# leijue222/Intra-and-Inter-Human-Relation-Network-for-MPEE

Hardware: AMD Instinct MI355X
Metric: images/sec (256x192 crops) I2R-Net HRNet-W48 inference (higher is better)
Workload: dtype f32; 1 GPU; vanilla I2R-Net HRNet-W48-S 256x192, 6 encoder layers, fp32, random weights (BASELINE configs[1]: w48_pure_en6); images_per_gpu=8, persons_per_image=4, crops_per_gpu_step=32, parallelism=single GPU, programs_per_forward=3

## Files before the change

### include/i2r_hip.h

```cpp
#ifndef I2R_HIP_H
#define I2R_HIP_H

#include <stdint.h>

#ifdef __cplusplus
extern "C" {
#endif

#define I2R_ABI_VERSION 17

#define I2R_API __attribute__((visibility("default")))

#define I2R_OK 0
#define I2R_E_ARG (-1)
#define I2R_E_LAUNCH (-2)
#define I2R_E_NODEV (-3)

#define I2R_MAX_TAPS 9

typedef struct i2r_conv_desc {
    const float* in;
    const float* in2;
    const float* w;
    const float* bias;
    const float* res1;
    const float* res2;
    const float* res_post;
    float* out;
    int32_t n_img;
    int32_t in_h, in_w, in_cs;
    int32_t cin;
    int32_t conv_h, conv_w;
    int32_t out_h, out_w, out_cs;
    int32_t cout, cout_pad;
    int32_t stride;
    int32_t iy0, ix0;
    int32_t ntaps;
    int32_t dy[I2R_MAX_TAPS], dx[I2R_MAX_TAPS];
    int32_t out_step, out_off_y, out_off_x, rep;
    int32_t relu;
    int32_t tile_h, tile_w;
    int32_t ck;
    int32_t wn;
    int32_t mt;
    int32_t dtype;
    int32_t in_f16, out_f16;
    int32_t algo;
    int32_t t1_shift, t2_shift;
    const float* t1;
    const float* t2;
    float* y;
    int32_t seq;
} i2r_conv_desc;

I2R_API int i2r_conv(const i2r_conv_desc* d, void* stream);

#define I2R_MAX_GROUP 4
I2R_API int i2r_conv_grouped(const i2r_conv_desc* const* descs, int32_t n, const int32_t* block_map, int32_t map_len,
                     void* stream);

I2R_API int i2r_stem_conv(const float* in_nchw, const float* w, const float* bias, float* out_nhwc, int32_t n_img,
                  int32_t cin, int32_t in_h, int32_t in_w, int32_t cout, int32_t out_cs, int32_t n_src, int32_t n_valid,
                  int32_t out_dt , void* stream);

I2R_API int i2r_pe_res_stem(const float* mask_nchw, const float* w_pre, const float* w7, const float* bias, float* out_nhwc,
                    int32_t n_img, int32_t in_h, int32_t in_w, int32_t cout, int32_t out_cs, int32_t n_src, int32_t n_valid, void* stream);

typedef struct i2r_pe_cat_vec_args {
    const float* in; const float* w; const float* bias; float* out;
    int32_t n_img, in_h, in_w, th, tw, rate, vec, out_cs, c0, c_end, n_src, n_valid;
} i2r_pe_cat_vec_args;
I2R_API int i2r_pe_cat_vec(const i2r_pe_cat_vec_args* a, void* stream);

I2R_API int i2r_maxpool3x3s2(const float* in, float* out, int32_t n_img, int32_t in_h, int32_t in_w, int32_t c,
                     int32_t in_cs, int32_t out_cs, void* stream);

I2R_API int i2r_head(const float* in, const float* w, const float* bias, float* out_nchw, int32_t n_img, int32_t h,
             int32_t w_, int32_t cin, int32_t in_cs, int32_t cout, void* stream);

I2R_API int i2r_conv_kernel_name(const i2r_conv_desc* const* descs, int32_t n, char* buf, int32_t buflen);

I2R_API int i2r_conv_grid(const i2r_conv_desc* const* descs, int32_t n, int32_t with_map, int32_t* grid, int32_t* seq);

I2R_API int i2r_flip_merge(const float* y, const float* y_flipped, const int32_t* joint_map, float* out, int32_t n, int32_t joints,
                   int32_t h, int32_t w, void* stream);

I2R_API int i2r_decode(const float* heatmaps, const float* center, const float* scale, float* preds, float* maxvals, int32_t n,
               int32_t joints, int32_t h, int32_t w, int32_t blur_kernel, int32_t transform_back, void* stream);

typedef struct i2r_pose_nms_args {
    const float* preds; const float* maxvals; const float* scale; const float* area; const float* box_score;
    const int32_t* img_off; const float* sigmas;
    float* score; int32_t* rank; int32_t* n_keep;
    double in_vis_thre, oks_thre, oks_vis_thre;
    int32_t n_crops, n_img, joints, max_persons, soft, max_dets, use_oks_vis, reserved;
} i2r_pose_nms_args;
I2R_API int i2r_pose_nms(const i2r_pose_nms_args* a, void* stream);

I2R_API int i2r_group_nearest(const double* anchors, const int32_t* person_off, const int32_t* member_off, int32_t n_img, int32_t n_persons,
                              int32_t n_members, int32_t max_patch, int32_t* members, void* stream);

typedef struct i2r_oks_match_args {
    const float* dt_kpts; const float* dt_score; const uint8_t* dt_valid; const int32_t* dt_off;
    const double* gt_kpts; const double* gt_area; const double* gt_bbox; const int32_t* gt_flags; const int32_t* gt_off;
    const double* sigmas; const double* thr; const double* area_rng;
    int32_t* dt_rank; uint32_t* dt_match; uint32_t* dt_ignore; uint8_t* gt_ignore; double* oks; const int64_t* oks_off;
    int64_t oks_len;
    int32_t n_dt, n_gt, n_img, joints, n_thr, n_area, max_dets, max_dt_per_img, max_gt_per_img, reserved;
} i2r_oks_match_args;
I2R_API int i2r_oks_match(const i2r_oks_match_args* a, void* stream);

typedef struct i2r_oks_accumulate_args {
    const uint32_t* dt_match; const uint32_t* dt_ignore; const int32_t* dt_rank; const int32_t* order; const int32_t* dt_img;
    const int32_t* img_group; const uint8_t* gt_ignore; const int32_t* gt_off; const double* rec_thr;
    double* precision; double* recall; int32_t* npig;
    int32_t n_dt, n_gt, n_img, n_part, n_group, n_thr, n_area, n_rec;
} i2r_oks_accumulate_args;
I2R_API int i2r_oks_accumulate(const i2r_oks_accumulate_args* a, void* stream);

typedef struct i2r_joint_targets_args {
    const double* joints_hm; const float* joints_vis; const float* joints_weight;
    float* target_weight; float* target;
    double sigma;
    int32_t n_crops, joints, h, w;
} i2r_joint_targets_args;
I2R_API int i2r_joint_targets(const i2r_joint_targets_args* a, void* stream);

typedef struct i2r_val_metrics_args {
    const float* output;
    const float* target; const float* target_weight;
    const double* joints_hm; const float* joints_vis; const float* joints_weight;
    void* ws;
    double* loss; double* acc; double* avg_acc; int32_t* cnt; float* pred; double* sse; int32_t* hits; int32_t* valid; double* meter;
    double sigma;
    int32_t n_crops, joints, h, w, use_target_weight, reserved;
} i2r_val_metrics_args;
I2R_API int i2r_val_metrics(const i2r_val_metrics_args* a, void* stream);

typedef struct i2r_val_combine_args {
    const double* parts;
    double* sse; int32_t* hits; int32_t* valid;
    double* loss; double* acc; double* avg_acc; int32_t* cnt; int32_t* n_crops; double* meter;
    int32_t n_part, joints, h, w;
} i2r_val_combine_args;
I2R_API int i2r_val_combine(const i2r_val_combine_args* a, void* stream);

I2R_API int i2r_crop_affine(const unsigned char* img, int32_t ih, int32_t iw, int32_t row_bytes, int32_t swap_rb, const float* inv_trans,
                    const float* mean, const float* inv_std, float* out, int32_t n, int32_t oh, int32_t ow, void* stream);

I2R_API int i2r_box_mask(const int32_t* boxes, int32_t ih, int32_t iw, float* out, int32_t n, int32_t oh, int32_t ow, void* stream);

I2R_API int i2r_crop_affine_cv2(const unsigned char* img, int32_t ih, int32_t iw, int32_t row_bytes, int32_t swap_rb, const double* inv_m,
                        const float* mean, const float* inv_std, float* out, int32_t n, int32_t oh, int32_t ow, void* stream);
I2R_API int i2r_box_mask_cv2(const int32_t* boxes, int32_t ih, int32_t iw, float* out, int32_t n, int32_t oh, int32_t ow, void* stream);

typedef struct {
    const unsigned char* img;
    int32_t ih, iw, row_bytes, reserved;
} i2r_image_ref;
typedef struct {
    double inv_m[6];
    int32_t box[4];
    int32_t image;
    int32_t reserved[3];
} i2r_crop_ref;
I2R_API int i2r_person_inputs_cv2(const i2r_image_ref* images, int32_t n_images, const i2r_crop_ref* crops, int32_t n_crops, int32_t swap_rb,
                          const float* mean, const float* inv_std, float* x_out, float* mask_out, int32_t oh, int32_t ow, void* stream);

I2R_API int i2r_layernorm(const float* in, const float* w, const float* b, float* out, int32_t npix, int32_t c, int32_t cs,
                  float eps, int32_t out_dt , void* stream);

I2R_API int i2r_window_attn(const float* qkv, const float* bias_qkv, float* out, int32_t n_img, int32_t h, int32_t w, int32_t c,
                    int32_t hs, int32_t heads, void* stream);

I2R_API int i2r_hrt_attn_block(const float* x, float* out, const float* ln_w, const float* ln_b, const void* wqkv, const float* bqkv,
                       const void* wo, const float* bo, int32_t n_img, int32_t h, int32_t w, int32_t c, int32_t cs, int32_t heads,
                       float eps, int32_t dtype, int32_t variant, void* stream);

I2R_API int i2r_hrt_mlp_block(const float* x, float* out, const float* ln_w, const float* ln_b, const void* w1, const float* b1,
                      const float* wdw, const float* bdw, const void* w2, const float* b2, int32_t n_img, int32_t h, int32_t w,
                      int32_t c, int32_t cs, int32_t hidden_pad, float eps, int32_t dtype, int32_t variant, void* stream);

I2R_API int i2r_dwconv3x3(const float* in, const float* w, const float* bias, float* out, int32_t n_img, int32_t in_h, int32_t in_w,
                  int32_t c, int32_t cs, int32_t stride, int32_t act, int32_t dt ,
                  void* stream);

I2R_API int i2r_upsample_bilinear_add(const float* low, const float* res, float* out, int32_t n_img, int32_t low_h, int32_t low_w,
                              int32_t scale, int32_t c, int32_t cs, int32_t act, void* stream);
struct i2r_up_args;
I2R_API int i2r_upsample_bilinear_add_multi(const struct i2r_up_args* a, void* stream);

I2R_API int i2r_fuse_up_add(const float* base, const float* t1, int32_t s1, const float* t2, int32_t s2, float* out, int32_t n_img,
                    int32_t h, int32_t w, int32_t cs, int32_t act, int32_t dt, void* stream);

typedef struct i2r_conv1x1_pair_args {
    const float* x; const float* w_a; const float* b_a; const float* res; float* y;
    const float* w_b; const float* b_b; float* z;
    int32_t n_pix, k_a, ca_out, cb_out, x_cs, y_cs, z_cs, relu_a, relu_b, mt;
} i2r_conv1x1_pair_args;
I2R_API int i2r_conv1x1_pair(const i2r_conv1x1_pair_args* a, void* stream);

typedef struct i2r_conv1x1_lp_args {
    const void* x; const void* w; const float* bias; const void* res1; const void* res_post; void* out;
    int32_t n_pix, cin_pad, cout_pad, x_cs, out_cs, act, dtype, in_16, out_16, mt;
    const void* res2;
} i2r_conv1x1_lp_args;
I2R_API int i2r_conv1x1_lp(const i2r_conv1x1_lp_args* a, void* stream);

typedef struct i2r_encoder_desc {
    const float* src;
    const float* pos;
    float* kbuf;
    float* vbuf;
    float* out;
    const int32_t* grp_off;
    const float* w_in;
    const float* b_in;
    const float* w_out;
    const float* b_out;
    const float* ln1_w; const float* ln1_b;
    const float* w1;
    const float* b1;
    const float* w2;
    const float* b2;
    const float* ln2_w; const float* ln2_b;
    int32_t n_tok, n_grp;
    int32_t d;
    int32_t cs;
    int32_t dff_pad;
    int32_t pos_period;
    int32_t n_qtiles32;
    float ln_eps;
    int32_t dtype;
    int32_t n_qtiles16, n_qtiles64;
    const void* w_in_lp; const void* w_out_lp; const void* w1_lp; const void* w2_lp;
    const float* next_w_in; const float* next_b_in; float* next_kbuf; float* next_vbuf;
    const float* vec_lp;
    float* split_ws; int32_t* split_cnt;
    int32_t n_qtiles192;
} i2r_encoder_desc;

I2R_API int i2r_encoder_kv(const i2r_encoder_desc* d, void* stream);
I2R_API int i2r_encoder_layer(const i2r_encoder_desc* d, void* stream);

typedef struct i2r_mh_attn_args {
    const float* qk; const float* v; float* out; const int32_t* grp_off;
    int32_t n_grp, heads, hp, k_off, qk_cs, v_cs, out_cs, n_qtiles16, n_qtiles32, n_qtiles64;
    const int32_t* key_len;
} i2r_mh_attn_args;
I2R_API int i2r_mh_attention(const i2r_mh_attn_args* a, void* stream);

typedef struct i2r_attn_weights_args {
    const float* qk; float* out; const int32_t* grp_off; const int64_t* out_off; float* ws;
    int32_t n_grp, heads, hp, k_off, qk_cs, n_tiles, ws_stride;
} i2r_attn_weights_args;
I2R_API int i2r_attn_weights(const i2r_attn_weights_args* a, void* stream);

typedef struct i2r_attn_query_args {
    const float* qk; float* out; const int32_t* grp_off; const int64_t* out_off; float* ws; const int32_t* q_tok; const int32_t* q_cnt;
    float* rows; const int32_t* grp_off_host;
    int32_t n_grp, heads, hp, k_off, qk_cs, n_tiles, ws_stride, mode, K, scale, h, w, n_col_tiles, reserved;
} i2r_attn_query_args;
I2R_API int i2r_attn_query_maps(const i2r_attn_query_args* a, void* stream);

I2R_API int i2r_rows_gather(const float* src, float* out, const int32_t* map, int32_t n_out, int32_t floats_per_crop, void* stream);
I2R_API int i2r_view_scramble(const float* o, float* out, const int32_t* person_map, int32_t n_out, int32_t n_images, int32_t max_persons, int32_t c,
                              int32_t cs, int32_t hw, void* stream);
typedef struct i2r_gather_args { const float* src; float* out; const int32_t* map; int32_t n_out, floats_per_crop; } i2r_gather_args;
typedef struct i2r_scramble_args { const float* o; float* out; const int32_t* person_map; int32_t n_out, n_images, max_persons, c, cs, hw; } i2r_scramble_args;

#define I2R_MAX_GATHER_SEGS 8
typedef struct i2r_gather_seg { const void* src; void* out; const int32_t* map; int32_t n_out, n_src; int64_t row_bytes; } i2r_gather_seg;
typedef struct i2r_gather_multi_args { i2r_gather_seg seg[I2R_MAX_GATHER_SEGS ]; int32_t n_seg; } i2r_gather_multi_args;
I2R_API int i2r_rows_gather_multi(const i2r_gather_multi_args* a, void* stream);

enum {
    I2R_OP_CONV = 1, I2R_OP_STEM = 2, I2R_OP_MAXPOOL = 3, I2R_OP_HEAD = 4,
    I2R_OP_ENC_KV = 5, I2R_OP_ENC_LAYER = 6, I2R_OP_FORK = 7, I2R_OP_JOIN = 8, I2R_OP_CONV_GROUP = 9,
    I2R_OP_LAYERNORM = 10, I2R_OP_WINATTN = 11, I2R_OP_DWCONV = 12, I2R_OP_UPSAMPLE = 13,
    I2R_OP_PE_RES_STEM = 15, I2R_OP_HRT_ATTN = 16, I2R_OP_HRT_MLP = 17,  I2R_OP_FUSE_UP = 19,
    I2R_OP_CONV1X1_PAIR = 20, I2R_OP_CONV1X1_LP = 21, I2R_OP_MH_ATTN = 22, I2R_OP_PE_CAT_VEC = 23, I2R_OP_ROWS_GATHER = 24, I2R_OP_VIEW_SCRAMBLE = 25,
    I2R_OP_RECORD = 26, I2R_OP_WAIT = 27, I2R_OP_LANE_FLAGS = 28, I2R_OP_ATTN_WEIGHTS = 29,
    I2R_OP_ATTN_QUERY = 30,
    I2R_OP_ROWS_GATHER_MULTI = 31
};

typedef struct i2r_stem_args {
    const float* in; const float* w; const float* bias; float* out;
    int32_t n_img, cin, in_h, in_w, cout, out_cs, n_src, n_valid, out_dt;
} i2r_stem_args;

typedef struct i2r_pe_res_args {
    const float* in; const float* w_pre; const float* w7; const float* bias; float* out;
    int32_t n_img, in_h, in_w, cout, out_cs, n_src, n_valid;
} i2r_pe_res_args;

typedef struct i2r_pool_args {
    const float* in; float* out;
    int32_t n_img, in_h, in_w, c, in_cs, out_cs;
} i2r_pool_args;

typedef struct i2r_head_args {
    const float* in; const float* w; const float* bias; float* out;
    int32_t n_img, h, w_, cin, in_cs, cout;
} i2r_head_args;

typedef struct i2r_ln_args {
    const float* in; const float* w; const float* b; float* out;
    int32_t npix, c, cs; float eps; int32_t out_dt;
} i2r_ln_args;

typedef struct i2r_winattn_args {
    const float* qkv; const float* bias; float* out;
    int32_t n_img, h, w_, c, cs, heads;
} i2r_winattn_args;

typedef struct i2r_hrt_attn_args {
    const float* x; float* out; const float* ln_w; const float* ln_b; const void* wqkv; const float* bqkv; const void* wo; const float* bo;
    int32_t n_img, h, w_, c, cs, heads; float eps; int32_t dtype, variant;
} i2r_hrt_attn_args;

typedef struct i2r_hrt_mlp_args {
    const float* x; float* out; const float* ln_w; const float* ln_b; const void* w1; const float* b1; const float* wdw; const float* bdw;
    const void* w2; const float* b2;
    int32_t n_img, h, w_, c, cs, hidden_pad; float eps; int32_t dtype, variant;
} i2r_hrt_mlp_args;

typedef struct i2r_dw_args {
    const float* in; const float* w; const float* bias; float* out;
    int32_t n_img, in_h, in_w, c, cs, stride, act, dt;
} i2r_dw_args;

typedef struct i2r_up_args {
    const float* low; const float* res; float* out;
    int32_t n_img, low_h, low_w, scale, c, cs, act;
    const float* low2; const float* low3;
    int32_t scale2, scale3;
} i2r_up_args;

typedef struct i2r_fuse_up_args {
    const float* base; const float* t1; const float* t2; float* out;
    int32_t n_img, h, w, cs, s1, s2, act, dt;
} i2r_fuse_up_args;

typedef struct i2r_conv_group_args {
    const i2r_conv_desc* d[I2R_MAX_GROUP];
    const int32_t* block_map;
    int32_t n;
    int32_t map_len;
} i2r_conv_group_args;

typedef struct i2r_op {
    int32_t kind;
    int32_t lane;
    const void* args;
} i2r_op;

I2R_API int i2r_run_program(const i2r_op* ops, int32_t n_ops, void* const* streams, void* const* events);
I2R_API int i2r_run_program_timed(const i2r_op* ops, int32_t n_ops, void* const* streams, void* const* events, void* const* t0,
                                  void* const* t1);

I2R_API int i2r_abi_version(void);
I2R_API const char* i2r_last_error(void);
I2R_API int i2r_device_check(int32_t dev, int32_t* cu_count, int32_t* lds_bytes);

#ifdef __cplusplus
}
#endif
#endif
```

### intra-and-inter-human-relation-network-for-mpee_amd/cabi.py

```python
import ctypes as C
import os

import torch

_HERE = os.path.dirname(os.path.abspath(__file__))
LIB_PATH = os.path.join(_HERE, "libi2r_hip.so")

MAX_TAPS = 9
ABI_VERSION = 17
OP_CONV, OP_STEM, OP_MAXPOOL, OP_HEAD, OP_ENC_KV, OP_ENC_LAYER, OP_FORK, OP_JOIN, OP_CONV_GROUP = 1, 2, 3, 4, 5, 6, 7, 8, 9
MAX_GROUP = 4
OP_LAYERNORM, OP_WINATTN, OP_DWCONV, OP_UPSAMPLE = 10, 11, 12, 13
OP_CONV_CHAIN = 14
OP_PE_RES_STEM = 15
OP_HRT_ATTN = 16
OP_HRT_MLP = 17
OP_XSYNC = 18
OP_FUSE_UP = 19
OP_CONV1X1_PAIR = 20
OP_CONV1X1_LP = 21
OP_MH_ATTN = 22
OP_PE_CAT_VEC = 23
OP_ROWS_GATHER, OP_VIEW_SCRAMBLE = 24, 25
OP_RECORD, OP_WAIT = 26, 27
OP_LANE_FLAGS = 28
CAPTURE_OP_ATTN_WEIGHTS = 29
CAPTURE_OP_ATTN_QUERY = 30
GROUPS_OP_ROWS_GATHER_MULTI = 31
MAX_GATHER_SEGS = 8
SYNC_OPS = (OP_FORK, OP_JOIN, OP_XSYNC, OP_RECORD, OP_WAIT, OP_LANE_FLAGS)

_fp = C.c_void_p
_i32 = C.c_int32


class ConvDesc(C.Structure):
    _fields_ = [
        ("in_", _fp), ("in2", _fp), ("w", _fp), ("bias", _fp), ("res1", _fp), ("res2", _fp), ("res_post", _fp), ("out", _fp),
        ("n_img", _i32), ("in_h", _i32), ("in_w", _i32), ("in_cs", _i32), ("cin", _i32),
        ("conv_h", _i32), ("conv_w", _i32), ("out_h", _i32), ("out_w", _i32), ("out_cs", _i32),
        ("cout", _i32), ("cout_pad", _i32), ("stride", _i32), ("iy0", _i32), ("ix0", _i32), ("ntaps", _i32),
        ("dy", _i32 * MAX_TAPS), ("dx", _i32 * MAX_TAPS),
        ("out_step", _i32), ("out_off_y", _i32), ("out_off_x", _i32), ("rep", _i32), ("relu", _i32),
        ("tile_h", _i32), ("tile_w", _i32), ("ck", _i32), ("wn", _i32), ("mt", _i32), ("dtype", _i32),
        ("in_f16", _i32), ("out_f16", _i32), ("algo", _i32),
        ("t1_shift", _i32), ("t2_shift", _i32), ("t1", _fp), ("t2", _fp), ("y", _fp),
        ("seq", _i32),
    ]


class EncoderDesc(C.Structure):
    _fields_ = [
        ("src", _fp), ("pos", _fp), ("kbuf", _fp), ("vbuf", _fp), ("out", _fp), ("grp_off", _fp),
        ("w_in", _fp), ("b_in", _fp), ("w_out", _fp), ("b_out", _fp), ("ln1_w", _fp), ("ln1_b", _fp),
        ("w1", _fp), ("b1", _fp), ("w2", _fp), ("b2", _fp), ("ln2_w", _fp), ("ln2_b", _fp),
        ("n_tok", _i32), ("n_grp", _i32), ("d", _i32), ("cs", _i32), ("dff_pad", _i32), ("pos_period", _i32),
        ("n_qtiles32", _i32), ("ln_eps", C.c_float), ("dtype", _i32), ("n_qtiles16", _i32), ("n_qtiles64", _i32),
        ("w_in_lp", _fp), ("w_out_lp", _fp), ("w1_lp", _fp), ("w2_lp", _fp),
        ("next_w_in", _fp), ("next_b_in", _fp), ("next_kbuf", _fp), ("next_vbuf", _fp), ("vec_lp", _fp),
        ("split_ws", _fp), ("split_cnt", _fp), ("n_qtiles192", _i32),
    ]


class StemArgs(C.Structure):
    _fields_ = [("in_", _fp), ("w", _fp), ("bias", _fp), ("out", _fp),
                ("n_img", _i32), ("cin", _i32), ("in_h", _i32), ("in_w", _i32), ("cout", _i32), ("out_cs", _i32), ("n_src", _i32),
                ("n_valid", _i32), ("out_dt", _i32)]


class PeResArgs(C.Structure):
    _fields_ = [("in_", _fp), ("w_pre", _fp), ("w7", _fp), ("bias", _fp), ("out", _fp),
                ("n_img", _i32), ("in_h", _i32), ("in_w", _i32), ("cout", _i32), ("out_cs", _i32), ("n_src", _i32), ("n_valid", _i32)]


class PeCatVecArgs(C.Structure):
    _fields_ = [("in_", _fp), ("w", _fp), ("bias", _fp), ("out", _fp),
                ("n_img", _i32), ("in_h", _i32), ("in_w", _i32), ("th", _i32), ("tw", _i32), ("rate", _i32), ("vec", _i32), ("out_cs", _i32),
                ("c0", _i32), ("c_end", _i32), ("n_src", _i32), ("n_valid", _i32)]


class PoolArgs(C.Structure):
    _fields_ = [("in_", _fp), ("out", _fp),
                ("n_img", _i32), ("in_h", _i32), ("in_w", _i32), ("c", _i32), ("in_cs", _i32), ("out_cs", _i32)]


class HeadArgs(C.Structure):
    _fields_ = [("in_", _fp), ("w", _fp), ("bias", _fp), ("out", _fp),
                ("n_img", _i32), ("h", _i32), ("w_", _i32), ("cin", _i32), ("in_cs", _i32), ("cout", _i32)]


class LnArgs(C.Structure):
    _fields_ = [("in_", _fp), ("w", _fp), ("b", _fp), ("out", _fp), ("npix", _i32), ("c", _i32), ("cs", _i32), ("eps", C.c_float),
                ("out_dt", _i32)]


class MhAttnArgs(C.Structure):
    _fields_ = [("qk", _fp), ("v", _fp), ("out", _fp), ("grp_off", _fp),
                ("n_grp", _i32), ("heads", _i32), ("hp", _i32), ("k_off", _i32), ("qk_cs", _i32), ("v_cs", _i32), ("out_cs", _i32),
                ("n_qtiles16", _i32), ("n_qtiles32", _i32), ("n_qtiles64", _i32), ("key_len", _fp)]


class AttnWeightsArgs(C.Structure):
    _fields_ = [("qk", _fp), ("out", _fp), ("grp_off", _fp), ("out_off", _fp), ("ws", _fp),
                ("n_grp", _i32), ("heads", _i32), ("hp", _i32), ("k_off", _i32), ("qk_cs", _i32), ("n_tiles", _i32), ("ws_stride", _i32)]


class AttnQueryArgs(C.Structure):
    _fields_ = [("qk", _fp), ("out", _fp), ("grp_off", _fp), ("out_off", _fp), ("ws", _fp), ("q_tok", _fp), ("q_cnt", _fp), ("rows", _fp),
                ("grp_off_host", _fp),
                ("n_grp", _i32), ("heads", _i32), ("hp", _i32), ("k_off", _i32), ("qk_cs", _i32), ("n_tiles", _i32), ("ws_stride", _i32),
                ("mode", _i32), ("K", _i32), ("scale", _i32), ("h", _i32), ("w", _i32), ("n_col_tiles", _i32), ("reserved", _i32)]


class GatherArgs(C.Structure):
    _fields_ = [("src", _fp), ("out", _fp), ("map", _fp), ("n_out", _i32), ("floats_per_crop", _i32)]


class GatherSeg(C.Structure):
    _fields_ = [("src", _fp), ("out", _fp), ("map", _fp), ("n_out", _i32), ("n_src", _i32), ("row_bytes", C.c_int64)]


class GatherMultiArgs(C.Structure):
    _fields_ = [("seg", GatherSeg * MAX_GATHER_SEGS), ("n_seg", _i32)]


class ScrambleArgs(C.Structure):
    _fields_ = [("o", _fp), ("out", _fp), ("person_map", _fp), ("n_out", _i32), ("n_images", _i32), ("max_persons", _i32), ("c", _i32), ("cs", _i32),
                ("hw", _i32)]


class WinAttnArgs(C.Structure):
    _fields_ = [("qkv", _fp), ("bias", _fp), ("out", _fp),
                ("n_img", _i32), ("h", _i32), ("w_", _i32), ("c", _i32), ("cs", _i32), ("heads", _i32)]


class HrtAttnArgs(C.Structure):
    _fields_ = [("x", _fp), ("out", _fp), ("ln_w", _fp), ("ln_b", _fp), ("wqkv", _fp), ("bqkv", _fp), ("wo", _fp), ("bo", _fp),
                ("n_img", _i32), ("h", _i32), ("w_", _i32), ("c", _i32), ("cs", _i32), ("heads", _i32), ("eps", C.c_float), ("dtype", _i32),
                ("variant", _i32)]


class HrtMlpArgs(C.Structure):
    _fields_ = [("x", _fp), ("out", _fp), ("ln_w", _fp), ("ln_b", _fp), ("w1", _fp), ("b1", _fp), ("wdw", _fp), ("bdw", _fp), ("w2", _fp),
                ("b2", _fp), ("n_img", _i32), ("h", _i32), ("w_", _i32), ("c", _i32), ("cs", _i32), ("hidden_pad", _i32), ("eps", C.c_float),
                ("dtype", _i32), ("variant", _i32)]


class DwArgs(C.Structure):
    _fields_ = [("in_", _fp), ("w", _fp), ("bias", _fp), ("out", _fp),
                ("n_img", _i32), ("in_h", _i32), ("in_w", _i32), ("c", _i32), ("cs", _i32), ("stride", _i32), ("act", _i32), ("dt", _i32)]


class UpArgs(C.Structure):
    _fields_ = [("low", _fp), ("res", _fp), ("out", _fp),
                ("n_img", _i32), ("low_h", _i32), ("low_w", _i32), ("scale", _i32), ("c", _i32), ("cs", _i32), ("act", _i32),
                ("low2", _fp), ("low3", _fp), ("scale2", _i32), ("scale3", _i32)]


class FuseUpArgs(C.Structure):
    _fields_ = [("base", _fp), ("t1", _fp), ("t2", _fp), ("out", _fp),
                ("n_img", _i32), ("h", _i32), ("w", _i32), ("cs", _i32), ("s1", _i32), ("s2", _i32), ("act", _i32), ("dt", _i32)]


class Conv1x1PairArgs(C.Structure):
    _fields_ = [("x", _fp), ("w_a", _fp), ("b_a", _fp), ("res", _fp), ("y", _fp), ("w_b", _fp), ("b_b", _fp), ("z", _fp),
                ("n_pix", _i32), ("k_a", _i32), ("ca_out", _i32), ("cb_out", _i32), ("x_cs", _i32), ("y_cs", _i32), ("z_cs", _i32),
                ("relu_a", _i32), ("relu_b", _i32), ("mt", _i32)]


class Conv1x1LpArgs(C.Structure):
    _fields_ = [("x", _fp), ("w", _fp), ("bias", _fp), ("res1", _fp), ("res_post", _fp), ("out", _fp),
                ("n_pix", _i32), ("cin_pad", _i32), ("cout_pad", _i32), ("x_cs", _i32), ("out_cs", _i32), ("act", _i32), ("dtype", _i32),
                ("in_16", _i32), ("out_16", _i32), ("mt", _i32), ("res2", _fp)]


class ConvGroupArgs(C.Structure):
    _fields_ = [("d", C.POINTER(ConvDesc) * MAX_GROUP), ("block_map", _fp), ("n", _i32), ("map_len", _i32)]


class PoseNmsArgs(C.Structure):
    _fields_ = [("preds", _fp), ("maxvals", _fp), ("scale", _fp), ("area", _fp), ("box_score", _fp), ("img_off", _fp), ("sigmas", _fp),
                ("score", _fp), ("rank", _fp), ("n_keep", _fp),
                ("in_vis_thre", C.c_double), ("oks_thre", C.c_double), ("oks_vis_thre", C.c_double),
                ("n_crops", _i32), ("n_img", _i32), ("joints", _i32), ("max_persons", _i32), ("soft", _i32), ("max_dets", _i32),
                ("use_oks_vis", _i32), ("reserved", _i32)]


class OksMatchArgs(C.Structure):
    _fields_ = [("dt_kpts", _fp), ("dt_score", _fp), ("dt_valid", _fp), ("dt_off", _fp),
                ("gt_kpts", _fp), ("gt_area", _fp), ("gt_bbox", _fp), ("gt_flags", _fp), ("gt_off", _fp),
                ("sigmas", _fp), ("thr", _fp), ("area_rng", _fp),
                ("dt_rank", _fp), ("dt_match", _fp), ("dt_ignore", _fp), ("gt_ignore", _fp), ("oks", _fp), ("oks_off", _fp),
                ("oks_len", C.c_int64),
                ("n_dt", _i32), ("n_gt", _i32), ("n_img", _i32), ("joints", _i32), ("n_thr", _i32), ("n_area", _i32), ("max_dets", _i32),
                ("max_dt_per_img", _i32), ("max_gt_per_img", _i32), ("reserved", _i32)]


class OksAccumulateArgs(C.Structure):
    _fields_ = [("dt_match", _fp), ("dt_ignore", _fp), ("dt_rank", _fp), ("order", _fp), ("dt_img", _fp),
                ("img_group", _fp), ("gt_ignore", _fp), ("gt_off", _fp), ("rec_thr", _fp),
                ("precision", _fp), ("recall", _fp), ("npig", _fp),
                ("n_dt", _i32), ("n_gt", _i32), ("n_img", _i32), ("n_part", _i32), ("n_group", _i32), ("n_thr", _i32), ("n_area", _i32),
                ("n_rec", _i32)]


class JointTargetsArgs(C.Structure):
    _fields_ = [("joints_hm", _fp), ("joints_vis", _fp), ("joints_weight", _fp), ("target_weight", _fp), ("target", _fp),
                ("sigma", C.c_double), ("n_crops", _i32), ("joints", _i32), ("h", _i32), ("w", _i32)]


class ValMetricsArgs(C.Structure):
    _fields_ = [("output", _fp), ("target", _fp), ("target_weight", _fp), ("joints_hm", _fp), ("joints_vis", _fp), ("joints_weight", _fp),
                ("ws", _fp), ("loss", _fp), ("acc", _fp), ("avg_acc", _fp), ("cnt", _fp), ("pred", _fp), ("sse", _fp), ("hits", _fp),
                ("valid", _fp), ("meter", _fp), ("sigma", C.c_double),
                ("n_crops", _i32), ("joints", _i32), ("h", _i32), ("w", _i32), ("use_target_weight", _i32), ("reserved", _i32)]


class ValCombineArgs(C.Structure):
    _fields_ = [("parts", _fp), ("sse", _fp), ("hits", _fp), ("valid", _fp), ("loss", _fp), ("acc", _fp), ("avg_acc", _fp), ("cnt", _fp),
                ("n_crops", _fp), ("meter", _fp), ("n_part", _i32), ("joints", _i32), ("h", _i32), ("w", _i32)]


class ImageRef(C.Structure):
    _fields_ = [("img", C.c_void_p), ("ih", _i32), ("iw", _i32), ("row_bytes", _i32), ("reserved", _i32)]


class CropRef(C.Structure):
    _fields_ = [("inv_m", C.c_double * 6), ("box", _i32 * 4), ("image", _i32), ("reserved", _i32 * 3)]


class Op(C.Structure):
    _fields_ = [("kind", _i32), ("lane", _i32), ("args", C.c_void_p)]


EXPORTS = ("i2r_conv", "i2r_conv_grouped", "i2r_conv_kernel_name", "i2r_conv_grid", "i2r_stem_conv", "i2r_pe_res_stem", "i2r_maxpool3x3s2", "i2r_head", "i2r_layernorm", "i2r_window_attn", "i2r_hrt_attn_block", "i2r_hrt_mlp_block", "i2r_dwconv3x3",
           "i2r_upsample_bilinear_add", "i2r_upsample_bilinear_add_multi", "i2r_fuse_up_add", "i2r_conv1x1_pair", "i2r_conv1x1_lp", "i2r_flip_merge", "i2r_decode", "i2r_pose_nms", "i2r_group_nearest", "i2r_oks_match", "i2r_oks_accumulate", "i2r_joint_targets", "i2r_val_metrics", "i2r_val_combine", "i2r_crop_affine", "i2r_box_mask", "i2r_crop_affine_cv2", "i2r_box_mask_cv2", "i2r_person_inputs_cv2", "i2r_encoder_kv", "i2r_encoder_layer", "i2r_mh_attention", "i2r_attn_weights", "i2r_attn_query_maps", "i2r_pe_cat_vec", "i2r_rows_gather", "i2r_rows_gather_multi", "i2r_view_scramble",
           "i2r_run_program", "i2r_run_program_timed", "i2r_abi_version", "i2r_last_error", "i2r_device_check")

_LIB = None


class I2RError(RuntimeError):
    pass


def load_library(path=LIB_PATH):
    if not os.path.exists(path):
        raise I2RError(
            "HIP extension %s is missing -- build it with `python -c 'import __graft_entry__ as g; g.build()'`. "
            "There is no CPU fallback for the product path." % path)
    L = C.CDLL(path)
    L.i2r_conv.argtypes = [C.POINTER(ConvDesc), C.c_void_p]
    L.i2r_conv_grouped.argtypes = [C.POINTER(C.POINTER(ConvDesc)), _i32, _fp, _i32, C.c_void_p]
    L.i2r_conv_kernel_name.argtypes = [C.POINTER(C.POINTER(ConvDesc)), _i32, C.c_char_p, _i32]
    L.i2r_conv_grid.argtypes = [C.POINTER(C.POINTER(ConvDesc)), _i32, _i32, C.POINTER(_i32), C.POINTER(_i32)]
    L.i2r_stem_conv.argtypes = [_fp, _fp, _fp, _fp, _i32, _i32, _i32, _i32, _i32, _i32, _i32, _i32, _i32, C.c_void_p]
    L.i2r_pe_res_stem.argtypes = [_fp, _fp, _fp, _fp, _fp, _i32, _i32, _i32, _i32, _i32, _i32, _i32, C.c_void_p]
    L.i2r_flip_merge.argtypes = [_fp, _fp, _fp, _fp, _i32, _i32, _i32, _i32, C.c_void_p]
    L.i2r_decode.argtypes = [_fp, _fp, _fp, _fp, _fp, _i32, _i32, _i32, _i32, _i32, _i32, C.c_void_p]
    L.i2r_pose_nms.argtypes = [C.POINTER(PoseNmsArgs), C.c_void_p]
    L.i2r_group_nearest.argtypes = [_fp, _fp, _fp, _i32, _i32, _i32, _i32, _fp, C.c_void_p]
    L.i2r_oks_match.argtypes = [C.POINTER(OksMatchArgs), C.c_void_p]
    L.i2r_oks_accumulate.argtypes = [C.POINTER(OksAccumulateArgs), C.c_void_p]
    L.i2r_joint_targets.argtypes = [C.POINTER(JointTargetsArgs), C.c_void_p]
    L.i2r_val_metrics.argtypes = [C.POINTER(ValMetricsArgs), C.c_void_p]
    L.i2r_val_combine.argtypes = [C.POINTER(ValCombineArgs), C.c_void_p]
    L.i2r_crop_affine.argtypes = [_fp, _i32, _i32, _i32, _i32, _fp, _fp, _fp, _fp, _i32, _i32, _i32, C.c_void_p]
    L.i2r_box_mask.argtypes = [_fp, _i32, _i32, _fp, _i32, _i32, _i32, C.c_void_p]
    L.i2r_crop_affine_cv2.argtypes = [_fp, _i32, _i32, _i32, _i32, _fp, _fp, _fp, _fp, _i32, _i32, _i32, C.c_void_p]
    L.i2r_box_mask_cv2.argtypes = [_fp, _i32, _i32, _fp, _i32, _i32, _i32, C.c_void_p]
    L.i2r_person_inputs_cv2.argtypes = [_fp, _i32, _fp, _i32, _i32, C.POINTER(C.c_float), C.POINTER(C.c_float), _fp, _fp, _i32, _i32, C.c_void_p]
    L.i2r_fuse_up_add.argtypes = [_fp, _fp, _i32, _fp, _i32, _fp, _i32, _i32, _i32, _i32, _i32, _i32, C.c_void_p]
    L.i2r_conv1x1_pair.argtypes = [C.POINTER(Conv1x1PairArgs), C.c_void_p]
    L.i2r_conv1x1_lp.argtypes = [C.POINTER(Conv1x1LpArgs), C.c_void_p]
    L.i2r_maxpool3x3s2.argtypes = [_fp, _fp, _i32, _i32, _i32, _i32, _i32, _i32, C.c_void_p]
    L.i2r_head.argtypes = [_fp, _fp, _fp, _fp, _i32, _i32, _i32, _i32, _i32, _i32, C.c_void_p]
    L.i2r_layernorm.argtypes = [_fp, _fp, _fp, _fp, _i32, _i32, _i32, C.c_float, _i32, C.c_void_p]
    L.i2r_window_attn.argtypes = [_fp, _fp, _fp, _i32, _i32, _i32, _i32, _i32, _i32, C.c_void_p]
    L.i2r_hrt_attn_block.argtypes = [_fp, _fp, _fp, _fp, _fp, _fp, _fp, _fp, _i32, _i32, _i32, _i32, _i32, _i32, C.c_float, _i32, _i32, C.c_void_p]
    L.i2r_hrt_mlp_block.argtypes = [_fp] * 10 + [_i32] * 6 + [C.c_float, _i32, _i32, C.c_void_p]
    L.i2r_dwconv3x3.argtypes = [_fp, _fp, _fp, _fp, _i32, _i32, _i32, _i32, _i32, _i32, _i32, _i32, C.c_void_p]
    L.i2r_upsample_bilinear_add_multi.argtypes = [C.POINTER(UpArgs), C.c_void_p]
    L.i2r_upsample_bilinear_add.argtypes = [_fp, _fp, _fp, _i32, _i32, _i32, _i32, _i32, _i32, _i32, C.c_void_p]
    L.i2r_encoder_kv.argtypes = [C.POINTER(EncoderDesc), C.c_void_p]
    L.i2r_encoder_layer.argtypes = [C.POINTER(EncoderDesc), C.c_void_p]
    L.i2r_rows_gather.argtypes = [_fp, _fp, _fp, _i32, _i32, C.c_void_p]
    L.i2r_rows_gather_multi.argtypes = [C.POINTER(GatherMultiArgs), C.c_void_p]
    L.i2r_view_scramble.argtypes = [_fp, _fp, _fp, _i32, _i32, _i32, _i32, _i32, _i32, C.c_void_p]
    L.i2r_pe_cat_vec.argtypes = [C.POINTER(PeCatVecArgs), C.c_void_p]
    L.i2r_mh_attention.argtypes = [C.POINTER(MhAttnArgs), C.c_void_p]
    L.i2r_attn_weights.argtypes = [C.POINTER(AttnWeightsArgs), C.c_void_p]
    L.i2r_attn_query_maps.argtypes = [C.POINTER(AttnQueryArgs), C.c_void_p]
    L.i2r_run_program.argtypes = [C.POINTER(Op), _i32, C.POINTER(C.c_void_p), C.POINTER(C.c_void_p)]
    L.i2r_run_program_timed.argtypes = [C.POINTER(Op), _i32] + [C.POINTER(C.c_void_p)] * 4
    L.i2r_device_check.argtypes = [_i32, C.POINTER(_i32), C.POINTER(_i32)]
    L.i2r_last_error.restype = C.c_char_p
    for name in EXPORTS:
        if name != "i2r_last_error":
            getattr(L, name).restype = C.c_int
    return L


def lib():
    global _LIB
    if _LIB is None:
        L = load_library()
        if L.i2r_abi_version() != ABI_VERSION:
            raise I2RError("libi2r_hip.so ABI version %d != %d -- rebuild" % (L.i2r_abi_version(), ABI_VERSION))
        _LIB = L
    return _LIB


def check(rc, what=""):
    if rc != 0:
        msg = lib().i2r_last_error()
        raise I2RError("%s failed (rc=%d): %s" % (what or "i2r call", rc, msg.decode() if msg else "?"))


def require_gfx950(device_index=0):
    cu, lds = _i32(0), _i32(0)
    check(lib().i2r_device_check(device_index, C.byref(cu), C.byref(lds)), "i2r_device_check")
    return cu.value, lds.value
```

### intra-and-inter-human-relation-network-for-mpee_amd/csrc/i2r_conv.h

```cpp
#pragma once
#include "i2r_common.h"

#ifdef I2R_TUNING
#define I2R_DBG(p) ((p).dbg)
#else
#define I2R_DBG(p) 0
#endif

namespace {

struct ConvK {
    const float* in;
    const float* in2;
    const float* w;
    const float* bias;
    const float* res1;
    const float* res2;
    const float* res_post;
    float* out;
    int n_img, in_h, in_w, in_cs, cin;
    int conv_h, conv_w, out_h, out_w, out_cs, cout, cout_pad;
    int stride, iy0, ix0, ntaps;
    int tap_kh, tap_kw;
    int out_step, out_off_y, out_off_x, rep, relu;
    int tile_h, tile_w, tiles_y, tiles_x, n_cblk;
    int ph, pw, plane;
    int ck;
    int wn;
    int dtype;
    int in16, out16;
    int dbg;
    unsigned m_cblk, m_tx, m_ty, m_pw, m_tw;
    unsigned in_bytes, w_bytes, out_bytes;
    int wn_log, npass;
    int algo, w_fwlog, w_pitch, w_half, w_nfrag, w_rcp;
    int w_seq;
    int w_band;
    unsigned w_m_cblk, w_m_img, w_m_tx;
    const float* f_t1;
    const float* f_t2;
    float* f_y;
    int f_sh1, f_sh2;
    unsigned f_bytes1, f_bytes2;
};

__device__ __forceinline__ int div_m(int n, int d, unsigned m) { return d == 1 ? n : (int)__umulhi((unsigned)n, m); }

typedef unsigned u32x4 __attribute__((ext_vector_type(4)));
typedef unsigned u32x2 __attribute__((ext_vector_type(2)));
constexpr unsigned kOOB = 0x80000000u;
__device__ __forceinline__ __amdgpu_buffer_rsrc_t make_rsrc(const void* base, unsigned bytes) {
    return __builtin_amdgcn_make_buffer_rsrc(const_cast<void*>(base), 0, base ? bytes : 0, 0x00020000);
}
__device__ __forceinline__ f32x4 buf_ld16(const __amdgpu_buffer_rsrc_t& rs, unsigned voff, int soff) {
    return __builtin_bit_cast(f32x4, __builtin_amdgcn_raw_buffer_load_b128(rs, voff, soff, 0));
}
__device__ __forceinline__ void buf_st16(const __amdgpu_buffer_rsrc_t& rs, unsigned voff, int soff, f32x4 v) {
    __builtin_amdgcn_raw_buffer_store_b128(__builtin_bit_cast(u32x4, v), rs, voff, soff, 0);
    asm volatile("s_nop 1" ::"v"(v));
}

constexpr int kMaxPP = 5;

constexpr int kMaxGroups = 4;
struct ConvGroupK {
    ConvK g[kMaxGroups];
    int blk_end[kMaxGroups];
    int n;
    const int* blk_map;
};

template <int DT>
__device__ __forceinline__ f32x4 ld_act4(const float* base, size_t off, bool h16) {
    if constexpr (DT != 0) {
        if (h16) {
            const uint2 u = *reinterpret_cast<const uint2*>(reinterpret_cast<const unsigned short*>(base) + off);
            if constexpr (DT == 1)
                return (f32x4){__uint_as_float(u.x << 16), __uint_as_float(u.x & 0xFFFF0000u), __uint_as_float(u.y << 16), __uint_as_float(u.y & 0xFFFF0000u)};
            else {
                typedef _Float16 h4 __attribute__((ext_vector_type(4)));
                const h4 h = __builtin_bit_cast(h4, u);
                return (f32x4){(float)h[0], (float)h[1], (float)h[2], (float)h[3]};
            }
        }
    }
    return *reinterpret_cast<const f32x4*>(base + off);
}
template <int DT>
__device__ __forceinline__ void st_act4(float* base, size_t off, f32x4 v, bool h16) {
    if constexpr (DT != 0) {
        if (h16) {
            uint2 u;
            if constexpr (DT == 1) {
                typedef __bf16 b4 __attribute__((ext_vector_type(4)));
                const b4 b = {(__bf16)v[0], (__bf16)v[1], (__bf16)v[2], (__bf16)v[3]};
                u = __builtin_bit_cast(uint2, b);
            } else {
                typedef _Float16 h4 __attribute__((ext_vector_type(4)));
                const h4 h = {(_Float16)v[0], (_Float16)v[1], (_Float16)v[2], (_Float16)v[3]};
                u = __builtin_bit_cast(uint2, h);
            }
            *reinterpret_cast<uint2*>(reinterpret_cast<unsigned short*>(base) + off) = u;
            return;
        }
    }
    *reinterpret_cast<f32x4*>(base + off) = v;
}

template <int DT>
__device__ __forceinline__ f32x4 buf_ld_act4(const __amdgpu_buffer_rsrc_t& rs, unsigned voff, bool h16) {
    if constexpr (DT != 0) {
        if (h16) {
            const u32x2 u = __builtin_amdgcn_raw_buffer_load_b64(rs, voff, 0, 0);
            if constexpr (DT == 1)
                return (f32x4){__uint_as_float(u.x << 16), __uint_as_float(u.x & 0xFFFF0000u), __uint_as_float(u.y << 16), __uint_as_float(u.y & 0xFFFF0000u)};
            else {
                typedef _Float16 h4 __attribute__((ext_vector_type(4)));
                const h4 h = __builtin_bit_cast(h4, u);
                return (f32x4){(float)h[0], (float)h[1], (float)h[2], (float)h[3]};
            }
        }
    }
    return buf_ld16(rs, voff, 0);
}
template <int DT>
__device__ __forceinline__ void buf_st_act4(const __amdgpu_buffer_rsrc_t& rs, unsigned voff, f32x4 v, bool h16) {
    if constexpr (DT != 0) {
        if (h16) {
            u32x2 u;
            if constexpr (DT == 1) {
                typedef __bf16 b4 __attribute__((ext_vector_type(4)));
                const b4 b = {(__bf16)v[0], (__bf16)v[1], (__bf16)v[2], (__bf16)v[3]};
                u = __builtin_bit_cast(u32x2, b);
            } else {
                typedef _Float16 h4 __attribute__((ext_vector_type(4)));
                const h4 h = {(_Float16)v[0], (_Float16)v[1], (_Float16)v[2], (_Float16)v[3]};
                u = __builtin_bit_cast(u32x2, h);
            }
            __builtin_amdgcn_raw_buffer_store_b64(u, rs, voff, 0, 0);
            return;
        }
    }
    __builtin_amdgcn_raw_buffer_store_b128(__builtin_bit_cast(u32x4, v), rs, voff, 0, 0);
}

template <int MT, int NT, int DT>
__device__ __forceinline__ void conv_epilogue(const ConvK& p, f32x4 (&acc)[MT][NT], int img, int oy0, int ox0, int wm, int n_base,
                                              int li, int g, int tile_px) {
    if ((I2R_DBG(p) & 1) && acc[0][0][0] != 12345.678f) return;
    const int j4 = li & 3;
    const int pj = li >> 2, pq = li & 3;
    const int perm_src = (g * 16 + pq * 4 + pj) * 4;
    auto to_pixel_major = [&](f32x4 v) {
        v = quad_transpose(v, j4);
#pragma unroll
        for (int e = 0; e < 4; ++e) {
            const float x = v[e];
            v[e] = __int_as_float(__builtin_amdgcn_ds_bpermute(perm_src, __float_as_int(x)));
        }
        return v;
    };
    const bool h16 = DT != 0 && p.out16;
    const unsigned esz = h16 ? 2u : 4u;
    const __amdgpu_buffer_rsrc_t rs_out = make_rsrc(p.out, p.out_bytes), rs_r1 = make_rsrc(p.res1, p.out_bytes),
                                 rs_r2 = make_rsrc(p.res2, p.out_bytes), rs_rp = make_rsrc(p.res_post, p.out_bytes);
    auto finish = [&](f32x4 t, int n, bool full, unsigned voff) {
        if (p.relu == 1) {
            t[0] = fmaxf(t[0], 0.f); t[1] = fmaxf(t[1], 0.f); t[2] = fmaxf(t[2], 0.f); t[3] = fmaxf(t[3], 0.f);
        } else if (p.relu == 2) {
#pragma unroll
            for (int e = 0; e < 4; ++e) t[e] = 0.5f * t[e] * (1.f + erff(t[e] * 0.70710678118654752f));
        }
        if (p.res_post) t += buf_ld_act4<DT>(rs_rp, voff, h16);
        if (!full) {
#pragma unroll
            for (int e = 0; e < 4; ++e)
                if (n + e >= p.cout) t[e] = 0.f;
        }
        return t;
    };
    f32x4 bias[NT];
    unsigned noff[NT];
    const bool tail = n_base + NT * 16 > p.cout || n_base + NT * 16 > p.out_cs;
#pragma unroll
    for (int nt = 0; nt < NT; ++nt) {
        const int n = n_base + nt * 16 + pq * 4;
        const bool nok = n < p.cout_pad && (n + 4 <= p.cout || n + 4 <= p.out_cs);
        noff[nt] = nok ? (unsigned)n * esz : kOOB;
        bias[nt] = n < p.cout_pad ? *reinterpret_cast<const f32x4*>(p.bias + n) : (f32x4){0.f, 0.f, 0.f, 0.f};
    }
    if (p.rep == 1 && !(I2R_DBG(p) & 16)) {
        unsigned off[MT];
#pragma unroll
        for (int mt = 0; mt < MT; ++mt) {
            const int m = (wm * MT + mt) * 16 + g * 4 + pj;
            const int ty = div_m(m, p.tile_w, p.m_tw), tx = m - ty * p.tile_w;
            const int oy = oy0 + ty, ox = ox0 + tx;
            const bool pv = m < tile_px && oy < p.conv_h && ox < p.conv_w;
            off[mt] = pv ? (unsigned)(((img * p.out_h + oy * p.out_step + p.out_off_y) * p.out_w + ox * p.out_step + p.out_off_x) * p.out_cs) * esz : kOOB;
        }
        auto at = [&](int mt, int nt) { return (tail && noff[nt] == kOOB) ? kOOB : off[mt] + noff[nt]; };
        f32x4 r[MT][NT];
#pragma unroll
        for (int mt = 0; mt < MT; ++mt)
#pragma unroll
            for (int nt = 0; nt < NT; ++nt) {
                r[mt][nt] = bias[nt];
                if (p.res1) r[mt][nt] += buf_ld_act4<DT>(rs_r1, at(mt, nt), h16);
                if (p.res2) r[mt][nt] += buf_ld_act4<DT>(rs_r2, at(mt, nt), h16);
            }
#pragma unroll
        for (int mt = 0; mt < MT; ++mt)
#pragma unroll
            for (int nt = 0; nt < NT; ++nt) {
                const f32x4 v = to_pixel_major(acc[mt][nt]);
                const int n = n_base + nt * 16 + pq * 4;
                const unsigned o = at(mt, nt);
                buf_st_act4<DT>(rs_out, o, finish(v + r[mt][nt], n, !tail || n + 4 <= p.cout, o), h16);
            }
        return;
    }
#pragma unroll
    for (int mt = 0; mt < MT; ++mt) {
        const int m = (wm * MT + mt) * 16 + g * 4 + pj;
        const int ty = div_m(m, p.tile_w, p.m_tw), tx = m - ty * p.tile_w;
        const int oy = oy0 + ty, ox = ox0 + tx;
        const bool pvalid = m < tile_px && oy < p.conv_h && ox < p.conv_w;
        const int by = oy * p.out_step + p.out_off_y, bx = ox * p.out_step + p.out_off_x;
#pragma unroll
        for (int nt = 0; nt < NT; ++nt) {
            const f32x4 v = to_pixel_major(acc[mt][nt]) + bias[nt];
            const int n = n_base + nt * 16 + pq * 4;
            if (!pvalid || noff[nt] == kOOB) continue;
            for (int ry = 0; ry < p.rep; ++ry)
                for (int rx = 0; rx < p.rep; ++rx) {
                    const unsigned o = (unsigned)(((img * p.out_h + by + ry) * p.out_w + bx + rx) * p.out_cs) * esz + noff[nt];
                    f32x4 t = v;
                    if (p.res1) t += buf_ld_act4<DT>(rs_r1, o, h16);
                    if (p.res2) t += buf_ld_act4<DT>(rs_r2, o, h16);
                    buf_st_act4<DT>(rs_out, o, finish(t, n, n + 4 <= p.cout, o), h16);
                }
        }
    }
}



typedef void (*conv_fn)(const ConvGroupK);

}

void* i2r_pick_conv_bf16(int nt, int mt, int cap, int pf);
void* i2r_pick_conv_f16(int nt, int mt, int cap, int pf);
void* i2r_pick_conv_wino(int nt, int mt, int fin);
size_t i2r_conv_wino_lds(int nt, int mt, int plane);
```

### intra-and-inter-human-relation-network-for-mpee_amd/csrc/i2r_conv.hip

```cpp
#include <stdlib.h>

#include <algorithm>

#include "i2r_conv.h"

namespace {

template <int MT, int NT, int CAP, int PF>
__device__ __forceinline__ void conv_body(const ConvK& p, int bid, f32x4* lds) {
    const int tid = threadIdx.x;
    unsigned long long ts0 = 0, ts1 = 0, ts2 = 0;
    const bool stamp = (I2R_DBG(p) & 8) != 0;
    const int bid_stamp = bid;
    if (stamp) ts0 = __builtin_amdgcn_s_memtime();
    const int lane = tid & 63, wave = tid >> 6;
    const int WN = p.wn;
    const int wm = wave >> p.wn_log, wn = wave & (WN - 1);
    const int li = lane & 15, g = lane >> 4;

    int q = div_m(bid, p.n_cblk, p.m_cblk);
    const int cb = bid - q * p.n_cblk;
    bid = q;
    q = div_m(bid, p.tiles_x, p.m_tx);
    const int tile_x = bid - q * p.tiles_x;
    bid = q;
    const int img = div_m(bid, p.tiles_y, p.m_ty);
    const int tile_y = bid - img * p.tiles_y;
    const int oy0 = tile_y * p.tile_h, ox0 = tile_x * p.tile_w;
    const int py0 = oy0 * p.stride + p.iy0, px0 = ox0 * p.stride + p.ix0;
    const int phw = p.ph * p.pw;

    constexpr int NPP = PF > 0 ? 4 * PF : kMaxPP;
    const int ul = tid & 3;
    const __amdgpu_buffer_rsrc_t rs_in = make_rsrc(p.in, p.in_bytes), rs_in2 = make_rsrc(p.in2, p.in_bytes), rs_w = make_rsrc(p.w, p.w_bytes);
    unsigned goff[NPP];
#pragma unroll
    for (int j = 0; j < NPP; ++j) {
        const int pp = PF > 0 ? (tid >> 2) + j * 64 : tid + j * 256;
        goff[j] = kOOB;
        if (pp < phw) {
            const int py = div_m(pp, p.pw, p.m_pw), px = pp - py * p.pw;
            const int iy = py0 + py, ix = px0 + px;
            if (iy >= 0 && iy < p.in_h && ix >= 0 && ix < p.in_w) goff[j] = (unsigned)(((img * p.in_h + iy) * p.in_w + ix) * p.in_cs) * 4u;
        }
    }
    const int npp = (phw + 255) >> 8;

    const int tile_px = p.tile_h * p.tile_w;
    int ppix[MT];
#pragma unroll
    for (int mt = 0; mt < MT; ++mt) {
        int m = (wm * MT + mt) * 16 + li;
        if (m >= tile_px) m = 0;
        const int ty = div_m(m, p.tile_w, p.m_tw), tx = m - ty * p.tile_w;
        ppix[mt] = ty * p.stride * p.pw + tx * p.stride;
    }

    f32x4 acc[MT][NT];
#pragma unroll
    for (int mt = 0; mt < MT; ++mt)
#pragma unroll
        for (int nt = 0; nt < NT; ++nt) acc[mt][nt] = (f32x4){0.f, 0.f, 0.f, 0.f};

    const int n_base = (cb * WN + wn) * NT * 16;
    const int cin4 = p.cin >> 2;
    const unsigned wlane = (unsigned)(n_base + li + g * p.cout_pad) * 16u;

    auto run_chunk = [&](const f32x4* buf, int c0, int ckc, auto&& mid) {
        const int ncs = ckc >> 4;
        const int nit = p.ntaps * ncs;
        const int wp0 = (c0 >> 2) * p.cout_pad * 16;
        int wp = wp0;
        const int inc_cs = 4 * p.cout_pad * 16;
        const int inc_tap = (cin4 - (ncs - 1) * 4) * p.cout_pad * 16;
        int cs_n = 0, tx_n = 0, ty_n = 0;
        auto fetch = [&](f32x4(&a)[MT], f32x4(&b)[NT]) {
#pragma unroll
            for (int nt = 0; nt < NT; ++nt) b[nt] = buf_ld16(rs_w, wlane + nt * 256u, (I2R_DBG(p) & 4) ? wp0 : wp);
            const int abase = (cs_n * 4 + g) * p.plane + ty_n * p.pw + tx_n;
#pragma unroll
            for (int mt = 0; mt < MT; ++mt) a[mt] = buf[abase + ppix[mt]];
            if (++cs_n == ncs) {
                cs_n = 0;
                wp += inc_tap;
                if (++tx_n == p.tap_kw) {
                    tx_n = 0;
                    if (++ty_n == p.tap_kh) { ty_n = 0; wp = wp0; }
                }
            } else {
                wp += inc_cs;
            }
        };
        auto fma_step = [&](const f32x4(&a)[MT], const f32x4(&b)[NT]) {
#pragma unroll
            for (int s = 0; s < 4; ++s)
#pragma unroll
                for (int mt = 0; mt < MT; ++mt)
#pragma unroll
                    for (int nt = 0; nt < NT; ++nt) acc[mt][nt] = mfma16(a[mt][s], b[nt][s], acc[mt][nt]);
        };
        f32x4 a0[MT], a1[MT], b0[NT], b1[NT];
        fetch(a0, b0);
        mid();
        int it = 0;
        for (; it + 2 <= nit; it += 2) {
            fetch(a1, b1);
            fma_step(a0, b0);
            fetch(a0, b0);
            fma_step(a1, b1);
        }
        if (it < nit) fma_step(a0, b0);
    };

    if constexpr (PF > 0) {
        constexpr int UQ = CAP / 4, PJ = 4 * PF;
        f32x4 v[UQ][PJ];
        const int ckg = p.ck >> 2;
        auto stage_load = [&](int c0) {
#pragma unroll
            for (int uq = 0; uq < UQ; ++uq)
                if (uq * 4 < ckg) {
#pragma unroll
                    for (int j = 0; j < PJ; ++j)
                        v[uq][j] = (I2R_DBG(p) & 2) ? (f32x4){0.f, 0.f, 0.f, 0.f} : buf_ld16(rs_in, goff[j] + (uq * 4 + ul) * 16u, c0 * 4);
                }
            if (p.in2) {
#pragma unroll
                for (int uq = 0; uq < UQ; ++uq)
                    if (uq * 4 < ckg) {
#pragma unroll
                        for (int j = 0; j < PJ; ++j)
                            v[uq][j] += buf_ld16(rs_in2, goff[j] + (uq * 4 + ul) * 16u, c0 * 4);
                    }
            }
        };
        auto stage_store = [&](f32x4* buf) {
#pragma unroll
            for (int uq = 0; uq < UQ; ++uq)
                if (uq * 4 < ckg) {
#pragma unroll
                    for (int j = 0; j < PJ; ++j) {
                        const int pp = (tid >> 2) + j * 64;
                        if (pp < phw) buf[(uq * 4 + ul) * p.plane + pp] = v[uq][j];
                    }
                }
        };
        const int npass = p.npass;
        stage_load(0);
        stage_store(lds);
        __syncthreads();
        if (stamp) ts1 = __builtin_amdgcn_s_memtime();
        for (int pass = 0; pass < npass; ++pass) {
            f32x4* cur = lds + (pass & 1) * ckg * p.plane;
            f32x4* nxt = lds + ((pass + 1) & 1) * ckg * p.plane;
            const bool more = pass + 1 < npass;
            run_chunk(cur, pass * p.ck, p.ck, [&]() { if (more) stage_load((pass + 1) * p.ck); });
            if (more) stage_store(nxt);
            __syncthreads();
        }
    } else {
        for (int c0 = 0; c0 < p.cin; c0 += p.ck) {
            const int ckc = min(p.ck, p.cin - c0);
            const int ncg = ckc >> 2;
            if (c0 != 0) __syncthreads();
            for (int cg0 = 0; cg0 < ncg; cg0 += 4) {
                f32x4 v[4][kMaxPP];
#pragma unroll
                for (int u = 0; u < 4; ++u)
#pragma unroll
                    for (int j = 0; j < kMaxPP; ++j)
                        v[u][j] = (j < npp && !(I2R_DBG(p) & 2)) ? buf_ld16(rs_in, goff[j] + u * 16u, (c0 + cg0 * 4) * 4) : (f32x4){0.f, 0.f, 0.f, 0.f};
                if (p.in2) {
#pragma unroll
                    for (int u = 0; u < 4; ++u)
#pragma unroll
                        for (int j = 0; j < kMaxPP; ++j)
                            if (j < npp) v[u][j] += buf_ld16(rs_in2, goff[j] + u * 16u, (c0 + cg0 * 4) * 4);
                }
#pragma unroll
                for (int u = 0; u < 4; ++u)
#pragma unroll
                    for (int j = 0; j < kMaxPP; ++j) {
                        const int pp = tid + j * 256;
                        if (j < npp && pp < phw)
                            lds[(cg0 + u) * p.plane + pp] = v[u][j];
                    }
            }
            __syncthreads();
            run_chunk(lds, c0, ckc, []() {});
        }
    }

    if (stamp) {
        ts2 = __builtin_amdgcn_s_memtime();
        ConvK q = p;
        q.res2 = nullptr;
        conv_epilogue<MT, NT, 0>(q, acc, img, oy0, ox0, wm, n_base, li, g, tile_px);
        asm volatile("s_waitcnt vmcnt(0)" ::: "memory");
        const unsigned long long ts3 = __builtin_amdgcn_s_memtime();
        if (tid == 0) {
            unsigned long long* o = reinterpret_cast<unsigned long long*>(const_cast<float*>(p.res2)) + (size_t)bid_stamp * 4;
            o[0] = ts0; o[1] = ts1; o[2] = ts2; o[3] = ts3;
            if (I2R_DBG(p) & 32) {
                const unsigned hw = __builtin_amdgcn_s_getreg((4 << 0) | (0 << 6) | (31 << 11));
                const unsigned xcc = __builtin_amdgcn_s_getreg((20 << 0) | (0 << 6) | (3 << 11));
                o[1] = ((unsigned long long)xcc << 32) | hw;
            }
        }
        return;
    }
    conv_epilogue<MT, NT, 0>(p, acc, img, oy0, ox0, wm, n_base, li, g, tile_px);
}

template <int MT, int NT, int CAP, int PF>
__global__ __launch_bounds__(256) void conv_igemm_f32(const ConvGroupK grp) {
    extern __shared__ __attribute__((aligned(16))) f32x4 lds[];
    int bid = blockIdx.x, gi = 0, start = 0;
    if (grp.blk_map) {
        const int v = __builtin_amdgcn_readfirstlane(grp.blk_map[bid]);
        gi = v >> 24;
        bid = v & 0xFFFFFF;
    } else {
#pragma unroll
        for (int i = 0; i < kMaxGroups - 1; ++i)
            if (i + 1 < grp.n && bid >= grp.blk_end[i]) { gi = i + 1; start = grp.blk_end[i]; }
    }
    conv_body<MT, NT, CAP, PF>(grp.g[gi], bid - start, lds);
}

template <int NT, int CAP, int PF>
conv_fn pick_mt(int mt) {
    switch (mt) {
        case 1: return conv_igemm_f32<1, NT, CAP, PF>;
        case 2: return conv_igemm_f32<2, NT, CAP, PF>;
        case 3: return conv_igemm_f32<3, NT, CAP, PF>;
        case 4: return conv_igemm_f32<4, NT, CAP, PF>;
    }
    return nullptr;
}

template <int CAP, int PF>
conv_fn pick_nt(int nt, int mt) {
    switch (nt) {
        case 3: return pick_mt<3, CAP, PF>(mt);
        case 4: return pick_mt<4, CAP, PF>(mt);
        case 5: return pick_mt<5, CAP, PF>(mt);
    }
    return nullptr;
}

conv_fn pick_kernel(int nt, int mt, int cap, int pf) {
    if (pf == 0) return pick_nt<4, 0>(nt, mt);
    if (pf == 1 && cap == 4) return pick_nt<4, 1>(nt, mt);
    if (pf == 1 && cap == 12) return pick_nt<12, 1>(nt, mt);
    if (pf == 2 && cap == 4) return pick_nt<4, 2>(nt, mt);
    return nullptr;
}

inline int cdiv(int a, int b) { return (a + b - 1) / b; }

}

static void copy_desc(const i2r_conv_desc* d, ConvK& k) {
    k.in = d->in; k.in2 = d->in2; k.w = d->w; k.bias = d->bias; k.res1 = d->res1; k.res2 = d->res2; k.res_post = d->res_post; k.out = d->out;
    k.n_img = d->n_img; k.in_h = d->in_h; k.in_w = d->in_w; k.in_cs = d->in_cs; k.cin = d->cin;
    k.conv_h = d->conv_h; k.conv_w = d->conv_w; k.out_h = d->out_h; k.out_w = d->out_w; k.out_cs = d->out_cs;
    k.cout = d->cout; k.cout_pad = d->cout_pad; k.stride = d->stride; k.iy0 = d->iy0; k.ix0 = d->ix0;
    k.ntaps = d->ntaps;
    k.out_step = d->out_step; k.out_off_y = d->out_off_y; k.out_off_x = d->out_off_x; k.rep = d->rep; k.relu = d->relu;
    k.dtype = d->dtype;
    k.in16 = d->in_f16; k.out16 = d->out_f16;
    k.algo = d->algo; k.w_fwlog = k.w_pitch = k.w_half = k.w_nfrag = k.w_rcp = k.w_band = 0; k.w_seq = 1;
    k.w_m_cblk = k.w_m_img = k.w_m_tx = 0; k.in_bytes = k.w_bytes = k.out_bytes = 0;
    k.m_cblk = k.m_tx = k.m_ty = k.m_pw = k.m_tw = 0; k.wn_log = 0; k.npass = 0;
    k.dbg = 0;
    k.f_t1 = d->t1; k.f_t2 = d->t2; k.f_y = d->y; k.f_sh1 = d->t1_shift; k.f_sh2 = d->t2 ? d->t2_shift : 0; k.f_bytes1 = k.f_bytes2 = 0;
}

constexpr int kWinoMaxSeq = 8;
constexpr int kWinoRunPasses = 6;
constexpr int kWinoMinWg = 512;
static long long wino_runs(const ConvK& k, int mt) { return (((long long)k.w_nfrag + mt - 1) / mt + k.w_seq - 1) / k.w_seq; }

static int prepare_wino(const i2r_conv_desc* d, int force_mt, ConvK& k, int* nt_out, int* mt_out, int* cap_out, int* pf_out, size_t* lds_out,
                        long long* nblk_out) {
    I2R_CHECK_ARG(d->dtype == 0 && !d->in_f16 && !d->out_f16, "i2r_conv: the Winograd kernels are fp32");
    I2R_CHECK_ARG(d->stride == 1 && d->ntaps == 9 && d->iy0 == -1 && d->ix0 == -1 && d->rep == 1 && d->out_step == 1 && d->out_off_y == 0 &&
                      d->out_off_x == 0 && d->in2 == nullptr,
                  "i2r_conv: algo 1 (Winograd) needs a plain 3x3 stride-1 pad-1 convolution");
    for (int t = 0; t < 9; ++t) I2R_CHECK_ARG(d->dy[t] == t / 3 && d->dx[t] == t % 3, "i2r_conv: algo 1 needs row-major 3x3 taps");
    I2R_CHECK_ARG(d->relu == 0 || d->relu == 1, "i2r_conv: algo 1 has no GELU epilogue");
    I2R_CHECK_ARG((long long)d->n_img * d->in_h * d->in_w * d->in_cs < (1ll << 29) && (long long)d->n_img * d->out_h * d->out_w * d->out_cs < (1ll << 29) &&
                      (long long)16 * d->cin * d->cout_pad < (1ll << 29),
                  "i2r_conv: algo 1 addresses its tensors through buffer descriptors of < 2 GiB");
    I2R_CHECK_ARG(d->conv_h == d->in_h && d->conv_w == d->in_w && d->out_h == d->conv_h && d->out_w == d->conv_w, "i2r_conv: algo 1 geometry");
    if (d->t1) {
        I2R_CHECK_ARG(d->y != nullptr, "i2r_conv: a fused input (t1) needs y");
        I2R_CHECK_ARG(d->in_cs == d->cin, "i2r_conv: fused input: y is complete only when the conv reads every channel (cin=%d in_cs=%d)", d->cin, d->in_cs);
        for (int t = 0; t < (d->t2 ? 2 : 1); ++t) {
            const int sh = t ? d->t2_shift : d->t1_shift;
            I2R_CHECK_ARG((sh == 1 || sh == 2) && d->in_h % (1 << sh) == 0 && d->in_w % (1 << sh) == 0,
                          "i2r_conv: fused input: t%d_shift %d must be 1 or 2 and the %dx%d map divisible by the scale", t + 1, sh, d->in_h, d->in_w);
        }
        const void* others[] = {d->in, d->t1, d->t2, d->out, d->res1, d->res2, d->res_post};
        for (const void* o : others) I2R_CHECK_ARG((const void*)d->y != o, "i2r_conv: fused input: y aliases another tensor of the launch");
        I2R_CHECK_ARG(d->t1 != (const float*)d->out && d->t2 != (const float*)d->out, "i2r_conv: out aliases a fused-input term");
    }
    const int nfrag = d->cout_pad / 16;
    const int nt = nfrag % 3 == 0 ? 3 : (nfrag % 4 == 0 ? 4 : 0);
    I2R_CHECK_ARG(nt != 0, "i2r_conv: algo 1 needs cout_pad=%d to be a multiple of 48 or 64", d->cout_pad);
    const int mt = force_mt ? force_mt : (d->mt ? d->mt : 1);
    I2R_CHECK_ARG(mt == 1, "i2r_conv: algo 1 takes mt 1 (got %d)", mt);
    I2R_CHECK_ARG(d->seq >= 0 && d->seq <= kWinoMaxSeq, "i2r_conv: algo 1 runs 1..%d fragments per workgroup (seq=%d; 0 = choose)", kWinoMaxSeq, d->seq);
    int fw = 0;
    if (d->tile_w) {
        I2R_CHECK_ARG(d->tile_w == 16 || d->tile_w == 8 || d->tile_w == 4, "i2r_conv: algo 1 fragment width %d (16, 8, 4)", d->tile_w);
        fw = d->tile_w / 2;
    } else {
        long long best = -1;
        for (int cand : {8, 4, 2}) {
            const long long n = (long long)cdiv(d->conv_w, 2 * cand) * cdiv(d->conv_h, 32 / cand);
            if (best < 0 || n < best) { best = n; fw = cand; }
        }
    }
    copy_desc(d, k);
    k.w_fwlog = fw == 8 ? 3 : (fw == 4 ? 2 : 1);
    k.tile_w = 2 * fw; k.tile_h = 32 / fw;
    k.tiles_x = cdiv(d->conv_w, k.tile_w); k.tiles_y = cdiv(d->conv_h, k.tile_h);
    k.n_cblk = nfrag / nt;
    k.ph = k.tile_h + 2; k.pw = k.tile_w + 2;
    k.w_half = fw + 1;
    k.w_pitch = fw == 8 ? 20 : (fw == 4 ? 10 : 9);
    k.plane = cdiv(k.ph * k.w_pitch, 16) * 16;
    k.w_rcp = (65536 + k.pw - 1) / k.pw;
    k.in_bytes = (unsigned)((long long)d->n_img * d->in_h * d->in_w * d->in_cs * 4);
    k.w_bytes = (unsigned)((long long)16 * d->cin * d->cout_pad * 4);
    k.out_bytes = (unsigned)((long long)d->n_img * d->out_h * d->out_w * d->out_cs * 4);
    if (d->t1) k.f_bytes1 = (unsigned)((long long)d->n_img * (d->in_h >> d->t1_shift) * (d->in_w >> d->t1_shift) * d->in_cs * 4);
    if (d->t2) k.f_bytes2 = (unsigned)((long long)d->n_img * (d->in_h >> d->t2_shift) * (d->in_w >> d->t2_shift) * d->in_cs * 4);
    auto magic = [](int d) { return d == 1 ? 0u : (unsigned)(((1ull << 32) + d - 1) / d); };
    k.w_m_cblk = magic(k.n_cblk); k.w_m_img = magic(k.tiles_y * k.tiles_x); k.w_m_tx = magic(k.tiles_x);
    k.tap_kw = k.tap_kh = 3;
    k.ck = 16; k.wn = 1;
    const long long nf = (long long)d->n_img * k.tiles_y * k.tiles_x;
    I2R_CHECK_ARG(nf > 0 && nf * k.n_cblk < (1ll << 20) && k.tiles_y * k.tiles_x < 2048 && k.n_cblk < 2048, "i2r_conv: algo 1 grid (%lld fragments)", nf);
    k.w_nfrag = (int)nf;
    k.w_seq = d->seq ? d->seq : 1;
#ifdef I2R_TUNING
    {
        static const int dbg = getenv("I2R_CONV_DBG") ? atoi(getenv("I2R_CONV_DBG")) : 0;
        k.dbg = dbg;
    }
#endif
    *nt_out = nt; *mt_out = mt; *cap_out = 0; *pf_out = 100;
    *lds_out = i2r_conv_wino_lds(nt, mt, k.plane);
    *nblk_out = wino_runs(k, mt) * k.n_cblk;
    return I2R_OK;
}

static void wino_choose_seq(ConvK* g, const i2r_conv_desc* const* descs, int n, int mt) {
    auto total = [&]() { long long t = 0; for (int i = 0; i < n; ++i) t += wino_runs(g[i], mt) * g[i].n_cblk; return t; };
    long long at_one = 0;
    for (int i = 0; i < n; ++i) at_one += ((long long)g[i].w_nfrag + mt - 1) / mt * g[i].n_cblk;
    const long long floor_wg = std::min<long long>(at_one, kWinoMinWg);
    for (int i = 0; i < n; ++i)
        if (descs[i]->seq == 0) g[i].w_seq = std::max(1, std::min(kWinoMaxSeq, kWinoRunPasses / (g[i].cin >> 4)));
    while (total() < floor_wg) {
        int pick = -1;
        for (int i = 0; i < n; ++i) {
            if (descs[i]->seq != 0 || g[i].w_seq == 1) continue;
            const int len = g[i].w_seq * (g[i].cin >> 4);
            if (pick < 0 || len > g[pick].w_seq * (g[pick].cin >> 4) || (len == g[pick].w_seq * (g[pick].cin >> 4) && g[i].cin > g[pick].cin)) pick = i;
        }
        if (pick < 0) break;
        --g[pick].w_seq;
    }
}

static int prepare(const i2r_conv_desc* d, int force_mt, int force_cap, int force_pf, ConvK& k, int* nt_out, int* mt_out, int* cap_out,
                   int* pf_out, size_t* lds_out, long long* nblk_out) {
    I2R_CHECK_ARG(d && d->in && d->w && d->bias && d->out, "i2r_conv: null pointer");
    I2R_CHECK_ARG(d->cin > 0 && d->cin % 16 == 0 && d->cin <= d->in_cs && d->in_cs % 4 == 0,
                  "i2r_conv: cin=%d must be a multiple of 16 and <= in_cs=%d (in_cs %% 4 == 0)", d->cin, d->in_cs);
    I2R_CHECK_ARG(d->cout > 0 && d->cout_pad % 16 == 0 && d->cout <= d->cout_pad && d->cout <= d->out_cs && d->out_cs % 4 == 0,
                  "i2r_conv: cout=%d cout_pad=%d out_cs=%d", d->cout, d->cout_pad, d->out_cs);
    I2R_CHECK_ARG(d->stride == 1 || d->stride == 2, "i2r_conv: stride %d", d->stride);
    I2R_CHECK_ARG(d->dtype >= 0 && d->dtype <= 2 && (d->dtype == 0 || d->in2 == nullptr), "i2r_conv: dtype %d", d->dtype);
    I2R_CHECK_ARG((d->in_f16 == 0 || d->in_f16 == 1) && (d->out_f16 == 0 || d->out_f16 == 1) && (d->dtype != 0 || (!d->in_f16 && !d->out_f16)),
                  "i2r_conv: 16-bit activation storage (in_f16=%d out_f16=%d) needs a 16-bit operand type (dtype=%d)", d->in_f16, d->out_f16, d->dtype);
    I2R_CHECK_ARG(!d->in_f16 || d->in_cs % 8 == 0, "i2r_conv: 16-bit input needs in_cs %% 8 == 0 (in_cs=%d)", d->in_cs);
    I2R_CHECK_ARG(d->ntaps >= 1 && d->ntaps <= I2R_MAX_TAPS, "i2r_conv: ntaps %d", d->ntaps);
    I2R_CHECK_ARG(d->rep >= 1 && d->out_step >= 1, "i2r_conv: rep/out_step");
    I2R_CHECK_ARG((d->conv_h - 1) * d->out_step + d->out_off_y + d->rep <= d->out_h &&
                      (d->conv_w - 1) * d->out_step + d->out_off_x + d->rep <= d->out_w,
                  "i2r_conv: destination grid exceeds out tensor");
    I2R_CHECK_ARG(d->in2 != (const float*)d->out && d->in != (const float*)d->out, "i2r_conv: out aliases in");
    I2R_CHECK_ARG(d->algo == 0 || d->algo == 1, "i2r_conv: algo %d", d->algo);
    I2R_CHECK_ARG(d->t1 ? d->algo == 1 : (!d->t2 && !d->y), "i2r_conv: a fused input (t1, t2, y) needs algo 1 and starts with t1");
    if (d->algo == 1) return prepare_wino(d, force_mt, k, nt_out, mt_out, cap_out, pf_out, lds_out, nblk_out);

    int max_dy = 0, max_dx = 0;
    for (int t = 0; t < d->ntaps; ++t) {
        I2R_CHECK_ARG(d->dy[t] >= 0 && d->dx[t] >= 0, "i2r_conv: negative tap offset");
        if (d->dy[t] > max_dy) max_dy = d->dy[t];
        if (d->dx[t] > max_dx) max_dx = d->dx[t];
    }

    const int nfrag = d->cout_pad / 16;
    int nt = 0;
    for (int cand : {3, 4, 5})
        if (nfrag % cand == 0) { nt = cand; break; }
    I2R_CHECK_ARG(nt != 0, "i2r_conv: cout_pad=%d is not a multiple of 48, 64 or 80", d->cout_pad);
    int wn = d->wn;
    if (wn == 0) {
        const int nb = nfrag / nt;
        wn = (nb % 4 == 0) ? 4 : (nb % 2 == 0) ? 2 : 1;
        if (wn == 4 && d->cout_pad < 192) wn = 2;
    }
    I2R_CHECK_ARG((wn == 1 || wn == 2 || wn == 4) && (nfrag / nt) % wn == 0, "i2r_conv: wn=%d does not divide cout", wn);
    const int wm = 4 / wn;

    int th = d->tile_h, tw = d->tile_w, mt = force_mt ? force_mt : d->mt;
    if (th == 0 || tw == 0) {
        tw = d->conv_w <= 16 ? d->conv_w : (d->conv_w % 16 == 0 ? 16 : (d->conv_w % 12 == 0 ? 12 : 8));
        if (mt == 0) mt = 2;
        th = (wm * mt * 16) / tw;
        if (th < 1) th = 1;
        if (th > d->conv_h) th = d->conv_h;
    }
    if (mt == 0) mt = cdiv(th * tw, wm * 16);
    I2R_CHECK_ARG(mt >= 1 && mt <= 4 && th * tw <= wm * mt * 16, "i2r_conv: tile %dx%d does not fit wm=%d mt=%d", th, tw, wm, mt);

    copy_desc(d, k);
    k.tile_h = th; k.tile_w = tw;
    k.tiles_y = cdiv(d->conv_h, th); k.tiles_x = cdiv(d->conv_w, tw);
    k.n_cblk = nfrag / (nt * wn);
    k.ph = (th - 1) * d->stride + max_dy + 1;
    k.pw = (tw - 1) * d->stride + max_dx + 1;
    I2R_CHECK_ARG(k.ph * k.pw <= kMaxPP * 256, "i2r_conv: patch %dx%d too large", k.ph, k.pw);
#ifdef I2R_TUNING
    static const int plane_pad = getenv("I2R_CONV_PLANE_PAD") ? atoi(getenv("I2R_CONV_PLANE_PAD")) : 0;
#else
    constexpr int plane_pad = 0;
#endif
    k.plane = cdiv(k.ph * k.pw, 16) * 16 + plane_pad;
    k.tap_kw = max_dx + 1;
    k.tap_kh = max_dy + 1;
    for (int t = 0; t < d->ntaps; ++t)
        I2R_CHECK_ARG(d->dy[t] == t / k.tap_kw && d->dx[t] == t % k.tap_kw && d->ntaps == (max_dy + 1) * (max_dx + 1),
                      "i2r_conv: taps must form a dense row-major kh x kw grid");
    const int npp = cdiv(k.ph * k.pw, 256);
#ifdef I2R_TUNING
    static const int pf_env = getenv("I2R_CONV_PF") ? atoi(getenv("I2R_CONV_PF")) : 1;
#else
    constexpr int pf_env = 1;
#endif
    const int cin_g = d->dtype == 0 ? d->cin / 4 : (d->cin / 8 + 3) / 4 * 4;
    const int g_ch = d->dtype == 0 ? 4 : 8;
    int pf = (pf_env && d->ck == 0 && npp <= 2 && cin_g % 4 == 0) ? npp : 0;
    int cap = 4;
    if (force_pf >= 0) {
        I2R_CHECK_ARG(force_pf == 0 || (npp <= force_pf && d->ck == 0 && cin_g % 4 == 0), "i2r_conv: grouped members disagree on the staging mode");
        pf = force_pf;
    }
    int ck = d->ck;
    size_t lds_bytes;
    if (pf > 0) {
        int ckg = 4;
#ifdef I2R_TUNING
        static const int cap_env = getenv("I2R_CONV_CAP") ? atoi(getenv("I2R_CONV_CAP")) : 12;
#else
        constexpr int cap_env = 12;
#endif
        const int cap_max = std::min(cap_env, d->dtype == 0 ? 12 : 8);
        const int cap_lim = force_pf >= 0 ? force_cap : (pf == 1 ? cap_max : 4);
        for (int cand : {12, 8, 4})
            if (cand <= cap_lim && cin_g % cand == 0 && (size_t)2 * cand * k.plane * 16 <= 40 * 1024) { ckg = cand; break; }
        cap = force_pf >= 0 ? force_cap : (ckg > 4 ? cap_max : 4);
        ck = ckg * g_ch;
        lds_bytes = (size_t)2 * ckg * k.plane * 16;
    } else if (d->dtype != 0) {
        const int g8_pad = (d->cin / 8 + 3) / 4 * 4;
        int fit = (24 * 1024 / (k.plane * 16)) / 4 * 4;
        if (fit < 4) fit = 4;
        const int nchunk = cdiv(g8_pad, fit);
        const int ckg = cdiv(cdiv(g8_pad, nchunk), 4) * 4;
        ck = ckg * 8;
        lds_bytes = (size_t)ckg * k.plane * 16;
    } else {
        if (ck == 0) {
            const int budget = 20 * 1024;
            int fit = (budget / (k.plane * 16)) * 4;
            fit = fit < 16 ? 16 : fit / 16 * 16;
            const int nchunk = cdiv(d->cin, fit);
            ck = cdiv(cdiv(d->cin, nchunk), 16) * 16;
        }
        I2R_CHECK_ARG(ck % 16 == 0 && ck >= 16, "i2r_conv: ck=%d", ck);
        lds_bytes = (size_t)(ck / 4) * k.plane * 16;
    }
    k.ck = ck;
    I2R_CHECK_ARG(lds_bytes <= 160 * 1024, "i2r_conv: LDS %zu B", lds_bytes);
    k.wn = wn;
    {
        const long long esz_in = d->in_f16 ? 2 : 4, esz_out = d->out_f16 ? 2 : 4;
        const long long inb = (long long)d->n_img * d->in_h * d->in_w * d->in_cs * esz_in, outb = (long long)d->n_img * d->out_h * d->out_w * d->out_cs * esz_out;
        const long long wb = d->dtype == 0 ? (long long)d->ntaps * d->cin * d->cout_pad * 4 : (long long)d->ntaps * ((d->cin / 8 + 3) / 4 * 4) * 8 * d->cout_pad * 2;
        I2R_CHECK_ARG(inb < (1ll << 31) && outb < (1ll << 31) && wb < (1ll << 31), "i2r_conv: tensors of 2 GiB and more are not supported (in %lld, out %lld, weights %lld bytes)", inb, outb, wb);
        k.in_bytes = (unsigned)inb; k.out_bytes = (unsigned)outb; k.w_bytes = (unsigned)wb;
        auto magic = [](int d) { return d == 1 ? 0u : (unsigned)(((1ull << 32) + d - 1) / d); };
        k.m_cblk = magic(k.n_cblk); k.m_tx = magic(k.tiles_x); k.m_ty = magic(k.tiles_y); k.m_pw = magic(k.pw); k.m_tw = magic(k.tile_w);
        k.wn_log = wn == 4 ? 2 : (wn == 2 ? 1 : 0);
        k.npass = d->dtype == 0 ? d->cin / ck : ((d->cin / 8 + 3) / 4 * 4) / (ck / 8);
    }
#ifdef I2R_TUNING
    {
        static const int dbg = getenv("I2R_CONV_DBG") ? atoi(getenv("I2R_CONV_DBG")) : 0;
        k.dbg = dbg;
    }
#endif
    const long long nblk = (long long)d->n_img * k.tiles_y * k.tiles_x * k.n_cblk;
    I2R_CHECK_ARG(nblk > 0 && nblk < (1ll << 30), "i2r_conv: grid");
    I2R_CHECK_ARG(nblk * std::max(k.n_cblk, std::max(k.tiles_x, k.tiles_y)) < (1ll << 32) && (long long)kMaxPP * 256 * k.pw < (1ll << 32),
                  "i2r_conv: grid of %lld workgroups exceeds the index-decode range", nblk);
    *nt_out = nt; *mt_out = mt; *cap_out = cap; *pf_out = pf; *lds_out = lds_bytes; *nblk_out = nblk;
    return I2R_OK;
}

static int resolve(const i2r_conv_desc* const* descs, int32_t n, ConvGroupK& grp, int* nt0_, int* mt0_, int* cap0_, int* pf0_,
                   size_t* lds_, long long* total_, bool table = true) {
    I2R_CHECK_ARG(descs && n >= 1 && n <= kMaxGroups, "i2r_conv_grouped: 1..%d descriptors", kMaxGroups);
    int nt0 = 0, mt0 = 0, pf0 = -1, cap0 = 4;
    size_t lds_max = 0;
    long long total = 0;
    for (int i = 0; i < n; ++i) I2R_CHECK_ARG(descs[i] && descs[i]->algo == descs[0]->algo, "i2r_conv_grouped: members mix algorithms");
    if (n > 1 && descs[0]->algo == 0) {
        pf0 = 0;
        cap0 = 4;
        bool all_pf = true;
        for (int i = 0; i < n; ++i) {
            ConvK tmp;
            int nt, mt, cap, pf;
            size_t lds;
            long long nblk;
            int rc = prepare(descs[i], mt0, 4, -1, tmp, &nt, &mt, &cap, &pf, &lds, &nblk);
            if (rc) return rc;
            if (i == 0) mt0 = mt;
            if (pf == 0) all_pf = false;
            if (pf > pf0) pf0 = pf;
            if (cap > cap0) cap0 = cap;
        }
        if (!all_pf) pf0 = 0;
        if (pf0 != 1) cap0 = 4;
        mt0 = 0;
    }
    for (int i = 0; i < n; ++i) {
        int nt, mt, cap, pf;
        size_t lds;
        long long nblk;
        int rc = prepare(descs[i], mt0, cap0, pf0, grp.g[i], &nt, &mt, &cap, &pf, &lds, &nblk);
        if (rc) return rc;
        if (i == 0) { nt0 = nt; mt0 = mt; pf0 = pf; cap0 = cap; }
        I2R_CHECK_ARG(nt == nt0 && mt == mt0, "i2r_conv_grouped: descriptor %d has fragment blocking (%d,%d) != (%d,%d)", i, mt, nt, mt0, nt0);
        I2R_CHECK_ARG(descs[i]->dtype == descs[0]->dtype, "i2r_conv_grouped: members mix compute dtypes");
        if (lds > lds_max) lds_max = lds;
        if (descs[i]->algo == 1) continue;
        total += nblk;
        grp.blk_end[i] = (int)total;
    }
    if (descs[0]->algo == 1) {
        wino_choose_seq(grp.g, descs, n, mt0);
        for (int i = 0; i < n; ++i) {
            const long long runs = wino_runs(grp.g[i], mt0);
            long long nblk = runs * grp.g[i].n_cblk;
            if (!table) {
                grp.g[i].w_band = (int)((runs + 7) / 8);
                nblk = (long long)grp.g[i].w_band * 8 * grp.g[i].n_cblk;
            }
            total += nblk;
            grp.blk_end[i] = (int)total;
        }
    }
    for (int i = n; i < kMaxGroups; ++i) { grp.g[i] = grp.g[0]; grp.blk_end[i] = (int)total; }
    grp.n = n;
    I2R_CHECK_ARG(total < (1ll << 31), "i2r_conv_grouped: grid");
    *nt0_ = nt0; *mt0_ = mt0; *cap0_ = cap0; *pf0_ = pf0; *lds_ = lds_max; *total_ = total;
    return I2R_OK;
}

static bool any_fused_input(const i2r_conv_desc* const* descs, int32_t n) {
    for (int i = 0; i < n; ++i)
        if (descs[i]->t1) return true;
    return false;
}

extern "C" int i2r_conv_grouped(const i2r_conv_desc* const* descs, int32_t n, const int32_t* block_map,
                                int32_t map_len, void* stream) {
    ConvGroupK grp;
    int nt0, mt0, cap0, pf0;
    size_t lds_max;
    long long total;
    int rc = resolve(descs, n, grp, &nt0, &mt0, &cap0, &pf0, &lds_max, &total, block_map != nullptr);
    if (rc) return rc;
    grp.blk_map = block_map;
    I2R_CHECK_ARG(block_map == nullptr || map_len == (int32_t)total, "i2r_conv_grouped: block_map has %d entries, grid has %lld", map_len, total);
    conv_fn fn = descs[0]->algo == 1 ? reinterpret_cast<conv_fn>(i2r_pick_conv_wino(nt0, mt0, any_fused_input(descs, n)))
                 : descs[0]->dtype == 0 ? pick_kernel(nt0, mt0, cap0, pf0)
                                      : reinterpret_cast<conv_fn>(descs[0]->dtype == 1 ? i2r_pick_conv_bf16(nt0, mt0, cap0, pf0) : i2r_pick_conv_f16(nt0, mt0, cap0, pf0));
    I2R_CHECK_ARG(fn != nullptr, "i2r_conv: no kernel for nt=%d mt=%d cap=%d pf=%d dtype=%d", nt0, mt0, cap0, pf0, descs[0]->dtype);
    if (lds_max > 64 * 1024)
        (void)hipFuncSetAttribute(reinterpret_cast<const void*>(fn), hipFuncAttributeMaxDynamicSharedMemorySize, (int)lds_max);
    const unsigned grid = (unsigned)total;
    i2r_launch(fn, dim3(grid), dim3(256), lds_max, (hipStream_t)stream, grp);
    I2R_CHECK_LAUNCH("i2r_conv");
    return I2R_OK;
}

extern "C" int i2r_conv(const i2r_conv_desc* d, void* stream) { return i2r_conv_grouped(&d, 1, nullptr, 0, stream); }

extern "C" int i2r_conv_grid(const i2r_conv_desc* const* descs, int32_t n, int32_t with_map, int32_t* grid, int32_t* seq) {
    ConvGroupK grp;
    int nt0, mt0, cap0, pf0;
    size_t lds_max;
    long long total;
    int rc = resolve(descs, n, grp, &nt0, &mt0, &cap0, &pf0, &lds_max, &total, with_map != 0);
    if (rc) return rc;
    I2R_CHECK_ARG(grid != nullptr, "i2r_conv_grid: grid");
    *grid = (int32_t)total;
    if (seq)
        for (int i = 0; i < n; ++i) seq[i] = descs[0]->algo == 1 ? grp.g[i].w_seq : 1;
    return I2R_OK;
}

extern "C" int i2r_conv_kernel_name(const i2r_conv_desc* const* descs, int32_t n, char* buf, int32_t buflen) {
    ConvGroupK grp;
    int nt0, mt0, cap0, pf0;
    size_t lds_max;
    long long total;
    int rc = resolve(descs, n, grp, &nt0, &mt0, &cap0, &pf0, &lds_max, &total);
    if (rc) return rc;
    I2R_CHECK_ARG(buf && buflen > 0, "i2r_conv_kernel_name: buffer");
    if (descs[0]->algo == 1)
        snprintf(buf, (size_t)buflen, "conv_wino_%sf32<%d, %d>", any_fused_input(descs, n) ? "fin_" : "", mt0, nt0);
    else if (descs[0]->dtype)
        snprintf(buf, (size_t)buflen, "conv_igemm_lp<%d, %d, %d, %d>/%s", mt0, nt0, cap0, pf0, descs[0]->dtype == 1 ? "bf16" : "f16");
    else
        snprintf(buf, (size_t)buflen, "conv_igemm_f32<%d, %d, %d, %d>", mt0, nt0, cap0, pf0);
    return I2R_OK;
}
```

### intra-and-inter-human-relation-network-for-mpee_amd/csrc/i2r_conv_wino.hip

```cpp
#include "i2r_conv.h"

namespace {

constexpr int kWinoPatchMax = 108;

typedef const ConvK __attribute__((address_space(4)))* ConvKArg;

template <int MT, int NT, bool FIN>
__device__ __forceinline__ void conv_wino_body(const ConvGroupK& grp, ConvKArg args) {
    extern __shared__ __attribute__((aligned(16))) f32x4 lds[];
    const int tid = threadIdx.x, lane = tid & 63;
    const int wi = __builtin_amdgcn_readfirstlane(tid >> 6);
    const int li = lane & 15, g = lane >> 4;

    int bid = blockIdx.x, gi = 0;
    if (grp.blk_map) {
        const int v = __builtin_amdgcn_readfirstlane(grp.blk_map[bid]);
        gi = v >> 24;
        bid = v & 0xFFFFFF;
    } else {
        int start = 0;
#pragma unroll
        for (int i = 0; i < kMaxGroups - 1; ++i)
            if (i + 1 < grp.n && bid >= grp.blk_end[i]) { gi = i + 1; start = grp.blk_end[i]; }
        bid -= start;
    }
    const ConvK& p = grp.g[gi];
    const bool stamp = (I2R_DBG(p) & 8) != 0;
    unsigned long long ts0 = 0, ts1 = 0, ts2 = 0;
    if (stamp) ts0 = __builtin_amdgcn_s_memtime();

    int wg, cb;
    if (grp.blk_map) {
        wg = div_m(bid, p.n_cblk, p.w_m_cblk);
        cb = bid - wg * p.n_cblk;
    } else {
        const int q = bid >> 3, qq = div_m(q, p.n_cblk, p.w_m_cblk);
        cb = q - qq * p.n_cblk;
        wg = (bid & 7) * p.w_band + qq;
    }
    const int run0 = wg * p.w_seq;
    const int nrun = min(p.w_seq, (p.w_nfrag + MT - 1) / MT - run0);
    if (nrun <= 0) return;
    const int fwl = p.w_fwlog, FW = 1 << fwl;
    const int pitch = p.w_pitch, half = p.w_half, plane = p.plane;
    const int n_base = cb * NT * 16;

    constexpr int NIT = (MT * kWinoPatchMax * 4 + 255) / 256;
    const __amdgpu_buffer_rsrc_t rs_in = __builtin_amdgcn_make_buffer_rsrc(const_cast<float*>(p.in), 0, p.in_bytes, 0x00020000);
    const __amdgpu_buffer_rsrc_t rs_w = __builtin_amdgcn_make_buffer_rsrc(const_cast<float*>(p.w), 0, p.w_bytes, 0x00020000);
    unsigned goff[NIT];
    int lslot[NIT];
    constexpr int kOwn = 1 << 30;
    const bool fin = FIN && p.f_t1 != nullptr, fin2 = fin && p.f_t2 != nullptr;
    const __amdgpu_buffer_rsrc_t rs_t1 = make_rsrc(fin ? p.f_t1 : nullptr, p.f_bytes1), rs_t2 = make_rsrc(fin2 ? p.f_t2 : nullptr, p.f_bytes2),
                                 rs_y = make_rsrc(fin ? p.f_y : nullptr, p.in_bytes);
    unsigned goff1[FIN ? NIT : 1], goff2[FIN ? NIT : 1];
    const int cg = tid & 3;
    auto patch_pixel = [&](const auto& pq, int t, int k, int& f, int& row, int& col) {
        const int PC = pq.pw, PP = pq.ph * pq.pw;
        const int pix = (t + k * 256) >> 2;
        int pp = pix;
        f = 0;
#pragma unroll
        for (int m = 1; m <= MT; ++m)
            if (pix >= m * PP) { f = m; pp = pix - m * PP; }
        row = (pp * pq.w_rcp) >> 16;
        col = pp - row * PC;
    };
#pragma unroll
    for (int k = 0; k < NIT; ++k) {
        int f, row, col;
        patch_pixel(p, tid, k, f, row, col);
        lslot[k] = f < MT ? (f * 4 + cg) * plane + row * pitch + (col & 1) * half + (col >> 1) : -1;
        if constexpr (FIN) {
            if (f < MT && row >= 1 && row < p.ph - 1 && col >= 1 && col < p.pw - 1) lslot[k] |= kOwn;
        }
    }
    auto lane_now = []() {
        int l;
        asm volatile("v_mbcnt_lo_u32_b32 %0, -1, 0\n\tv_mbcnt_hi_u32_b32 %0, -1, %0" : "=v"(l));
        return l;
    };
    int f_img[MT], f_oy[MT], f_ox[MT];
    bool f_ok[MT];
    auto set_fragment = [&](int fg, int t, const auto& ps) {
#pragma unroll
        for (int mt = 0; mt < MT; ++mt) {
            int fid = fg * MT + mt;
            f_ok[mt] = fid < ps.w_nfrag;
            if (!f_ok[mt]) fid = 0;
            f_img[mt] = div_m(fid, (ps.tiles_y * ps.tiles_x), ps.w_m_img);
            const int rem = fid - f_img[mt] * (ps.tiles_y * ps.tiles_x);
            const int fy = div_m(rem, ps.tiles_x, ps.w_m_tx);
            f_oy[mt] = fy * (32 >> fwl);
            f_ox[mt] = (rem - fy * ps.tiles_x) * (2 * FW);
        }
#pragma unroll
        for (int k = 0; k < NIT; ++k) {
            int f, row, col;
            patch_pixel(ps, t, k, f, row, col);
            int img = f_img[0], oy = f_oy[0], ox = f_ox[0];
            bool ok = f_ok[0] && f < MT;
#pragma unroll
            for (int m = 1; m < MT; ++m)
                if (f == m) { img = f_img[m]; oy = f_oy[m]; ox = f_ox[m]; ok = f_ok[m]; }
            const int iy = oy - 1 + row, ix = ox - 1 + col;
            const bool in_img = ok && (unsigned)iy < (unsigned)ps.in_h && (unsigned)ix < (unsigned)ps.in_w;
            goff[k] = in_img ? (unsigned)(((img * ps.in_h + iy) * ps.in_w + ix) * ps.in_cs + (t & 3) * 4) * 4u : kOOB;
            if constexpr (FIN) {
                const int s1 = ps.f_sh1, s2 = ps.f_sh2;
                goff1[k] = in_img ? (unsigned)(((img * (ps.in_h >> s1) + (iy >> s1)) * (ps.in_w >> s1) + (ix >> s1)) * ps.in_cs + (t & 3) * 4) * 4u : kOOB;
                goff2[k] = in_img ? (unsigned)(((img * (ps.in_h >> s2) + (iy >> s2)) * (ps.in_w >> s2) + (ix >> s2)) * ps.in_cs + (t & 3) * 4) * 4u : kOOB;
            }
        }
    };
    f32x4 v[NIT];
    auto stage_load = [&](int c0) {
#pragma unroll
        for (int k = 0; k < NIT; ++k)
            v[k] = (I2R_DBG(p) & 2) ? (f32x4){0.f, 0.f, 0.f, 0.f}
                                    : __builtin_bit_cast(f32x4, __builtin_amdgcn_raw_buffer_load_b128(rs_in, goff[k], c0 * 4, 0));
    };
    f32x4 vt[FIN ? NIT : 1];
    auto stage_load_t1 = [&](int c0) {
        if constexpr (FIN) {
            if (fin) {
#pragma unroll
                for (int k = 0; k < NIT; ++k) vt[k] = buf_ld16(rs_t1, goff1[k], c0 * 4);
            }
        }
    };
    auto stage_mid = [&](int c0) {
        if constexpr (FIN) {
            if (fin2) {
#pragma unroll
                for (int k = 0; k < NIT; ++k) {
                    v[k] += vt[k];
                    vt[k] = buf_ld16(rs_t2, goff2[k], c0 * 4);
                }
            }
        }
    };
    auto stage_store = [&](f32x4* buf, int c0) {
        if constexpr (FIN) {
            if (fin) {
#pragma unroll
                for (int k = 0; k < NIT; ++k) {
                    v[k] += vt[k];
                    v[k][0] = fmaxf(v[k][0], 0.f); v[k][1] = fmaxf(v[k][1], 0.f); v[k][2] = fmaxf(v[k][2], 0.f); v[k][3] = fmaxf(v[k][3], 0.f);
                    if (cb == 0) buf_st16(rs_y, (unsigned)lslot[k] >= (unsigned)kOwn ? goff[k] : kOOB, c0 * 4, v[k]);
                }
            }
        }
#pragma unroll
        for (int k = 0; k < NIT; ++k)
            if (lslot[k] >= 0) buf[FIN ? lslot[k] & (kOwn - 1) : lslot[k]] = v[k];
    };

    const int ra = wi == 0 ? 0 : (wi == 2 ? 2 : 1);
    const int rb = wi == 0 ? 2 : (wi == 1 ? 2 : (wi == 2 ? 1 : 3));
    const float sg = wi == 1 ? 1.f : -1.f;
    const int ty = li >> fwl, tx = li & (FW - 1);
    const int abase = g * plane + 2 * ty * pitch + tx;
    int abase_f;
    const int oa = ra * pitch, ob = rb * pitch;
    auto load_a = [&](const f32x4* buf, f32x4 (&a)[MT][4]) {
#pragma unroll
        for (int mt = 0; mt < MT; ++mt) {
            const f32x4* q = buf + mt * 4 * plane + abase_f;
            f32x4 R[4];
#pragma unroll
            for (int c = 0; c < 4; ++c) {
                const int oc = (c & 1) * half + (c >> 1);
                const f32x4 xa = q[oa + oc], xb = q[ob + oc];
                R[c] = xa + sg * xb;
            }
            a[mt][0] = R[0] - R[2];
            a[mt][1] = R[1] + R[2];
            a[mt][2] = R[2] - R[1];
            a[mt][3] = R[1] - R[3];
        }
    };

    const int cin4 = p.cin >> 2;
    const unsigned wlane = (unsigned)(n_base + li + g * p.cout_pad) * 16u;
    const int wp0 = wi * 4 * cin4 * p.cout_pad * 16;
    int wp;
    const int inc_j = cin4 * p.cout_pad * 16;
    const int inc_wrap = (4 - 3 * cin4) * p.cout_pad * 16;
    auto fetch_b = [&](f32x4 (&b)[NT]) {
#pragma unroll
        for (int nt = 0; nt < NT; ++nt)
            b[nt] = __builtin_bit_cast(f32x4, __builtin_amdgcn_raw_buffer_load_b128(rs_w, wlane + nt * 256u, (I2R_DBG(p) & 4) ? 0 : wp, 0));
    };

    f32x4 acc[4][MT][NT];
    const int npass = p.cin >> 4;
    const int bufsz = MT * 4 * plane;
    f32x4 a[MT][4], b0[NT], b1[NT];
#define WINO_MMA(J, B, FIRST)                                                                                   \
    if (!(I2R_DBG(p) & 16))                                                                                     \
    _Pragma("unroll") for (int s = 0; s < 4; ++s) _Pragma("unroll") for (int mt = 0; mt < MT; ++mt)             \
        _Pragma("unroll") for (int nt = 0; nt < NT; ++nt)                                                       \
            acc[J][mt][nt] = mfma16(a[mt][J][s], B[nt][s], ((FIRST) && s == 0) ? (f32x4){0.f, 0.f, 0.f, 0.f} : acc[J][mt][nt]);
#define WINO_PASS(PASS, FIRST)                                                                   \
    {                                                                                            \
        const int pass_ = (PASS);                                                                \
        f32x4* cur = lds + (pass_ & 1) * bufsz;                                                  \
        f32x4* nxt = lds + ((pass_ + 1) & 1) * bufsz;                                            \
        const bool more = pass_ + 1 < npass;                                                     \
        if (more) { stage_load((pass_ + 1) * 16); stage_load_t1((pass_ + 1) * 16); }             \
        load_a(cur, a);                                                                          \
        wp += inc_j; fetch_b(b1);                                                                \
        WINO_MMA(0, b0, FIRST)                                                                   \
        wp += inc_j; fetch_b(b0);                                                                \
        WINO_MMA(1, b1, FIRST)                                                                   \
        if (more) stage_mid((pass_ + 1) * 16);                                                   \
        wp += inc_j; fetch_b(b1);                                                                \
        WINO_MMA(2, b0, FIRST)                                                                   \
        if (more) { wp += inc_wrap; fetch_b(b0); }                                               \
        WINO_MMA(3, b1, FIRST)                                                                   \
        if (more) stage_store(nxt, (pass_ + 1) * 16);                                            \
        if (!(I2R_DBG(p) & 64)) __syncthreads();                                                 \
    }
    float* const Tl = reinterpret_cast<float*>(lds);
    constexpr int TW = NT * 16;
    constexpr int TPL = MT * 16 * TW;
    const bool tail = n_base + NT * 16 > p.cout || n_base + NT * 16 > p.out_cs;

    for (int fs = 0; fs < nrun; ++fs) {
    {
        const int tid_s = wi * 64 + lane_now();
        ConvKArg ps_ = args + gi;
        asm volatile("" : "+s"(ps_));
        set_fragment(run0 + fs, tid_s, *ps_);
        abase_f = abase;
        asm volatile("" : "+v"(abase_f));
#pragma unroll
        for (int k = 0; k < NIT; ++k) asm volatile("" : "+v"(lslot[k]));
    }
    wp = wp0;
    stage_load(0);
    stage_load_t1(0);
    if constexpr (FIN) {
        if (fin2) {
            f32x4 vu[NIT];
#pragma unroll
            for (int k = 0; k < NIT; ++k) vu[k] = buf_ld16(rs_t2, goff2[k], 0);
#pragma unroll
            for (int k = 0; k < NIT; ++k) {
                v[k] += vt[k];
                vt[k] = vu[k];
            }
        }
    }
    fetch_b(b0);
    if (fs) __syncthreads();
    stage_store(lds, 0);
    __syncthreads();
    if (stamp) ts1 = __builtin_amdgcn_s_memtime();
    WINO_PASS(0, true)
    for (int pass = 1; pass < npass; ++pass) WINO_PASS(pass, false)
    if (stamp) ts2 = __builtin_amdgcn_s_memtime();

    const int tid_f = wi * 64 + lane_now();
    ConvKArg pe_ = args + gi;
    asm volatile("" : "+s"(pe_));
    const auto& pe = *pe_;
    const float* const res2e = stamp ? nullptr : pe.res2;
    const unsigned out_bytes = pe.out_bytes;
    const __amdgpu_buffer_rsrc_t rs_out = make_rsrc(pe.out, out_bytes), rs_r1 = make_rsrc(pe.res1, out_bytes), rs_r2 = make_rsrc(res2e, out_bytes),
                                 rs_rp = make_rsrc(pe.res_post, out_bytes);
#pragma unroll
    for (int mt = 0; mt < MT; ++mt)
#pragma unroll
        for (int nt = 0; nt < NT; ++nt) {
            const f32x4 t0 = acc[0][mt][nt] + acc[1][mt][nt] + acc[2][mt][nt];
            const f32x4 t1 = acc[1][mt][nt] - acc[2][mt][nt] - acc[3][mt][nt];
            float* q = Tl + (wi * 2) * TPL + (mt * 16 + ((tid_f & 63) >> 4) * 4) * TW + nt * 16 + (tid_f & 15);
#pragma unroll
            for (int r = 0; r < 4; ++r) {
                q[r * TW] = t0[r];
                q[TPL + r * TW] = t1[r];
            }
        }
    unsigned obase[MT];
    const int q4 = tid_f & 3, px = tid_f >> 2;
    const bool hi = (px & 2) != 0;
    const int n0 = n_base + q4 * 4;
    f32x4 r[MT][NT];
#pragma unroll
    for (int mt = 0; mt < MT; ++mt) {
        const int t = px >> 2;
        const int oy = f_oy[mt] + 2 * (t >> fwl) + (hi ? 1 : 0);
        const int ox = f_ox[mt] + 2 * (t & (FW - 1)) + (px & 1);
        const bool ok = f_ok[mt] && oy < pe.conv_h && ox < pe.conv_w;
        obase[mt] = ok ? (unsigned)(((f_img[mt] * pe.out_h + oy) * pe.out_w + ox) * pe.out_cs + n0) * 4u : kOOB;
#pragma unroll
        for (int k = 0; k < NT; ++k) {
            r[mt][k] = *reinterpret_cast<const f32x4*>(pe.bias + n0 + 16 * k);
            if (!(I2R_DBG(p) & 1)) {
                if (pe.res1) r[mt][k] += buf_ld16(rs_r1, obase[mt] + 64u * k, 0);
                if (res2e) r[mt][k] += buf_ld16(rs_r2, obase[mt] + 64u * k, 0);
            }
        }
    }
    const float* const tq = Tl + ((px & 1) + (hi ? 2 : 0)) * TPL + (px >> 2) * TW + q4 * 4;
    const float sgn = hi ? -1.f : 1.f;
    __syncthreads();
#pragma unroll
    for (int mt = 0; mt < MT; ++mt)
#pragma unroll
        for (int k = 0; k < NT; ++k) {
            const float* q = tq + mt * 16 * TW + 16 * k;
            const f32x4 u0 = *reinterpret_cast<const f32x4*>(q);
            const f32x4 u1 = *reinterpret_cast<const f32x4*>(q + 2 * TPL);
            const f32x4 u2 = *reinterpret_cast<const f32x4*>(q + 4 * TPL);
            f32x4 y = u0 + sgn * (u1 + u2) + r[mt][k];
            if (pe.relu) { y[0] = fmaxf(y[0], 0.f); y[1] = fmaxf(y[1], 0.f); y[2] = fmaxf(y[2], 0.f); y[3] = fmaxf(y[3], 0.f); }
            unsigned off = obase[mt] + 64u * k;
            if (pe.res_post) y += buf_ld16(rs_rp, off, 0);
            if (tail) {
                const int n = n0 + 16 * k;
                if (!(n + 4 <= pe.cout || n + 4 <= pe.out_cs)) off = kOOB;
#pragma unroll
                for (int e = 0; e < 4; ++e)
                    if (n + e >= pe.cout) y[e] = 0.f;
            }
            if (!(I2R_DBG(p) & 1) || y[0] == 12345.678f) __builtin_amdgcn_raw_buffer_store_b128(__builtin_bit_cast(u32x4, y), rs_out, off, 0, 0);
        }
    }
#undef WINO_PASS
#undef WINO_MMA
    if (stamp) {
        asm volatile("s_waitcnt vmcnt(0)" ::: "memory");
        const unsigned long long ts3 = __builtin_amdgcn_s_memtime();
        if (tid == 0) {
            unsigned long long* o = reinterpret_cast<unsigned long long*>(const_cast<float*>(p.res2)) + (size_t)bid * 4;
            o[0] = ts0; o[1] = ts1; o[2] = ts2; o[3] = ts3;
        }
    }
}

__device__ __forceinline__ ConvKArg wino_args() {
    static_assert(offsetof(ConvGroupK, g) == 0, "the members lead the kernel argument");
    return (ConvKArg)__builtin_amdgcn_kernarg_segment_ptr();
}

template <int MT, int NT>
__global__ __launch_bounds__(256, (MT == 1 ? (NT == 3 ? 4 : 3) : 2)) void conv_wino_f32(const ConvGroupK grp) {
    conv_wino_body<MT, NT, false>(grp, wino_args());
}

template <int MT, int NT>
__global__ __launch_bounds__(256, (MT == 1 ? (NT == 3 ? 4 : 3) : 2)) void conv_wino_fin_f32(const ConvGroupK grp) {
    conv_wino_body<MT, NT, true>(grp, wino_args());
}

}

void* i2r_pick_conv_wino(int nt, int mt, int fin) {
    conv_fn fn = nullptr;
    if (mt == 1 && nt == 3) fn = fin ? conv_wino_fin_f32<1, 3> : conv_wino_f32<1, 3>;
    if (mt == 1 && nt == 4) fn = fin ? conv_wino_fin_f32<1, 4> : conv_wino_f32<1, 4>;
    return reinterpret_cast<void*>(fn);
}

size_t i2r_conv_wino_lds(int nt, int mt, int plane) {
    const size_t stage = (size_t)2 * mt * 4 * plane * 16;
    const size_t xchg = (size_t)4 * 2 * mt * 16 * nt * 16 * 4;
    return stage > xchg ? stage : xchg;
}
```

### intra-and-inter-human-relation-network-for-mpee_amd/engine.py

```python
import ctypes as C
import math
import os

import torch

from . import cabi
from .pack import (PRECISIONS, PackedConv, Packer, _m16, _r16, fold_bn, pack_frag, pack_frag32, pack_k4, pack_k8,
                   winograd_weights)


def wino_fragment(conv_h, conv_w):
    best = None
    for fw in (8, 4, 2):
        n = -(-conv_w // (2 * fw)) * -(-conv_h // (32 // fw))
        if best is None or n < best[0]:
            best = (n, 2 * fw, 32 // fw)
    return best[1], best[2]


LP1X1 = True
LP1X1_MAX_PIX = 65536
_HRT_FUSED_ATTN = (78, 156, 312)
_HRT_FUSED_MLP = (78, 156, 312)
_MLP_VARIANT = {78: 1, 156: 2, 312: 2}
PAIR1X1 = True
FUSE_IN = True
PRUNE_FUSE = True
WINOGRAD = True
WINO_SEQ = True
PROFILER_ATTACHED = bool(os.environ.get("ROCP_TOOL_LIBRARIES") or os.environ.get("ROCPROFILER_LIBRARY_CTOR") or os.environ.get("HSA_TOOLS_LIB")
                         or any(t in os.environ.get("LD_PRELOAD", "") for t in ("rocprof", "roctracer", "rocprofiler")))
DEVICE_SYNC = not PROFILER_ATTACHED


class Act:
    __slots__ = ("t", "n", "h", "w", "c", "cs", "dt")
    TORCH_DT = {0: torch.float32, 1: torch.bfloat16, 2: torch.float16}

    def __init__(self, t, n, h, w, c, cs, dt=0):
        self.t, self.n, self.h, self.w, self.c, self.cs, self.dt = t, n, h, w, c, cs, dt

    def view(self):
        return self.t.view(self.TORCH_DT[self.dt])[:self.n * self.h * self.w * self.cs].view(self.n, self.h, self.w, self.cs)

    @property
    def ptr(self):
        return self.t.data_ptr()


class _RawAct:
    __slots__ = ("ptr", "n", "h", "w", "c", "cs", "dt")

    def __init__(self, ptr, like, n=None):
        self.ptr, self.n, self.h, self.w, self.c, self.cs, self.dt = ptr, like.n if n is None else n, like.h, like.w, like.c, like.cs, 0


_MT_EFF = {1: 0.62, 2: 0.9, 3: 1.0, 4: 0.9}


def choose_tile(conv_h, conv_w, wm, stride, max_d, n_img, n_cblk, force_mt=0, want_cost=False):
    best = None
    cands_w = sorted({w for w in (conv_w, 48, 32, 24, 16, 12, 8, 6, 4) if w <= conv_w and w <= 48})
    for mt in ((force_mt,) if force_mt else (1, 2, 3, 4)):
        cap = wm * mt * 16
        for tw in cands_w:
            th = min(conv_h, cap // tw)
            if th < 1:
                continue
            ph, pw = (th - 1) * stride + max_d + 1, (tw - 1) * stride + max_d + 1
            if ph * pw > 1280:
                continue
            tiles = -(-conv_h // th) * -(-conv_w // tw)
            blocks = tiles * n_img * n_cblk
            rounds = -(-blocks // 256)
            halo = ph * pw / float(th * stride * tw * stride)
            cost = rounds * (cap / _MT_EFF[mt]) * (1.0 + 0.08 * (halo - 1.0))
            if best is None or cost < best[0] - 1e-9:
                best = (cost, th, tw, mt)
    assert best is not None, "no tile for %dx%d" % (conv_h, conv_w)
    if want_cost:
        return best
    return best[1], best[2], best[3]


_LPT_CACHE = {}
_LPT_DEV = {}


def lpt_block_table(device, counts, works):
    key = (str(device), tuple(counts), tuple(works))
    t = _LPT_DEV.get(key)
    if t is None:
        ck = (tuple(counts), tuple(works), 256)
        if ck not in _LPT_CACHE:
            _LPT_CACHE[ck] = lpt_block_order(counts, works)
        t = _LPT_DEV[key] = torch.tensor(_LPT_CACHE[ck], dtype=torch.int32, device=device)
    return t


def lpt_block_order(counts, works, n_cu=256):
    import heapq
    items = sorted(((w, g, i) for g, (c, w) in enumerate(zip(counts, works)) for i in range(c)),
                   key=lambda t: (-t[0], t[1], t[2]))
    heap = [(0, b) for b in range(n_cu)]
    bins = [[] for _ in range(n_cu)]
    for w, g, i in items:
        load, b = heapq.heappop(heap)
        bins[b].append((g << 24) | i)
        heapq.heappush(heap, (load + w, b))
    out, r = [], 0
    while len(out) < len(items):
        for b in range(n_cu):
            if r < len(bins[b]):
                out.append(bins[b][r])
        r += 1
    return out


def conv_split(cout_pad):
    nfrag = cout_pad // 16
    nt = next(c for c in (3, 4, 5) if nfrag % c == 0)
    nb = nfrag // nt
    wn = 4 if nb % 4 == 0 else 2 if nb % 2 == 0 else 1
    return nt, wn


class Program:
    def __init__(self, device):
        self.device = device
        self.ops = []
        self.keep = []
        self.pool = {}
        self.pending = []
        self.lane_pool = {}
        self.lane_ctx = 0
        self.groupings = []
        self.enc_stacks = []
        self.split_counters = []
        self.captures = []
        self.query = None
        self.store_dt = 0
        self.in_fork = False
        self.nbytes = 0
        self._snap = None
        self._next_slot = -1
        self._c_ops = None
        self._flags_op = None
        self.uses_lanes = False
        self.device_sync = False
        self._flags = None
        self._events = None
        self._tev = None
        self._capture_ws = None

    def alloc(self, n, h, w, c, dt=0):
        cs = _r16(c)
        numel = (n * h * w * cs + 1) // 2 if dt else n * h * w * cs
        lst = (self.lane_pool.get((self.lane_ctx, numel)) if self.in_fork else None) or self.pool.get(numel)
        if lst:
            t = lst.pop()
        else:
            t = torch.empty(numel, dtype=torch.float32, device=self.device)
            self.nbytes += numel * 4
            self.keep.append(t)
        return Act(t, n, h, w, c, cs, dt)

    def release(self, *acts):
        for a in acts:
            if a is None:
                continue
            if self.in_fork:
                self.lane_pool.setdefault((self.lane_ctx, a.t.numel()), []).append(a.t)
            else:
                self.pool.setdefault(a.t.numel(), []).append(a.t)

    def release_deferred(self, *acts):
        for a in acts:
            if self.in_fork:
                self.pending.append(a.t)
            else:
                self.pool.setdefault(a.t.numel(), []).append(a.t)

    def stem(self, st, n, h, w, in_ptr=0, lane=0, n_src=None, out_dt=0):
        out = self.alloc(n, (h - 1) // 2 + 1, (w - 1) // 2 + 1, st["cout"], out_dt)
        self.keep.append(st)
        ns = n if n_src is None else n_src
        a = cabi.StemArgs(in_ptr, st["w"].data_ptr(), st["bias"].data_ptr(), out.ptr, n, st["cin"], h, w, st["cout"], out.cs, ns, ns, out_dt)
        self.ops.append((cabi.OP_STEM, lane, a))
        return out, a

    def pe_res_stem(self, st, n, h, w, lane=0, n_src=None):
        out = self.alloc(n, (h - 1) // 2 + 1, (w - 1) // 2 + 1, st["cout"])
        self.keep.append(st)
        ns = n if n_src is None else n_src
        a = cabi.PeResArgs(0, st["w_pre"].data_ptr(), st["w7"].data_ptr(), st["bias"].data_ptr(), out.ptr, n, h, w, st["cout"], out.cs, ns, ns)
        self.ops.append((cabi.OP_PE_RES_STEM, lane, a))
        return out, a

    def conv(self, x, pc, relu=False, res1=None, res2=None, res_post=None, in2=None, up=1, out=None, out_step=1,
             out_off=(0, 0), out_hw=None, lane=0, group=None, act=None, out_dt=None, fuse_in=None):
        assert x.cs >= pc.cin_pad and x.c == pc.cin, "conv input channels %d/%d vs weight %d" % (x.c, x.cs, pc.cin)
        assert x.dt in (0, pc.dtype), "16-bit stored input needs the matching 16-bit conv (input %d, conv %d)" % (x.dt, pc.dtype)
        if (LP1X1 and pc.w_lp1 is not None and fuse_in is None and group is None and in2 is None and up == 1 and out_step == 1 and tuple(out_off) == (0, 0)
                and out_hw is None and x.n * x.h * x.w <= LP1X1_MAX_PIX and (out is None or (out.n, out.h, out.w) == (x.n, x.h, x.w))
                and (out is None or out.cs >= pc.cout_pad) and all(r is None or out is None or r.cs == out.cs for r in (res1, res2, res_post))
                and all(r is None or r.cs >= pc.cout_pad for r in (res1, res2, res_post))):
            return self.conv1x1_lp(x, pc, relu=relu, res1=res1, res2=res2, res_post=res_post, out=out, lane=lane, act=act, out_dt=out_dt)
        k = pc.ksize
        if pc.stride == 1:
            conv_h, conv_w = x.h, x.w
        else:
            conv_h, conv_w = (x.h - 1) // 2 + 1, (x.w - 1) // 2 + 1
        if up > 1:
            out_step = up
        if out is None:
            oh, ow = out_hw if out_hw else (conv_h * out_step, conv_w * out_step)
            out = self.alloc(x.n, oh, ow, pc.cout, x.dt if out_dt is None else out_dt)
        assert out.cs >= pc.cout_pad or out.cs >= pc.cout
        assert out.dt in (0, pc.dtype) and all(r is None or r.dt == out.dt for r in (res1, res2, res_post)), "residuals share the output's storage type"
        self._check_like(out, res1, res2, res_post)
        if in2 is not None and (in2.n, in2.h, in2.w, in2.cs) != (x.n, x.h, x.w, x.cs):
            raise ValueError("conv second input is [%d, %d, %d, cs %d], the first [%d, %d, %d, cs %d]" % (in2.n, in2.h, in2.w, in2.cs, x.n, x.h, x.w, x.cs))
        self.keep.append(pc)
        d = cabi.ConvDesc()
        d.in_, d.in2, d.w, d.bias = x.ptr, (in2.ptr if in2 is not None else None), pc.w.data_ptr(), pc.bias.data_ptr()
        d.res1 = res1.ptr if res1 is not None else None
        d.res2 = res2.ptr if res2 is not None else None
        d.res_post = res_post.ptr if res_post is not None else None
        d.out = out.ptr
        d.n_img, d.in_h, d.in_w, d.in_cs, d.cin = x.n, x.h, x.w, x.cs, pc.cin_pad
        d.conv_h, d.conv_w, d.out_h, d.out_w, d.out_cs = conv_h, conv_w, out.h, out.w, out.cs
        d.cout, d.cout_pad, d.stride, d.iy0, d.ix0 = pc.cout, pc.cout_pad, pc.stride, pc.iy0, pc.ix0
        d.ntaps = len(pc.taps)
        for i, (dy, dx) in enumerate(pc.taps):
            d.dy[i], d.dx[i] = dy, dx
        d.out_step, d.out_off_y, d.out_off_x, d.rep = out_step, out_off[0], out_off[1], up
        d.relu = int(relu) if act is None else act
        d.dtype = pc.dtype
        d.in_f16, d.out_f16 = int(x.dt != 0), int(out.dt != 0)
        wino = (WINOGRAD and pc.w_wino is not None and pc.dtype == 0 and in2 is None and up == 1 and out_step == 1 and tuple(out_off) == (0, 0)
                and (out.h, out.w) == (conv_h, conv_w) and d.relu in (0, 1))
        if fuse_in is not None:
            terms, y = fuse_in
            if not (wino and self.fuse_in_ok(x, terms, pc)):
                raise ValueError("fuse_in needs an fp32 Winograd conv over every channel of x and 1 or 2 terms at 1/2 or 1/4 of its map")
            assert all(t.cs == x.cs and t.dt == 0 and t.n == x.n for t in terms) and (y.n, y.h, y.w, y.cs, y.dt) == (x.n, x.h, x.w, x.cs, 0)
            sh = [{2: 1, 4: 2}[x.h // t.h] for t in terms]
            assert all((t.h << k, t.w << k) == (x.h, x.w) for t, k in zip(terms, sh))
            d.t1, d.t1_shift, d.y = terms[0].ptr, sh[0], y.ptr
            if len(terms) > 1:
                d.t2, d.t2_shift = terms[1].ptr, sh[1]
        if wino:
            nfrag = pc.cout_pad // 16
            nt = 3 if nfrag % 3 == 0 else 4
            fw, fh = wino_fragment(conv_h, conv_w)
            d.algo, d.w = 1, pc.w_wino.data_ptr()
            mt = 1
            d.tile_h, d.tile_w, d.mt, d.wn, d.ck = fh, fw, mt, 1, 0
            d.seq = 0 if WINO_SEQ else 1
            n_frag = x.n * -(-conv_h // fh) * -(-conv_w // fw)
            geo = ("wino", -(-n_frag // mt) * (nfrag // nt))
            key = ("wino", nt, mt)
        else:
            nt, wn = conv_split(pc.cout_pad)
            n_cblk = (pc.cout_pad // 16) // (nt * wn)
            max_d = max(max(t) for t in pc.taps)
            th, tw, mt = choose_tile(conv_h, conv_w, 4 // wn, pc.stride, max_d, x.n, n_cblk, force_mt=1 if pc.stride == 2 else 0)
            d.tile_h, d.tile_w, d.mt, d.wn, d.ck = th, tw, mt, wn, 0
            geo = (conv_h, conv_w, 4 // wn, pc.stride, max_d, x.n, n_cblk)
            key = nt
        if group is not None:
            group.append((d, geo, key))
        elif wino:
            self.flush_group([(d, geo, key)], lane=lane)
        else:
            self.ops.append((cabi.OP_CONV, lane, d))
        return out

    @staticmethod
    def fuse_in_ok(x, terms, pc):
        return (WINOGRAD and pc.w_wino is not None and pc.dtype == 0 and x.dt == 0 and x.c == pc.cin and x.cs == pc.cin_pad
                and 1 <= len(terms) <= 2 and all((t.h * 2, t.w * 2) == (x.h, x.w) or (t.h * 4, t.w * 4) == (x.h, x.w) for t in terms))

    @staticmethod
    def _group_tiles(group):
        best = None
        s2 = all(geo[3] == 2 for _, geo, _ in group)
        for mt in ((1,) if s2 else (2, 3, 4, 1)):
            try:
                tiles = [choose_tile(*geo, force_mt=mt, want_cost=True) for _, geo, _ in group]
            except AssertionError:
                continue
            blocks = 0
            work = 0.0
            for (d, geo, _), t in zip(group, tiles):
                conv_h, conv_w, wm, stride, max_d, n_img, n_cblk = geo
                nb = -(-conv_h // t[1]) * -(-conv_w // t[2]) * n_img * n_cblk
                blocks += nb
                work += nb * (wm * mt * 16 / _MT_EFF[mt]) * d.cin * d.ntaps
            cost = work * max(1.0, 256.0 / blocks)
            if best is None or cost < best[0]:
                best = (cost, mt, tiles)
        _, mt, tiles = best
        return mt, tiles

    def flush_group(self, group, lane=0):
        if not group:
            return
        nts = {g[2] for g in group}
        wino = group[0][0].algo == 1
        if (len(group) == 1 and not wino) or len(nts) != 1 or len(group) > cabi.MAX_GROUP:
            for m in list(group):
                if m[0].algo == 1:
                    self.flush_group([m], lane=lane)
                else:
                    self.ops.append((cabi.OP_CONV, lane, m[0]))
            del group[:]
            return
        if not wino:
            mt, tiles = self._group_tiles(group)
        order = sorted(range(len(group)), key=lambda i: -(group[i][0].cin * group[i][0].ntaps))
        a = cabi.ConvGroupArgs()
        counts, works = [], []
        for slot, i in enumerate(order):
            d, geo, _ = group[i]
            a.d[slot] = C.pointer(d)
            self.keep.append(d)
            if wino:
                counts.append(geo[1])
            else:
                d.tile_h, d.tile_w, d.mt = tiles[i][1], tiles[i][2], mt
                conv_h, conv_w, wm, stride, max_d, n_img, n_cblk = geo
                counts.append(-(-conv_h // d.tile_h) * -(-conv_w // d.tile_w) * n_img * n_cblk)
            works.append(d.cin * d.ntaps)
        a.n = len(group)
        if not wino and len(set(works)) > 1:
            bm = lpt_block_table(self.device, counts, works)
            self.keep.append(bm)
            a.block_map, a.map_len = bm.data_ptr(), bm.numel()
        self.ops.append((cabi.OP_CONV_GROUP, lane, a))
        del group[:]

    def channel_slice(self, a, c0, c):
        assert c0 % 16 == 0 and c0 + c <= a.cs
        words = c0 // 2 if a.dt else c0
        return Act(a.t[words:], a.n, a.h, a.w, c, a.cs, a.dt)

    def stem_conv2_layer1(self, a, conv2, blocks):
        first = blocks[0]
        assert "c3ds" in first, "layer1.0 carries the downsample"
        cx, cm = conv2.cout, first["c2"].cout
        cat = self.alloc(a.n, (a.h - 1) // 2 + 1, (a.w - 1) // 2 + 1, cx + cm, a.dt)
        x, t2 = self.channel_slice(cat, 0, cx), self.channel_slice(cat, cx, cm)
        self.conv(a, conv2, relu=True, out=x)
        self.release(a)
        t1 = self.conv(x, first["c1"], relu=True)
        self.conv(t1, first["c2"], relu=True, out=t2)
        def pair_ok(pa, pb):
            return (pa.w_frag is not None and pa.cin in (64, 128) and pa.cout % 32 == 0 and pa.cout == pa.cout_pad
                    and (pb is None or (pb.w_frag is not None and pb.cout == 64 and pb.cin == pa.cout)))
        nxt = [b["c1"] for b in blocks[1:]] + [None]
        if PAIR1X1 and a.dt == 0 and pair_ok(first["c3ds"], nxt[0]) and all(pair_ok(b["c3"], nxt[i]) for i, b in enumerate(blocks[1:], 1)):
            self.release(t1)
            y, t1 = self.conv1x1_pair(cat, first["c3ds"], None, blocks[1]["c1"] if len(blocks) > 1 else None)
            self.release(cat)
            for i, blk in enumerate(blocks[1:], 1):
                t2 = self.conv(t1, blk["c2"], relu=True)
                self.release(t1)
                yn, t1 = self.conv1x1_pair(t2, blk["c3"], y, blocks[i + 1]["c1"] if i + 1 < len(blocks) else None)
                self.release(t2, y)
                y = yn
            return y
        y = self.conv(cat, first["c3ds"], relu=True)
        self.release(t1, cat)
        x = y
        for blk in blocks[1:]:
            t1 = self.conv(x, blk["c1"], relu=True)
            t2 = self.conv(t1, blk["c2"], relu=True)
            y = self.conv(t2, blk["c3"], relu=True, res1=x)
            self.release(t1, t2, x)
            x = y
        return x

    def deconv(self, x, pcs, relu=True, res_post=None, lane=0):
        out = self.alloc(x.n, 2 * x.h, 2 * x.w, pcs[(0, 0)].cout, x.dt)
        grp = []
        for (py, px), pc in pcs.items():
            self.conv(x, pc, relu=relu, res_post=res_post, out=out, out_step=2, out_off=(py, px), lane=lane, group=grp)
        self.flush_group(grp, lane=lane)
        return out

    def rows_gather(self, src, crop_map, lane=0):
        out = self.alloc(len(crop_map), src.h, src.w, src.c)
        assert out.cs == src.cs, "rows_gather copies whole rows: source and output need the same row stride (%d vs %d)" % (src.cs, out.cs)
        m = torch.tensor(list(crop_map), dtype=torch.int32).to(self.device)
        self.keep.append(m)
        a = cabi.GatherArgs(src.ptr, out.ptr, m.data_ptr(), len(crop_map), src.h * src.w * src.cs)
        self.ops.append((cabi.OP_ROWS_GATHER, lane, a))
        return out

    def rows_gather_multi(self, segments, lane=0):
        assert 1 <= len(segments) <= cabi.MAX_GATHER_SEGS, "rows_gather_multi: %d segments (1..%d)" % (len(segments), cabi.MAX_GATHER_SEGS)
        a = cabi.GatherMultiArgs()
        a.n_seg = len(segments)
        for g, (src, out, table, n_out, n_src, src_crop, out_crop) in zip(a.seg, segments):
            row = src.h * src.w * src.cs * (2 if src.dt else 4)
            assert (out.h, out.w, out.cs, out.dt) == (src.h, src.w, src.cs, src.dt), "rows_gather_multi copies whole rows of one stride and type"
            assert row % 16 == 0 and table.dtype == torch.int32 and table.numel() >= n_out
            assert 0 <= out_crop and out_crop + n_out <= out.n and 0 <= src_crop and src_crop + n_src <= src.n
            self.keep.append(table)
            g.src, g.out, g.map = src.ptr + row * src_crop, out.ptr + row * out_crop, table.data_ptr()
            g.n_out, g.n_src, g.row_bytes = n_out, n_src, row
        self.ops.append((cabi.GROUPS_OP_ROWS_GATHER_MULTI, lane, a))
        return a

    def view_scramble(self, o, person_map, n_images, max_persons, c, lane=0):
        out = self.alloc(len(person_map), o.h, o.w, c)
        m = torch.tensor(list(person_map), dtype=torch.int32).to(self.device)
        self.keep.append(m)
        a = cabi.ScrambleArgs(o.ptr, out.ptr, m.data_ptr(), len(person_map), n_images, max_persons, c, out.cs, o.h * o.w)
        assert o.cs == out.cs and o.n == n_images * max_persons
        self.ops.append((cabi.OP_VIEW_SCRAMBLE, lane, a))
        return out

    def pe_cat_vec(self, fc, n, h, w, th, tw, out, c0, lane=0, n_src=None):
        rate = int(math.log(w // tw, 2))
        assert (out.n, out.h, out.w) == (n, th, tw) and out.dt == 0 and c0 + fc["vec"] <= out.cs
        self.keep.append(fc)
        ns = n if n_src is None else n_src
        a = cabi.PeCatVecArgs(0, fc["w"].data_ptr(), fc["b"].data_ptr(), out.ptr, n, h, w, th, tw, rate, fc["vec"], out.cs, c0, out.cs, ns, ns)
        self.ops.append((cabi.OP_PE_CAT_VEC, lane, a))
        return a

    def maxpool(self, x, lane=0, out=None):
        assert x.dt == 0, "fp32 kernel: the producer must store fp32 (conv(..., out_dt=0))"
        if out is None:
            out = self.alloc(x.n, (x.h - 1) // 2 + 1, (x.w - 1) // 2 + 1, x.c)
        assert (out.n, out.h, out.w) == (x.n, (x.h - 1) // 2 + 1, (x.w - 1) // 2 + 1) and out.cs >= x.cs and out.dt == 0
        a = cabi.PoolArgs(x.ptr, out.ptr, x.n, x.h, x.w, x.cs, x.cs, out.cs)
        self.ops.append((cabi.OP_MAXPOOL, lane, a))
        return out

    def layernorm(self, x, ln, eps=1e-6, lane=0, out_dt=0):
        assert x.dt == 0, "fp32 kernel: the producer must store fp32 (conv(..., out_dt=0))"
        out = self.alloc(x.n, x.h, x.w, x.c, out_dt)
        self.keep.append(ln)
        a = cabi.LnArgs(x.ptr, ln["w"].data_ptr(), ln["b"].data_ptr(), out.ptr, x.n * x.h * x.w, x.c, x.cs, eps, out_dt)
        self.ops.append((cabi.OP_LAYERNORM, lane, a))
        return out

    def winattn(self, qkv, bias, c, heads, lane=0):
        hs = heads * Packer.HEAD_PAD
        assert qkv.cs == 3 * hs, (qkv.cs, hs)
        out = self.alloc(qkv.n, qkv.h, qkv.w, hs)
        self.keep.append(bias)
        a = cabi.WinAttnArgs(qkv.ptr, bias.data_ptr(), out.ptr, qkv.n, qkv.h, qkv.w, c, hs, heads)
        self.ops.append((cabi.OP_WINATTN, lane, a))
        return out

    def hrt_attn(self, x, ab, eps=1e-6, lane=0, variant=None):
        assert x.dt == 0 and x.c == ab["c"] and x.cs == ab["cs"]
        if not variant or (variant == 1 and ab["c"] not in (78, 156)):
            variant = 2
        out = self.alloc(x.n, x.h, x.w, x.c)
        self.keep.append(ab)
        a = cabi.HrtAttnArgs(x.ptr, out.ptr, ab["ln"]["w"].data_ptr(), ab["ln"]["b"].data_ptr(), ab["wqkv"].data_ptr(), ab["bqkv"].data_ptr(),
                             ab["wo"].data_ptr(), ab["bo"].data_ptr(), x.n, x.h, x.w, x.c, x.cs, ab["heads"], eps, ab["dtype"], variant)
        self.ops.append((cabi.OP_HRT_ATTN, lane, a))
        return out

    def hrt_mlp(self, x, mb, eps=1e-6, lane=0, variant=None):
        assert x.dt == 0 and x.c == mb["c"] and x.cs == mb["cs"]
        if not variant or (variant == 1 and mb["c"] > 156):
            variant = _MLP_VARIANT[mb["c"]]
        out = self.alloc(x.n, x.h, x.w, x.c)
        self.keep.append(mb)
        a = cabi.HrtMlpArgs(x.ptr, out.ptr, mb["ln"]["w"].data_ptr(), mb["ln"]["b"].data_ptr(), mb["w1"].data_ptr(), mb["b1"].data_ptr(),
                            mb["wdw"].data_ptr(), mb["bdw"].data_ptr(), mb["w2"].data_ptr(), mb["b2"].data_ptr(), x.n, x.h, x.w, x.c, x.cs,
                            mb["hidden_pad"], eps, mb["dtype"], variant)
        self.ops.append((cabi.OP_HRT_MLP, lane, a))
        return out

    def dwconv(self, x, dw, stride=1, act=0, lane=0):
        assert x.dt == 0 or stride == 1
        assert x.c == dw["c"] and x.cs == dw["cs"]
        out = self.alloc(x.n, (x.h - 1) // stride + 1, (x.w - 1) // stride + 1, x.c, x.dt)
        self.keep.append(dw)
        a = cabi.DwArgs(x.ptr, dw["w"].data_ptr(), dw["bias"].data_ptr(), out.ptr, x.n, x.h, x.w, x.c, x.cs, stride, act, x.dt)
        self.ops.append((cabi.OP_DWCONV, lane, a))
        return out

    def upsample_add(self, low, res, out, act=0, lane=0):
        lows = list(low) if isinstance(low, (list, tuple)) else [low]
        assert 1 <= len(lows) <= 3
        sc = [out.h // t.h for t in lows]
        assert all(t.h * s == out.h and t.w * s == out.w and t.cs == out.cs == res.cs and t.n == out.n for t, s in zip(lows, sc))
        a = cabi.UpArgs(lows[0].ptr, res.ptr, out.ptr, lows[0].n, lows[0].h, lows[0].w, sc[0], lows[0].c, lows[0].cs, act,
                        lows[1].ptr if len(lows) > 1 else None, lows[2].ptr if len(lows) > 2 else None,
                        sc[1] if len(lows) > 1 else 1, sc[2] if len(lows) > 2 else 1)
        self.ops.append((cabi.OP_UPSAMPLE, lane, a))
        return out

    @staticmethod
    def _check_like(out, *residuals):
        for r in residuals:
            if r is not None and (r.n, r.h, r.w, r.cs) != (out.n, out.h, out.w, out.cs):
                raise ValueError("conv residual is [%d, %d, %d, row %d], the output [%d, %d, %d, row %d]" % (r.n, r.h, r.w, r.cs, out.n, out.h, out.w, out.cs))

    def conv1x1_lp(self, x, pc, relu=False, res1=None, res_post=None, out=None, lane=0, act=None, out_dt=None, res2=None):
        if out is None:
            out = self.alloc(x.n, x.h, x.w, pc.cout, x.dt if out_dt is None else out_dt)
        assert out.cs >= pc.cout_pad and out.dt in (0, pc.dtype) and all(r is None or (r.dt == out.dt and r.cs == out.cs) for r in (res1, res2, res_post))
        self._check_like(out, res1, res2, res_post)
        self.keep.append(pc)
        a = cabi.Conv1x1LpArgs(x.ptr, pc.w_lp1.data_ptr(), pc.bias.data_ptr(), res1.ptr if res1 is not None else None,
                               res_post.ptr if res_post is not None else None, out.ptr, x.n * x.h * x.w, pc.cin_pad, pc.cout_pad, x.cs, out.cs,
                               (int(relu) if act is None else act), pc.dtype, int(x.dt != 0), int(out.dt != 0), 0,
                               res2.ptr if res2 is not None else None)
        self.ops.append((cabi.OP_CONV1X1_LP, lane, a))
        return out

    def conv1x1_pair(self, x, pa, res, pb, lane=0):
        assert x.dt == 0 and pa.w_frag is not None and pa.ksize == 1 and pa.cin == x.cs and (pb is None or (pb.w_frag is not None and pb.cin == pa.cout))
        y = self.alloc(x.n, x.h, x.w, pa.cout)
        z = self.alloc(x.n, x.h, x.w, pb.cout) if pb is not None else None
        assert res is None or (res.cs == y.cs and res.dt == 0 and res.n * res.h * res.w == y.n * y.h * y.w)
        self.keep.extend([pa, pb])
        a = cabi.Conv1x1PairArgs(x.ptr, pa.w_frag.data_ptr(), pa.bias.data_ptr(), res.ptr if res is not None else None, y.ptr,
                                 pb.w_frag.data_ptr() if pb is not None else None, pb.bias.data_ptr() if pb is not None else None,
                                 z.ptr if z is not None else None, x.n * x.h * x.w, pa.cin, pa.cout, pb.cout if pb is not None else 0,
                                 x.cs, y.cs, z.cs if z is not None else 0, 1, 1, 0)
        self.ops.append((cabi.OP_CONV1X1_PAIR, lane, a))
        return y, z

    def fuse_up_add(self, base, terms, out, relu=True, lane=0):
        assert 1 <= len(terms) <= 2 and all(t.cs == base.cs == out.cs and t.dt == base.dt == out.dt and t.n == base.n for t in terms)
        sc = [base.h // t.h for t in terms]
        assert all(t.h * s == base.h and t.w * s == base.w for t, s in zip(terms, sc))
        a = cabi.FuseUpArgs(base.ptr, terms[0].ptr, terms[1].ptr if len(terms) > 1 else None, out.ptr, base.n, base.h, base.w, base.cs,
                            sc[0], sc[1] if len(terms) > 1 else 1, int(relu), base.dt)
        self.ops.append((cabi.OP_FUSE_UP, lane, a))
        return out

    def head(self, x, hd, out_ptr=0, lane=0):
        assert x.dt == 0, "fp32 kernel: the producer must store fp32 (conv(..., out_dt=0))"
        self.keep.append(hd)
        tmp = None
        if hd.get("conv3") is not None:
            x = tmp = self.conv(x, hd["conv3"], out_dt=0, lane=lane)
        a = cabi.HeadArgs(x.ptr, hd["w"].data_ptr(), hd["bias"].data_ptr(), out_ptr, x.n, x.h, x.w, hd["cin"], x.cs, hd["cout"])
        self.ops.append((cabi.OP_HEAD, lane, a))
        if tmp is not None:
            self.release(tmp)
        return a

    def encoder(self, x, layers, grp_off_host, pos=None, pos_period=0, lane=0, regroupable=False, pre_norm=False, pos_table=None, capture=None):
        assert x.dt == 0, "the encoder kernels read fp32 token rows"
        if layers and layers[0].get("mh"):
            return self.encoder_mh(x, layers, grp_off_host, pos=pos, pos_period=pos_period, lane=lane, regroupable=regroupable, pre_norm=pre_norm,
                                   pos_table=pos_table, capture=capture)
        assert not pre_norm, "the fused layer kernels are post-norm"
        cap = self._capture_begin(capture, x)
# ... 4 lines not shown
        fuse_kv = all(not L.get("dtype", 0) for L in layers) and len(layers) > 1
        nbuf = 2 if fuse_kv else 1
        kv_floats = max((n_tok // 16 + x.n + 1) * 16 * cs, (n_tok // 32 + x.n + 1) * 32 * 96 // 2)
        kbufs = [torch.zeros(kv_floats, dtype=torch.float32, device=self.device) for _ in range(nbuf)]
        vbufs = [torch.zeros(kv_floats, dtype=torch.float32, device=self.device) for _ in range(nbuf)]
        goff = torch.zeros(x.n + 1, dtype=torch.int32, device=self.device)
        split_ws = torch.empty(256 * 2 * 1792, dtype=torch.float32, device=self.device)
        split_cnt = torch.zeros(256, dtype=torch.int32, device=self.device)
        self.keep += kbufs + vbufs + [goff, split_ws, split_cnt]
        self.nbytes += sum(t.numel() * t.element_size() for t in kbufs + vbufs + [goff, split_ws, split_cnt])
        self.split_counters.append(split_cnt)
        cur = x
        self.keep.append(layers)
        descs = []
        for i, L in enumerate(layers):
            assert L["cs"] == cs
            if cap is not None and i in capture["layers"]:
                mh = capture["layers"][i]
                qk = self.conv(cur, mh["qk"], in2=pos_act, lane=lane)
                self._capture_layer(cap, i, qk, mh, goff, lane)
                self.release(qk)
            out = self.alloc(x.n, x.h, x.w, x.c)
            d = cabi.EncoderDesc()
            d.src, d.pos = cur.ptr, (pos if pos else None)
            d.kbuf, d.vbuf, d.out, d.grp_off = kbufs[i % nbuf].data_ptr(), vbufs[i % nbuf].data_ptr(), out.ptr, goff.data_ptr()
            for name in ("w_in", "b_in", "w_out", "b_out", "ln1_w", "ln1_b", "w1", "b1", "w2", "b2", "ln2_w", "ln2_b"):
                setattr(d, name, L[name].data_ptr())
            d.n_tok, d.d, d.cs, d.dff_pad = n_tok, L["d"], cs, L["dff_pad"]
            d.pos_period, d.ln_eps = pos_period, 1e-5
            d.split_ws, d.split_cnt = split_ws.data_ptr(), split_cnt.data_ptr()
            if L.get("dtype", 0):
                d.w_in_lp, d.w_out_lp, d.w1_lp, d.w2_lp, d.vec_lp = (L[k].data_ptr() for k in ("w_in_lp", "w_out_lp", "w1_lp", "w2_lp", "vec_lp"))
            if fuse_kv and i + 1 < len(layers):
                nxt = layers[i + 1]
                d.next_w_in, d.next_b_in = nxt["w_in"].data_ptr(), nxt["b_in"].data_ptr()
                d.next_kbuf, d.next_vbuf = kbufs[(i + 1) % nbuf].data_ptr(), vbufs[(i + 1) % nbuf].data_ptr()
            descs.append((d, L.get("dtype", 0)))
            if i == 0 or not fuse_kv:
                self.ops.append((cabi.OP_ENC_KV, lane, d))
            self.ops.append((cabi.OP_ENC_LAYER, lane, d))
            if cur is not x:
                self.release(cur)
            cur = out
        self._register_stack(dict(descs=descs, goff=goff, current=None), grp_off_host, cap, x.h * x.w if regroupable else None)
        return cur

    def encoder_mh(self, x, layers, grp_off_host, pos=None, pos_period=0, lane=0, regroupable=False, pre_norm=False, pos_table=None, capture=None):
        pos_act = self._pos_rows(x, pos, pos_period, pos_table)
        goff = torch.zeros(x.n + 1, dtype=torch.int32, device=self.device)
        self.keep += [goff, layers]
        self.nbytes += goff.numel() * 4
        cap = self._capture_begin(capture, x)
        cur, mh_args = x, []
        for i, L in enumerate(layers):
            assert L["cs"] == x.cs
            qk_in = self.layernorm(cur, L["ln1"], eps=1e-5, lane=lane) if pre_norm else cur
            qk = self.conv(qk_in, L["qk"], in2=pos_act, lane=lane)
            if cap is not None and i in capture["layers"]:
                self._capture_layer(cap, i, qk, L, goff, lane)
            v = self.conv(cur, L["v"], lane=lane)
            if pre_norm:
                self.release(qk_in)
            att = self.alloc(x.n, x.h, x.w, L["hs"])
            a = cabi.MhAttnArgs(qk.ptr, v.ptr, att.ptr, goff.data_ptr(), 0, L["heads"], L["hp"], L["hs"], qk.cs, v.cs, att.cs, 0, 0, 0)
            self.ops.append((cabi.OP_MH_ATTN, lane, a))
            mh_args.append(a)
            self.release(qk, v)
            x1 = self.conv(att, L["o"], res1=cur, lane=lane)
            self.release(att)
            if cur is not x:
                self.release(cur)
            if pre_norm:
                n2 = self.layernorm(x1, L["ln2"], eps=1e-5, lane=lane)
                hdn = self.conv(n2, L["w1"], relu=True, lane=lane)
                self.release(n2)
                cur = self.conv(hdn, L["w2"], res1=x1, lane=lane)
                self.release(hdn, x1)
            else:
                n1 = self.layernorm(x1, L["ln1"], eps=1e-5, lane=lane)
                self.release(x1)
                hdn = self.conv(n1, L["w1"], relu=True, lane=lane)
                y = self.conv(hdn, L["w2"], res1=n1, lane=lane)
                self.release(hdn, n1)
                cur = self.layernorm(y, L["ln2"], eps=1e-5, lane=lane)
                self.release(y)
        self._register_stack(dict(descs=[], mh=mh_args, goff=goff, current=None), grp_off_host, cap, x.h * x.w if regroupable else None)
        return cur

    def _register_stack(self, grouping, grp_off_host, cap=None, regroup_tok=None):
        self.set_groups(grouping, grp_off_host)
        if cap is not None:
            cap["grouping"] = grouping
        self.enc_stacks.append(grouping)
        if regroup_tok is not None:
            self.groupings.append((grouping, regroup_tok))

    def _pos_rows(self, x, pos, pos_period, pos_table):
        if not pos:
            return None
        if pos_period:
            assert x.h * x.w == pos_period and pos_table is not None and pos_table.data_ptr() == pos and tuple(pos_table.shape) == (pos_period, x.cs)
            rep = pos_table.unsqueeze(0).expand(x.n, pos_period, x.cs).contiguous()
            self.keep.append(rep)
            self.nbytes += rep.numel() * 4
            pos = rep.data_ptr()
        return _RawAct(pos, x)

    def _capture_begin(self, capture, x):
        if not capture:
            return None
        cap = dict(stack=capture["stack"], x=x, ops=[], out_off=torch.zeros(x.n, dtype=torch.int64, device=self.device))
        self.keep.append(cap["out_off"])
        self.captures.append(cap)
        return cap

    def _capture_layer(self, cap, i, qk, L, goff, lane):
        assert qk.dt == 0 and qk.cs >= 2 * L["hs"]
        self.keep.append(L)
        if self.query is not None:
            mode, scale = self.query[0], self.query[1][cap["stack"]]
            a = cabi.AttnQueryArgs(qk=qk.ptr, grp_off=goff.data_ptr(), out_off=cap["out_off"].data_ptr(), heads=L["heads"], hp=L["hp"], k_off=L["hs"],
                                   qk_cs=qk.cs, mode=mode, K=1, scale=scale, h=cap["x"].h, w=cap["x"].w)
            self.ops.append((cabi.CAPTURE_OP_ATTN_QUERY, lane, a))
            cap["ops"].append((i, a))
            return
        a = cabi.AttnWeightsArgs(qk.ptr, 0, goff.data_ptr(), cap["out_off"].data_ptr(), 0, 0, L["heads"], L["hp"], L["hs"], qk.cs, 0, 0)
        self.ops.append((cabi.CAPTURE_OP_ATTN_WEIGHTS, lane, a))
        cap["ops"].append((i, a))

    AW_KEYS = 128

    @staticmethod
    def _capture_groups(cap, lens):
        cur = cap["grouping"]["current"]
        assert len(lens) >= 1 and list(lens) == [cur[g + 1] - cur[g] for g in range(len(lens))]
        return max(a.heads for _, a in cap["ops"]) if cap["ops"] else 1

    @staticmethod
    def _capture_blocks(sizes):
        offs = [0]
        for n in sizes:
            offs.append(offs[-1] + n)
        return offs, -(-offs[-1] // 4) * 4

    @staticmethod
    def _upload_out_off(cap, offs):
        cap["out_off"][:len(offs) - 1].copy_(torch.tensor(offs[:-1], dtype=torch.int64).pin_memory(), non_blocking=True)

    def set_capture(self, glens):
        sizes, per_layer, need_ws, rows = [], [], 2, 0
        for cap, lens in zip(self.captures, glens):
            heads = self._capture_groups(cap, lens)
            need_ws = max(need_ws, 2 * heads * -(-max(lens) // self.AW_KEYS))
            rows = max(rows, sum(lens))
            offs, n_layer = self._capture_blocks([n * n for n in lens])
            sizes.append(offs)
            per_layer.append(n_layer)
        total = sum(n * len(cap["ops"]) for n, cap in zip(per_layer, self.captures))
        buf = torch.empty(max(total, 1), dtype=torch.float32, device=self.device)
        ws = torch.empty(rows * need_ws, dtype=torch.float32, device=self.device)
        self._capture_ws = ws
        maps, base = {}, 0
        for cap, lens, offs, n_layer in zip(self.captures, glens, sizes, per_layer):
            self._upload_out_off(cap, offs)
            tiles = sum(-(-n // 16) * -(-n // self.AW_KEYS) for n in lens)
            for i, a in cap["ops"]:
                a.out, a.ws = buf.data_ptr() + 4 * base, ws.data_ptr()
                a.n_grp, a.n_tiles, a.ws_stride = len(lens), tiles, need_ws
                maps[(cap["stack"], i)] = [buf[base + o:base + o + n * n].view(n, n) for o, n in zip(offs, lens)]
                base += n_layer
        return buf, maps, {cap["stack"]: cap["x"] for cap in self.captures}

    def set_query_capture(self, glens, queries):
        mode, scales = self.query
        plan, per_layer, n_ws, n_rows = [], [], 2, 1
        for cap, lens in zip(self.captures, glens):
            scale = scales[cap["stack"]]
            heads = self._capture_groups(cap, lens)
            tok = torch.as_tensor(queries.tokens[cap["stack"]]).to("cpu", torch.int32).contiguous()
            if tok.dim() != 2 or tok.shape[0] != len(lens) or tok.shape[1] < 1:
                raise ValueError("query tokens of %r: shape %s, expected [%d groups, K]" % (cap["stack"], tuple(tok.shape), len(lens)))
            K = tok.shape[1]
            cnt = getattr(queries, "counts", None)
            cnt = [int(c) for c in cnt[cap["stack"]]] if cnt and cnt.get(cap["stack"]) is not None else [K] * len(lens)
            if len(cnt) != len(lens) or not all(1 <= c <= K for c in cnt):
                raise ValueError("query counts of %r: %s for %d groups of up to %d entries" % (cap["stack"], cnt, len(lens), K))
            for g, (n, c) in enumerate(zip(lens, cnt)):
                if int(tok[g, :c].max()) >= n:
                    raise ValueError("query token %d of group %d of %r is outside its %d tokens" % (int(tok[g, :c].max()), g, cap["stack"], n))
            hw = cap["x"].h * cap["x"].w
            assert all(n % hw == 0 for n in lens)
            stride = 2 * heads * -(-max(lens) // self.AW_KEYS)
            n_ws = max(n_ws, stride * (len(lens) * K if mode == 0 else sum(lens)))
            if scale > 1:
                n_rows = max(n_rows, K * sum(lens))
            offs, n_layer = self._capture_blocks([c * n * scale * scale for n, c in zip(lens, cnt)])
            plan.append((tok, cnt, K, stride, offs, scale))
            per_layer.append(n_layer)
        starts, base = [], 0
        for n, cap in zip(per_layer, self.captures):
            starts.append([base + j * n for j in range(len(cap["ops"]))])
            base += n * len(cap["ops"])
        total = max((st[-1] + p[4][-1] for st, p in zip(starts, plan) if st), default=1)
        buf = torch.empty(total, dtype=torch.float32, device=self.device)
        ws = torch.empty(n_ws, dtype=torch.float32, device=self.device)
        rows = torch.empty(n_rows, dtype=torch.float32, device=self.device)
        held = [ws, rows]
        maps = {}
        for cap, lens, (tok, cnt, K, stride, offs, scale), st in zip(self.captures, glens, plan, starts):
            self._upload_out_off(cap, offs)
            d_tok = tok.pin_memory().to(self.device, non_blocking=True)
            d_cnt = torch.tensor(cnt, dtype=torch.int32).pin_memory().to(self.device, non_blocking=True)
            cur = cap["grouping"]["current"]
            host_off = (C.c_int32 * (len(lens) + 1))(*cur[:len(lens) + 1])
            held += [d_tok, d_cnt, host_off]
            h, w = cap["x"].h, cap["x"].w
            if mode == 0:
                tiles, col_tiles = sum(-(-c // 16) * -(-n // self.AW_KEYS) for n, c in zip(lens, cnt)), 0
            else:
                tiles = sum(-(-n // 16) * -(-n // self.AW_KEYS) for n in lens)
                col_tiles = sum(-(-n // 16) * -(-c // 16) for n, c in zip(lens, cnt))
            for (i, a), b0 in zip(cap["ops"], st):
                a.out, a.ws, a.rows = buf.data_ptr() + 4 * b0, ws.data_ptr(), rows.data_ptr()
                a.q_tok, a.q_cnt, a.grp_off_host = d_tok.data_ptr(), d_cnt.data_ptr(), C.cast(host_off, C.c_void_p)
                a.n_grp, a.n_tiles, a.n_col_tiles, a.ws_stride, a.K = len(lens), tiles, col_tiles, stride, K
                maps[(cap["stack"], i)] = [buf[b0 + o:b0 + o + c * n * scale * scale].view(c, n // (h * w), h * scale, w * scale)
                                           for o, n, c in zip(offs, lens, cnt)]
        self._capture_ws = held
        return buf, maps, {cap["stack"]: cap["x"] for cap in self.captures}

    def set_groups(self, grouping, grp_off_host):
        offs = tuple(int(o) for o in grp_off_host)
        if grouping["current"] == offs:
            return
        assert len(offs) <= grouping["goff"].numel()
        lens = [offs[i + 1] - offs[i] for i in range(len(offs) - 1)]
        assert all(l > 0 for l in lens)
        nq, nq16, nq64, nq192 = (sum(-(-l // t) for l in lens) for t in (32, 16, 64, 192))
        grouping["goff"][:len(offs)].copy_(torch.tensor(offs, dtype=torch.int32).pin_memory(), non_blocking=True)
        for d, dt in grouping["descs"]:
            d.n_grp, d.n_qtiles32, d.n_qtiles16, d.n_qtiles64 = len(offs) - 1, nq, nq16, nq64
            d.n_qtiles192 = nq192
            d.dtype = dt
        for a in grouping.get("mh", ()):
            a.n_grp, a.n_qtiles16, a.n_qtiles32, a.n_qtiles64 = len(offs) - 1, nq16, nq, nq64
        grouping["current"] = offs

    def fork(self, mask):
        if not any(k == cabi.OP_LANE_FLAGS for k, _, _ in self.ops):
            self.ops.append((cabi.OP_LANE_FLAGS, 0, None))
        self.ops.append((cabi.OP_FORK, mask, None))
        self.in_fork = True

    def _flush_lane_pools(self):
        for t in self.pending:
            self.pool.setdefault(t.numel(), []).append(t)
        self.pending = []
        for (_, numel), lst in self.lane_pool.items():
            self.pool.setdefault(numel, []).extend(lst)
        self.lane_pool = {}

    def records(self, lanes):
        assert self.in_fork and self._snap is None
        slots, region = {}, 0
        for l in lanes:
            region |= 1 << l
        for l in lanes:
            slot = self._next_slot = (self._next_slot + 1) % 8
            self.ops.append((cabi.OP_RECORD, l | slot << 8 | region << 16, None))
            slots[l] = slot
        self._snap = (self.pending, self.lane_pool)
        self.pending, self.lane_pool = [], {}
        return slots

    def wait(self, lane, slot):
        self.ops.append((cabi.OP_WAIT, lane | slot << 8, None))

    def all_waited(self):
        pend, lp = self._snap
        self._snap = None
        for t in pend:
            self.pool.setdefault(t.numel(), []).append(t)
        for (_, numel), lst in lp.items():
            self.pool.setdefault(numel, []).extend(lst)

    def join(self, mask):
        assert self._snap is None
        self.ops.append((cabi.OP_JOIN, mask, None))
        self.in_fork = False
        self._flush_lane_pools()
        self.lane_ctx = 0

    def finalize(self):
        arr = (cabi.Op * len(self.ops))()
        for i, (kind, lane, st) in enumerate(self.ops):
            arr[i].kind, arr[i].lane = kind, lane
            arr[i].args = C.cast(C.pointer(st), C.c_void_p) if st is not None else None
        self._c_ops = arr
        self._flags_op = next((i for i, (kind, _, _) in enumerate(self.ops) if kind == cabi.OP_LANE_FLAGS), None)
        self.uses_lanes = any(lane != 0 or kind in cabi.SYNC_OPS for kind, lane, _ in self.ops)

    def run(self, side_streams=None, events=None):
        L = cabi.lib()
        cur = torch.cuda.current_stream(self.device).cuda_stream
        if side_streams is None:
            streams = (C.c_void_p * 4)(cur, cur, cur, cur)
        else:
            streams = (C.c_void_p * 4)(cur, *[s.cuda_stream for s in side_streams])
        evs = None
        if self._flags_op is not None:
            spin = side_streams is not None and DEVICE_SYNC and lanes_independent(self.device, side_streams, cur)
            self._c_ops[self._flags_op].args = self._lane_flags().data_ptr() if spin else None
            self.device_sync = spin
        if self.uses_lanes:
            if events is None:
                events = self._own_events()
            evs = (C.c_void_p * len(events))(*[e.cuda_event for e in events])
        try:
            if Program.timing_log is not None:
                self._run_timed(L, streams, evs)
            else:
                cabi.check(L.i2r_run_program(self._c_ops, len(self.ops), streams, evs), "i2r_run_program")
        except Exception:
            for t in self.split_counters:
                t.zero_()
            raise

    timing_log = None
    timing_markers = True

    def _run_timed(self, L, streams, evs):
        n = len(self.ops)
        key = (tuple(streams), Program.timing_markers)
        if self._tev is None or self._tev[0] != key:
            t0, t1, seen = [None] * n, [None] * n, set()
            for i, (kind, lane, st) in enumerate(self.ops):
                if kind in cabi.SYNC_OPS:
                    continue
                t1[i] = torch.cuda.Event(enable_timing=True)
                t1[i].record()
                if Program.timing_markers or streams[lane] not in seen:
                    seen.add(streams[lane])
                    t0[i] = torch.cuda.Event(enable_timing=True)
                    t0[i].record()
            torch.cuda.synchronize(self.device)
            self._tev = (key, t0, t1, (C.c_void_p * n)(*[e.cuda_event if e is not None else None for e in t0]),
                         (C.c_void_p * n)(*[e.cuda_event if e is not None else None for e in t1]))
        _, t0, t1, a0, a1 = self._tev
        cabi.check(L.i2r_run_program_timed(self._c_ops, n, streams, evs, a0, a1), "i2r_run_program_timed")
        Program.timing_log.append((self, t0, t1, key[0]))

    def _lane_flags(self):
        if self._flags is None:
            self._flags = torch.zeros(64, dtype=torch.int32, device=self.device)
        return self._flags

    def sync_timed_out(self):
        return self._flags is not None and bool(self._flags[63].item())

    def _own_events(self):
        if self._events is None:
            self._events = [torch.cuda.Event(enable_timing=False) for _ in range(16)]
            for e in self._events:
                e.record()
        return self._events


class _PendingFuse:
    __slots__ = ("base", "terms")

    def __init__(self, base, terms):
        self.base, self.terms = base, terms


class HRNetW48:

    def __init__(self, pk, p, extra):
        self.extra = extra
        s2, s3 = extra["STAGE2"], extra["STAGE3"]
        self.stride = 4 * 2 ** (s3["NUM_BRANCHES"] - 1)
        self.stem1 = pk.stem(p + "conv1", p + "bn1")
        self.conv2 = pk.conv(p + "conv2", p + "bn2", stride=2)
        self.layer1 = pk.bottlenecks(p + "layer1", 4)
        self.t1 = [pk.conv(p + "transition1.0.0", p + "transition1.0.1"),
                   pk.conv(p + "transition1.1.0.0", p + "transition1.1.0.1", stride=2)]
        self.stage2 = [self._module(pk, "%sstage2.%d" % (p, m), s2) for m in range(s2["NUM_MODULES"])]
        self.t2 = pk.conv(p + "transition2.2.0.0", p + "transition2.2.0.1", stride=2)
        self.stage3 = [self._module(pk, "%sstage3.%d" % (p, m), s3) for m in range(s3["NUM_MODULES"])]

    @staticmethod
    def _module(pk, q, st):
        nb = st["NUM_BRANCHES"]
        mod = dict(nb=nb, blocks=[], fuse={})
        for i in range(nb):
            mod["blocks"].append([(pk.conv("%s.branches.%d.%d.conv1" % (q, i, b), "%s.branches.%d.%d.bn1" % (q, i, b)),
                                   pk.conv("%s.branches.%d.%d.conv2" % (q, i, b), "%s.branches.%d.%d.bn2" % (q, i, b)))
                                  for b in range(st["NUM_BLOCKS"][i])])
        for i in range(nb):
            for j in range(nb):
                if j > i:
                    mod["fuse"][(i, j)] = pk.conv("%s.fuse_layers.%d.%d.0" % (q, i, j), "%s.fuse_layers.%d.%d.1" % (q, i, j))
                elif j < i:
                    mod["fuse"][(i, j)] = [pk.conv("%s.fuse_layers.%d.%d.%d.0" % (q, i, j, k),
                                                   "%s.fuse_layers.%d.%d.%d.1" % (q, i, j, k), stride=2)
                                           for k in range(i - j)]
        return mod

    @staticmethod
    def _close(P, x):
        if not isinstance(x, _PendingFuse):
            return x
        y = P.alloc(x.base.n, x.base.h, x.base.w, x.base.c, x.base.dt)
        P.fuse_up_add(x.base, x.terms, y, relu=True)
        P.release(x.base, *x.terms)
        return y

    @staticmethod
    def _emit_module(P, mod, xs, need=None, defer=None):
        nb = mod["nb"]
        xs = list(xs)
        need = set(range(nb)) if need is None else {i % nb for i in need}
        for k in range(max(len(b) for b in mod["blocks"])):
            grp, ts, folded = [], {}, []
            for i in range(nb):
                if k < len(mod["blocks"][i]):
                    if isinstance(xs[i], _PendingFuse):
                        pf = xs[i]
                        xs[i] = P.alloc(pf.base.n, pf.base.h, pf.base.w, pf.base.c, pf.base.dt)
                        ts[i] = P.conv(pf.base, mod["blocks"][i][k][0], relu=True, group=grp, fuse_in=(pf.terms, xs[i]))
                        folded.append(pf)
                        continue
                    ts[i] = P.conv(xs[i], mod["blocks"][i][k][0], relu=True, group=grp)
            P.flush_group(grp)
            for pf in folded:
                P.release(pf.base, *pf.terms)
            for i, t in ts.items():
                y = P.conv(t, mod["blocks"][i][k][1], relu=True, res1=xs[i], group=grp)
                P.release(t, xs[i])
                xs[i] = y
            P.flush_group(grp)
        xs = [HRNetW48._close(P, x) for x in xs]
        terms, ups = [], []
        for i in range(nb):
            ts = []
            for j in range(i if i in need else 0):
                chain = mod["fuse"][(i, j)]
                ts.append(dict(j=j, mids=list(chain[:-1]), last=chain[-1], cur=None))
            ts.sort(key=lambda t: (len(t["mids"]), t["j"]))
            terms.append(ts)
            ups.append([(j, mod["fuse"][(i, j)]) for j in range(i + 1, nb)] if i in need else [])
        n_up = sum(len(u) for u in ups)
        ys = [None] * nb
        n_sum = [0] * nb
        tmaps = [[] for _ in range(nb)]
        levels_left = max([1 + len(t["mids"]) for ts in terms for t in ts] + [1 if n_up else 0])
        while levels_left > 0:
            levels_left -= 1
            grp, rel = [], []
            for i in range(nb):
                ready = [t for t in terms[i] if not t["mids"]]
                for t in terms[i]:
                    if t["mids"]:
                        src = t["cur"] if t["cur"] is not None else xs[t["j"]]
                        nxt = P.conv(src, t["mids"].pop(0), relu=True, group=grp)
                        if t["cur"] is not None:
                            rel.append(t["cur"])
                        t["cur"] = nxt
                if ready:
                    t = ready[0]
                    terms[i].remove(t)
                    src = t["cur"] if t["cur"] is not None else xs[t["j"]]
                    if ys[i] is None:
                        ys[i] = P.alloc(xs[i].n, xs[i].h, xs[i].w, xs[i].c, xs[i].dt)
                    P.conv(src, t["last"], relu=(not terms[i] and not ups[i]), res1=xs[i] if n_sum[i] == 0 else ys[i], out=ys[i], group=grp)
                    n_sum[i] += 1
                    if t["cur"] is not None:
                        rel.append(t["cur"])
            if levels_left == 0 and n_up:
                cands = [(i, j, pc) for i in range(nb) for j, pc in ups[i]]
                if len(grp) + len(cands) > cabi.MAX_GROUP:
                    P.flush_group(grp)
                for i, j, pc in cands:
                    tmaps[i].append(P.conv(xs[j], pc, group=grp))
                    if len(grp) == cabi.MAX_GROUP:
                        P.flush_group(grp)
            P.flush_group(grp)
            P.release(*rel)
        assert not any(terms)
        kept = []
        for i in range(nb):
            if not tmaps[i]:
                continue
            base = xs[i] if ys[i] is None else ys[i]
            if FUSE_IN and defer is not None and defer[i] is not None and P.fuse_in_ok(base, tmaps[i], defer[i]):
                if ys[i] is None:
                    kept.append(xs[i])
                ys[i] = _PendingFuse(base, list(tmaps[i]))
                continue
            if ys[i] is None:
                ys[i] = P.alloc(xs[i].n, xs[i].h, xs[i].w, xs[i].c, xs[i].dt)
            pend = list(tmaps[i])
            while pend:
                now, pend = pend[:2], pend[2:]
                P.fuse_up_add(base, now, ys[i], relu=not pend)
                base = ys[i]
            P.release(*tmaps[i])
        P.release(*[x for x in xs if not any(x is k for k in kept)])
        return ys

    def emit(self, P, n, h, w, n_src=None, need=None):
        a, stem_args = P.stem(self.stem1, n, h, w, n_src=n_src, out_dt=P.store_dt)
        x = P.stem_conv2_layer1(a, self.conv2, self.layer1)
        grp = []
        xs = [P.conv(x, self.t1[0], relu=True, group=grp), P.conv(x, self.t1[1], relu=True, group=grp)]
        P.flush_group(grp)
        P.release(x)
        if not PRUNE_FUSE:
            need = None
        mods = list(self.stage2) + list(self.stage3)
        def first_convs(m, nb):
            nxt = mods[m + 1]["blocks"] if m + 1 < len(mods) else []
            return [nxt[i][0][0] if i < len(nxt) and nxt[i] else None for i in range(nb)]
        for m, mod in enumerate(self.stage2):
            xs = self._emit_module(P, mod, xs, defer=first_convs(m, mod["nb"]))
        xs[-1] = self._close(P, xs[-1])
        t = P.conv(xs[-1], self.t2, relu=True)
        xs = [xs[0], xs[1], t]
        for m, mod in enumerate(self.stage3, len(self.stage2)):
            last = m + 1 == len(mods)
            xs = self._emit_module(P, mod, xs, need=need if last else None, defer=None if last else first_convs(m, mod["nb"]))
        return xs, stem_args


class HRFormerB:

    def __init__(self, pk, p):
        from .arch_hrformer import STAGES
        b = p + "backbone."
        self.stem1 = pk.stem(b + "conv1", b + "bn1")
        self.conv2 = pk.conv(b + "conv2", b + "bn2", stride=2)
        self.layer1 = pk.bottlenecks(b + "layer1", 2)
        self.stages = []
        pre = [256]
        for sname, tname in (("stage2", "transition1"), ("stage3", "transition2"), ("stage4", "transition3")):
            st = STAGES[sname]
            ch = st["num_channels"]
            trans = []
            for i in range(st["num_branches"]):
                if i < len(pre):
                    trans.append(pk.conv("%s%s.%d.0" % (b, tname, i), "%s%s.%d.1" % (b, tname, i)) if ch[i] != pre[i] else None)
                else:
                    trans.append(pk.conv("%s%s.%d.0.0" % (b, tname, i), "%s%s.%d.0.1" % (b, tname, i), stride=2))
            mods = []
            for m in range(st["num_modules"]):
                multiscale = not (sname == "stage4" and m == st["num_modules"] - 1)
                mods.append(self._module(pk, "%s%s.%d" % (b, sname, m), st, multiscale))
            self.stages.append(dict(trans=trans, mods=mods, n_pre=len(pre)))
            pre = list(ch)

    @staticmethod
    def _module(pk, q, st, multiscale):
        nb, ch = st["num_branches"], st["num_channels"]
        mod = dict(nb=nb, n_out=nb if multiscale else 1, blocks=[], fuse={})
        for i in range(nb):
            blks = []
            for k in range(st["num_blocks"][i]):
                r = "%s.branches.%d.%d" % (q, i, k)
                fused = pk.attn_block_lp(r, ch[i], st["num_heads"][i]) if (pk.dtype != 0 and ch[i] in _HRT_FUSED_ATTN) else None
                fused_mlp = pk.mlp_block_lp(r, ch[i]) if (pk.dtype != 0 and ch[i] in _HRT_FUSED_MLP) else None
                blks.append(dict(c=ch[i], heads=st["num_heads"][i], ln1=pk.ln(r + ".norm1", ch[i]), ln2=pk.ln(r + ".norm2", ch[i]), attn_lp=fused, mlp_lp=fused_mlp,
                                 qkv=pk.qkv(r + ".attn.attn", ch[i], st["num_heads"][i]),
                                 out=pk.attn_out(r + ".attn.attn", ch[i], st["num_heads"][i]),
                                 fc1=pk.conv(r + ".mlp.fc1", r + ".mlp.norm1"), dw=pk.dw(r + ".mlp.dw3x3", r + ".mlp.norm2"),
                                 fc2=pk.conv(r + ".mlp.fc2", r + ".mlp.norm3")))
            mod["blocks"].append(blks)
        for i in range(mod["n_out"]):
            for j in range(nb):
                r = "%s.fuse_layers.%d.%d" % (q, i, j)
                if j > i:
                    mod["fuse"][(i, j)] = pk.conv(r + ".0", r + ".1")
                elif j < i:
                    mod["fuse"][(i, j)] = [(pk.dw("%s.%d.0" % (r, k), "%s.%d.1" % (r, k)), pk.conv("%s.%d.2" % (r, k), "%s.%d.3" % (r, k)))
                                           for k in range(i - j)]
        return mod

    @staticmethod
    def _emit_block(P, blk, x, lane=0):
        P.lane_ctx = lane
        if blk.get("attn_lp") is not None:
            x1 = P.hrt_attn(x, blk["attn_lp"], lane=lane)
            P.release(x)
        else:
            n1 = P.layernorm(x, blk["ln1"], lane=lane, out_dt=P.store_dt)
            qkv = P.conv(n1, blk["qkv"], lane=lane, out_dt=0)
            P.release(n1)
            a = P.winattn(qkv, blk["qkv"].bias, blk["c"], blk["heads"], lane=lane)
            P.release(qkv)
            x1 = P.conv(a, blk["out"], res1=x, lane=lane)
            P.release(a, x)
        if blk.get("mlp_lp") is not None:
            x2 = P.hrt_mlp(x1, blk["mlp_lp"], lane=lane)
            P.release(x1)
            return x2
        n2 = P.layernorm(x1, blk["ln2"], lane=lane, out_dt=P.store_dt)
        h1 = P.conv(n2, blk["fc1"], act=2, lane=lane)
        P.release(n2)
# ... 1113 lines not shown
```

Baseline: 8776 images/sec.

## Add specialized Winograd epilogue forms for plain ReLU and residual-ReLU convs

Adds templated Winograd conv kernel variants (EPI=1 bias+ReLU, EPI=2 bias+residual+ReLU) with a streamlined output-transform epilogue and a host-side selector that picks them when the conv group qualifies. Kernel parameters move into a precomputed Wino sub-struct with reciprocal-based divisions and hoisted weight-offset increments, cutting per-thread integer work in indexing. The aim is to shorten the generic epilogue and the fragment-index arithmetic. In exchange there are more kernel instantiations and a larger kernarg struct. The path can be toggled through a global flag.

```diff
diff --git a/include/i2r_hip.h b/include/i2r_hip.h
--- a/include/i2r_hip.h
+++ b/include/i2r_hip.h
@@ -82,6 +82,9 @@
 
 I2R_API int i2r_conv_grid(const i2r_conv_desc* const* descs, int32_t n, int32_t with_map, int32_t* grid, int32_t* seq);
 
+I2R_API int i2r_conv_wino_form(const i2r_conv_desc* const* descs, int32_t n, int32_t* form);
+I2R_API int i2r_conv_wino_forms(int32_t on);
+
 I2R_API int i2r_flip_merge(const float* y, const float* y_flipped, const int32_t* joint_map, float* out, int32_t n, int32_t joints,
                    int32_t h, int32_t w, void* stream);
 
diff --git a/intra-and-inter-human-relation-network-for-mpee_amd/cabi.py b/intra-and-inter-human-relation-network-for-mpee_amd/cabi.py
--- a/intra-and-inter-human-relation-network-for-mpee_amd/cabi.py
+++ b/intra-and-inter-human-relation-network-for-mpee_amd/cabi.py
@@ -233,7 +233,7 @@
     _fields_ = [("kind", _i32), ("lane", _i32), ("args", C.c_void_p)]
 
 
-EXPORTS = ("i2r_conv", "i2r_conv_grouped", "i2r_conv_kernel_name", "i2r_conv_grid", "i2r_stem_conv", "i2r_pe_res_stem", "i2r_maxpool3x3s2", "i2r_head", "i2r_layernorm", "i2r_window_attn", "i2r_hrt_attn_block", "i2r_hrt_mlp_block", "i2r_dwconv3x3",
+EXPORTS = ("i2r_conv", "i2r_conv_grouped", "i2r_conv_kernel_name", "i2r_conv_grid", "i2r_conv_wino_form", "i2r_conv_wino_forms", "i2r_stem_conv", "i2r_pe_res_stem", "i2r_maxpool3x3s2", "i2r_head", "i2r_layernorm", "i2r_window_attn", "i2r_hrt_attn_block", "i2r_hrt_mlp_block", "i2r_dwconv3x3",
            "i2r_upsample_bilinear_add", "i2r_upsample_bilinear_add_multi", "i2r_fuse_up_add", "i2r_conv1x1_pair", "i2r_conv1x1_lp", "i2r_flip_merge", "i2r_decode", "i2r_pose_nms", "i2r_group_nearest", "i2r_oks_match", "i2r_oks_accumulate", "i2r_joint_targets", "i2r_val_metrics", "i2r_val_combine", "i2r_crop_affine", "i2r_box_mask", "i2r_crop_affine_cv2", "i2r_box_mask_cv2", "i2r_person_inputs_cv2", "i2r_encoder_kv", "i2r_encoder_layer", "i2r_mh_attention", "i2r_attn_weights", "i2r_attn_query_maps", "i2r_pe_cat_vec", "i2r_rows_gather", "i2r_rows_gather_multi", "i2r_view_scramble",
            "i2r_run_program", "i2r_run_program_timed", "i2r_abi_version", "i2r_last_error", "i2r_device_check")
 
@@ -254,6 +254,8 @@
     L.i2r_conv_grouped.argtypes = [C.POINTER(C.POINTER(ConvDesc)), _i32, _fp, _i32, C.c_void_p]
     L.i2r_conv_kernel_name.argtypes = [C.POINTER(C.POINTER(ConvDesc)), _i32, C.c_char_p, _i32]
     L.i2r_conv_grid.argtypes = [C.POINTER(C.POINTER(ConvDesc)), _i32, _i32, C.POINTER(_i32), C.POINTER(_i32)]
+    L.i2r_conv_wino_form.argtypes = [C.POINTER(C.POINTER(ConvDesc)), _i32, C.POINTER(_i32)]
+    L.i2r_conv_wino_forms.argtypes = [_i32]
     L.i2r_stem_conv.argtypes = [_fp, _fp, _fp, _fp, _i32, _i32, _i32, _i32, _i32, _i32, _i32, _i32, _i32, C.c_void_p]
     L.i2r_pe_res_stem.argtypes = [_fp, _fp, _fp, _fp, _fp, _i32, _i32, _i32, _i32, _i32, _i32, _i32, C.c_void_p]
     L.i2r_flip_merge.argtypes = [_fp, _fp, _fp, _fp, _i32, _i32, _i32, _i32, C.c_void_p]
diff --git a/intra-and-inter-human-relation-network-for-mpee_amd/csrc/i2r_conv.h b/intra-and-inter-human-relation-network-for-mpee_amd/csrc/i2r_conv.h
--- a/intra-and-inter-human-relation-network-for-mpee_amd/csrc/i2r_conv.h
+++ b/intra-and-inter-human-relation-network-for-mpee_amd/csrc/i2r_conv.h
@@ -42,9 +42,34 @@
     float* f_y;
     int f_sh1, f_sh2;
     unsigned f_bytes1, f_bytes2;
+    struct Wino {
+        float* out;
+        const float* res1;
+        const float* bias;
+        unsigned out_bytes, bias_bytes;
+        int conv_h, conv_w, out_cs, pad_;
+        int frags_img, tiles_x;
+        unsigned r_img, r_tx;
+        int in_h, in_w, in_cs;
+        int pw, pp, w_rcp;
+        int oy_step;
+        int f_sh1, f_sh2;
+        int nfrag;
+        int w_row, w_inc_j, w_inc_wrap;
+        int npass, bufsz;
+        int nruns;
+        int n_cblk, w_seq, w_band;
+        unsigned r_cblk;
+        int fwlog, pitch, half, plane, cout_pad, ph;
+        unsigned in_bytes, w_bytes;
+        const float* in;
+        const float* w;
+    } wk;
 };
 
 __device__ __forceinline__ int div_m(int n, int d, unsigned m) { return d == 1 ? n : (int)__umulhi((unsigned)n, m); }
+
+__device__ __forceinline__ int div_r(int n, unsigned r) { return (int)__umulhi((unsigned)n << 1, r); }
 
 typedef unsigned u32x4 __attribute__((ext_vector_type(4)));
 typedef unsigned u32x2 __attribute__((ext_vector_type(2)));
@@ -252,5 +277,5 @@
 
 void* i2r_pick_conv_bf16(int nt, int mt, int cap, int pf);
 void* i2r_pick_conv_f16(int nt, int mt, int cap, int pf);
-void* i2r_pick_conv_wino(int nt, int mt, int fin);
+void* i2r_pick_conv_wino(int nt, int mt, int fin, int epi);
 size_t i2r_conv_wino_lds(int nt, int mt, int plane);
diff --git a/intra-and-inter-human-relation-network-for-mpee_amd/csrc/i2r_conv.hip b/intra-and-inter-human-relation-network-for-mpee_amd/csrc/i2r_conv.hip
--- a/intra-and-inter-human-relation-network-for-mpee_amd/csrc/i2r_conv.hip
+++ b/intra-and-inter-human-relation-network-for-mpee_amd/csrc/i2r_conv.hip
@@ -1,6 +1,7 @@
 #include <stdlib.h>
 
 #include <algorithm>
+#include <atomic>
 
 #include "i2r_conv.h"
 
@@ -275,6 +276,7 @@
     k.m_cblk = k.m_tx = k.m_ty = k.m_pw = k.m_tw = 0; k.wn_log = 0; k.npass = 0;
     k.dbg = 0;
     k.f_t1 = d->t1; k.f_t2 = d->t2; k.f_y = d->y; k.f_sh1 = d->t1_shift; k.f_sh2 = d->t2 ? d->t2_shift : 0; k.f_bytes1 = k.f_bytes2 = 0;
+    k.wk = ConvK::Wino{};
 }
 
 constexpr int kWinoMaxSeq = 8;
@@ -343,7 +345,7 @@
     k.tap_kw = k.tap_kh = 3;
     k.ck = 16; k.wn = 1;
     const long long nf = (long long)d->n_img * k.tiles_y * k.tiles_x;
-    I2R_CHECK_ARG(nf > 0 && nf * k.n_cblk < (1ll << 20) && k.tiles_y * k.tiles_x < 2048 && k.n_cblk < 2048, "i2r_conv: algo 1 grid (%lld fragments)", nf);
+    I2R_CHECK_ARG(nf > 0 && (nf + 8) * k.n_cblk < (1ll << 20) && k.tiles_y * k.tiles_x < 2048 && k.n_cblk < 2048, "i2r_conv: algo 1 grid (%lld fragments)", nf);
     k.w_nfrag = (int)nf;
     k.w_seq = d->seq ? d->seq : 1;
 #ifdef I2R_TUNING
@@ -352,6 +354,28 @@
         k.dbg = dbg;
     }
 #endif
+    auto recip31 = [](int d) { return (unsigned)(((1ull << 31) + d - 1) / d); };
+    {
+        ConvK::Wino& wk = k.wk;
+        wk.out = k.out; wk.res1 = k.res1; wk.bias = k.bias;
+        wk.out_bytes = k.out_bytes; wk.bias_bytes = (unsigned)d->cout_pad * 4; wk.conv_h = k.conv_h; wk.conv_w = k.conv_w; wk.out_cs = k.out_cs;
+        wk.frags_img = k.tiles_y * k.tiles_x; wk.tiles_x = k.tiles_x; wk.r_img = recip31(wk.frags_img); wk.r_tx = recip31(k.tiles_x);
+        wk.in_h = k.in_h; wk.in_w = k.in_w; wk.in_cs = k.in_cs;
+        wk.pw = k.pw; wk.pp = k.ph * k.pw; wk.w_rcp = k.w_rcp;
+        wk.oy_step = k.tile_h;
+        wk.f_sh1 = k.f_sh1; wk.f_sh2 = k.f_sh2;
+        wk.nfrag = k.w_nfrag;
+        const int cin4 = d->cin / 4;
+        wk.w_row = 4 * cin4 * d->cout_pad * 16;
+        wk.w_inc_j = cin4 * d->cout_pad * 16;
+        wk.w_inc_wrap = (4 - 3 * cin4) * d->cout_pad * 16;
+        wk.npass = d->cin / 16;
+        wk.bufsz = mt * 4 * k.plane;
+        wk.nruns = (k.w_nfrag + mt - 1) / mt;
+        wk.n_cblk = k.n_cblk; wk.r_cblk = recip31(k.n_cblk); wk.w_seq = k.w_seq;
+        wk.fwlog = k.w_fwlog; wk.pitch = k.w_pitch; wk.half = k.w_half; wk.plane = k.plane; wk.cout_pad = k.cout_pad; wk.ph = k.ph;
+        wk.in_bytes = k.in_bytes; wk.w_bytes = k.w_bytes; wk.in = k.in; wk.w = k.w;
+    }
     *nt_out = nt; *mt_out = mt; *cap_out = 0; *pf_out = 100;
     *lds_out = i2r_conv_wino_lds(nt, mt, k.plane);
     *nblk_out = wino_runs(k, mt) * k.n_cblk;
@@ -578,6 +602,7 @@
             }
             total += nblk;
             grp.blk_end[i] = (int)total;
+            grp.g[i].wk.w_seq = grp.g[i].w_seq; grp.g[i].wk.w_band = grp.g[i].w_band;
         }
     }
     for (int i = n; i < kMaxGroups; ++i) { grp.g[i] = grp.g[0]; grp.blk_end[i] = (int)total; }
@@ -591,6 +616,36 @@
     for (int i = 0; i < n; ++i)
         if (descs[i]->t1) return true;
     return false;
+}
+
+static std::atomic<int> g_wino_forms{1};
+
+static int wino_form(const i2r_conv_desc* const* descs, int32_t n, const ConvGroupK& grp) {
+    if (!g_wino_forms.load(std::memory_order_relaxed)) return 0;
+    for (int i = 0; i < n; ++i) {
+        const i2r_conv_desc* d = descs[i];
+        if (d->relu != 1 || d->res2 || d->res_post || d->cout != d->cout_pad || d->cout_pad > d->out_cs) return 0;
+        if ((d->res1 != nullptr) != (descs[0]->res1 != nullptr)) return 0;
+        if (I2R_DBG(grp.g[i]) != 0) return 0;
+    }
+    return descs[0]->res1 ? 2 : 1;
+}
+
+extern "C" int i2r_conv_wino_forms(int32_t on) {
+    g_wino_forms.store(on ? 1 : 0, std::memory_order_relaxed);
+    return I2R_OK;
+}
+
+extern "C" int i2r_conv_wino_form(const i2r_conv_desc* const* descs, int32_t n, int32_t* form) {
+    ConvGroupK grp;
+    int nt0, mt0, cap0, pf0;
+    size_t lds_max;
+    long long total;
+    int rc = resolve(descs, n, grp, &nt0, &mt0, &cap0, &pf0, &lds_max, &total);
+    if (rc) return rc;
+    I2R_CHECK_ARG(form != nullptr, "i2r_conv_wino_form: form");
+    *form = descs[0]->algo == 1 ? wino_form(descs, n, grp) : 0;
+    return I2R_OK;
 }
 
 extern "C" int i2r_conv_grouped(const i2r_conv_desc* const* descs, int32_t n, const int32_t* block_map,
@@ -603,7 +658,7 @@
     if (rc) return rc;
     grp.blk_map = block_map;
     I2R_CHECK_ARG(block_map == nullptr || map_len == (int32_t)total, "i2r_conv_grouped: block_map has %d entries, grid has %lld", map_len, total);
-    conv_fn fn = descs[0]->algo == 1 ? reinterpret_cast<conv_fn>(i2r_pick_conv_wino(nt0, mt0, any_fused_input(descs, n)))
+    conv_fn fn = descs[0]->algo == 1 ? reinterpret_cast<conv_fn>(i2r_pick_conv_wino(nt0, mt0, any_fused_input(descs, n), wino_form(descs, n, grp)))
                  : descs[0]->dtype == 0 ? pick_kernel(nt0, mt0, cap0, pf0)
                                       : reinterpret_cast<conv_fn>(descs[0]->dtype == 1 ? i2r_pick_conv_bf16(nt0, mt0, cap0, pf0) : i2r_pick_conv_f16(nt0, mt0, cap0, pf0));
     I2R_CHECK_ARG(fn != nullptr, "i2r_conv: no kernel for nt=%d mt=%d cap=%d pf=%d dtype=%d", nt0, mt0, cap0, pf0, descs[0]->dtype);
diff --git a/intra-and-inter-human-relation-network-for-mpee_amd/csrc/i2r_conv_wino.hip b/intra-and-inter-human-relation-network-for-mpee_amd/csrc/i2r_conv_wino.hip
--- a/intra-and-inter-human-relation-network-for-mpee_amd/csrc/i2r_conv_wino.hip
+++ b/intra-and-inter-human-relation-network-for-mpee_amd/csrc/i2r_conv_wino.hip
@@ -6,7 +6,7 @@
 
 typedef const ConvK __attribute__((address_space(4)))* ConvKArg;
 
-template <int MT, int NT, bool FIN>
+template <int MT, int NT, bool FIN, int EPI>
 __device__ __forceinline__ void conv_wino_body(const ConvGroupK& grp, ConvKArg args) {
     extern __shared__ __attribute__((aligned(16))) f32x4 lds[];
     const int tid = threadIdx.x, lane = tid & 63;
@@ -30,35 +30,32 @@
     unsigned long long ts0 = 0, ts1 = 0, ts2 = 0;
     if (stamp) ts0 = __builtin_amdgcn_s_memtime();
 
-    int wg, cb;
-    if (grp.blk_map) {
-        wg = div_m(bid, p.n_cblk, p.w_m_cblk);
-        cb = bid - wg * p.n_cblk;
-    } else {
-        const int q = bid >> 3, qq = div_m(q, p.n_cblk, p.w_m_cblk);
-        cb = q - qq * p.n_cblk;
-        wg = (bid & 7) * p.w_band + qq;
-    }
-    const int run0 = wg * p.w_seq;
-    const int nrun = min(p.w_seq, (p.w_nfrag + MT - 1) / MT - run0);
+    const auto& pk = p.wk;
+    const int n_cblk = pk.n_cblk;
+    const int bq = grp.blk_map ? bid : bid >> 3;
+    const int qq = div_r(bq, pk.r_cblk);
+    const int cb = bq - qq * n_cblk;
+    const int wg = grp.blk_map ? qq : (bid & 7) * pk.w_band + qq;
+    const int run0 = wg * pk.w_seq;
+    const int nrun = min(pk.w_seq, pk.nruns - run0);
     if (nrun <= 0) return;
-    const int fwl = p.w_fwlog, FW = 1 << fwl;
-    const int pitch = p.w_pitch, half = p.w_half, plane = p.plane;
+    const int fwl = pk.fwlog, FW = 1 << fwl;
+    const int pitch = pk.pitch, half = pk.half, plane = pk.plane;
     const int n_base = cb * NT * 16;
 
     constexpr int NIT = (MT * kWinoPatchMax * 4 + 255) / 256;
-    const __amdgpu_buffer_rsrc_t rs_in = __builtin_amdgcn_make_buffer_rsrc(const_cast<float*>(p.in), 0, p.in_bytes, 0x00020000);
-    const __amdgpu_buffer_rsrc_t rs_w = __builtin_amdgcn_make_buffer_rsrc(const_cast<float*>(p.w), 0, p.w_bytes, 0x00020000);
+    const __amdgpu_buffer_rsrc_t rs_in = __builtin_amdgcn_make_buffer_rsrc(const_cast<float*>(pk.in), 0, pk.in_bytes, 0x00020000);
+    const __amdgpu_buffer_rsrc_t rs_w = __builtin_amdgcn_make_buffer_rsrc(const_cast<float*>(pk.w), 0, pk.w_bytes, 0x00020000);
     unsigned goff[NIT];
     int lslot[NIT];
     constexpr int kOwn = 1 << 30;
     const bool fin = FIN && p.f_t1 != nullptr, fin2 = fin && p.f_t2 != nullptr;
     const __amdgpu_buffer_rsrc_t rs_t1 = make_rsrc(fin ? p.f_t1 : nullptr, p.f_bytes1), rs_t2 = make_rsrc(fin2 ? p.f_t2 : nullptr, p.f_bytes2),
-                                 rs_y = make_rsrc(fin ? p.f_y : nullptr, p.in_bytes);
+                                 rs_y = make_rsrc(fin ? p.f_y : nullptr, pk.in_bytes);
     unsigned goff1[FIN ? NIT : 1], goff2[FIN ? NIT : 1];
     const int cg = tid & 3;
     auto patch_pixel = [&](const auto& pq, int t, int k, int& f, int& row, int& col) {
-        const int PC = pq.pw, PP = pq.ph * pq.pw;
+        const int PC = pq.pw, PP = pq.pp;
         const int pix = (t + k * 256) >> 2;
         int pp = pix;
         f = 0;
@@ -71,10 +68,11 @@
 #pragma unroll
     for (int k = 0; k < NIT; ++k) {
         int f, row, col;
-        patch_pixel(p, tid, k, f, row, col);
+        patch_pixel(pk, tid, k, f, row, col);
+        asm volatile("" : "+v"(row), "+v"(col));
         lslot[k] = f < MT ? (f * 4 + cg) * plane + row * pitch + (col & 1) * half + (col >> 1) : -1;
         if constexpr (FIN) {
-            if (f < MT && row >= 1 && row < p.ph - 1 && col >= 1 && col < p.pw - 1) lslot[k] |= kOwn;
+            if (f < MT && row >= 1 && row < pk.ph - 1 && col >= 1 && col < pk.pw - 1) lslot[k] |= kOwn;
         }
     }
     auto lane_now = []() {
@@ -88,12 +86,12 @@
 #pragma unroll
         for (int mt = 0; mt < MT; ++mt) {
             int fid = fg * MT + mt;
-            f_ok[mt] = fid < ps.w_nfrag;
+            f_ok[mt] = MT == 1 || fid < ps.nfrag;
             if (!f_ok[mt]) fid = 0;
-            f_img[mt] = div_m(fid, (ps.tiles_y * ps.tiles_x), ps.w_m_img);
-            const int rem = fid - f_img[mt] * (ps.tiles_y * ps.tiles_x);
-            const int fy = div_m(rem, ps.tiles_x, ps.w_m_tx);
-            f_oy[mt] = fy * (32 >> fwl);
+            f_img[mt] = div_r(fid, ps.r_img);
+            const int rem = fid - f_img[mt] * ps.frags_img;
+            const int fy = div_r(rem, ps.r_tx);
+            f_oy[mt] = fy * ps.oy_step;
             f_ox[mt] = (rem - fy * ps.tiles_x) * (2 * FW);
         }
 #pragma unroll
@@ -183,12 +181,11 @@
         }
     };
 
-    const int cin4 = p.cin >> 2;
-    const unsigned wlane = (unsigned)(n_base + li + g * p.cout_pad) * 16u;
-    const int wp0 = wi * 4 * cin4 * p.cout_pad * 16;
+    const unsigned wlane = (unsigned)(n_base + li + g * pk.cout_pad) * 16u;
+    const int wp0 = wi * pk.w_row;
     int wp;
-    const int inc_j = cin4 * p.cout_pad * 16;
-    const int inc_wrap = (4 - 3 * cin4) * p.cout_pad * 16;
+    const int inc_j = pk.w_inc_j;
+    const int inc_wrap = pk.w_inc_wrap;
     auto fetch_b = [&](f32x4 (&b)[NT]) {
 #pragma unroll
         for (int nt = 0; nt < NT; ++nt)
@@ -196,8 +193,8 @@
     };
 
     f32x4 acc[4][MT][NT];
-    const int npass = p.cin >> 4;
-    const int bufsz = MT * 4 * plane;
+    const int npass = pk.npass;
+    const int bufsz = pk.bufsz;
     f32x4 a[MT][4], b0[NT], b1[NT];
 #define WINO_MMA(J, B, FIRST)                                                                                   \
     if (!(I2R_DBG(p) & 16))                                                                                     \
@@ -234,9 +231,14 @@
         const int tid_s = wi * 64 + lane_now();
         ConvKArg ps_ = args + gi;
         asm volatile("" : "+s"(ps_));
-        set_fragment(run0 + fs, tid_s, *ps_);
-        abase_f = abase;
-        asm volatile("" : "+v"(abase_f));
+        set_fragment(run0 + fs, tid_s, ps_->wk);
+        if constexpr (FIN) {
+            const int l = tid_s & 63;
+            abase_f = (l >> 4) * plane + 2 * ((l & 15) >> fwl) * pitch + (l & (FW - 1));
+        } else {
+            abase_f = abase;
+            asm volatile("" : "+v"(abase_f));
+        }
 #pragma unroll
         for (int k = 0; k < NIT; ++k) asm volatile("" : "+v"(lslot[k]));
     }
@@ -264,6 +266,69 @@
     for (int pass = 1; pass < npass; ++pass) WINO_PASS(pass, false)
     if (stamp) ts2 = __builtin_amdgcn_s_memtime();
 
+    if constexpr (EPI != 0) {
+    const int tid_f = wi * 64 + lane_now();
+    ConvKArg pe_ = args + gi;
+    asm volatile("" : "+s"(pe_));
+    const auto& we = pe_->wk;
+    const int conv_h = we.conv_h, conv_w = we.conv_w, out_cs = we.out_cs;
+    const __amdgpu_buffer_rsrc_t rs_out = __builtin_amdgcn_make_buffer_rsrc(we.out, 0, we.out_bytes, 0x00020000),
+                                 rs_bias = __builtin_amdgcn_make_buffer_rsrc(const_cast<float*>(we.bias), 0, we.bias_bytes, 0x00020000);
+    const int q4 = tid_f & 3, px = tid_f >> 2;
+    const bool hi = (px & 2) != 0;
+    const int n0 = n_base + q4 * 4;
+    float neg1_ = -1.f;
+    asm volatile("" : "+s"(neg1_));
+    const f32x4 neg1 = {neg1_, neg1_, neg1_, neg1_};
+    unsigned obase[MT];
+    f32x4 bs[NT], rr[EPI == 2 ? MT : 1][NT];
+#pragma unroll
+    for (int mt = 0; mt < MT; ++mt) {
+        const int t = px >> 2;
+        const int oy = f_oy[mt] + 2 * (t >> fwl) + (hi ? 1 : 0);
+        const int ox = f_ox[mt] + 2 * (t & (FW - 1)) + (px & 1);
+        const bool ok = (int)f_ok[mt] & (int)(oy < conv_h) & (int)(ox < conv_w);
+        obase[mt] = ok ? (unsigned)(((f_img[mt] * conv_h + oy) * conv_w + ox) * out_cs + n0) * 4u : kOOB;
+        if constexpr (EPI == 2) {
+            const __amdgpu_buffer_rsrc_t rs_r1 = __builtin_amdgcn_make_buffer_rsrc(const_cast<float*>(we.res1), 0, we.out_bytes, 0x00020000);
+#pragma unroll
+            for (int k = 0; k < NT; ++k) rr[mt][k] = buf_ld16(rs_r1, obase[mt] + 64u * k, 0);
+        }
+    }
+#pragma unroll
+    for (int mt = 0; mt < MT; ++mt)
+#pragma unroll
+        for (int nt = 0; nt < NT; ++nt) {
+            f32x4 t0 = acc[0][mt][nt] + acc[1][mt][nt] + acc[2][mt][nt];
+            f32x4 t1 = __builtin_elementwise_fma(acc[3][mt][nt], neg1, __builtin_elementwise_fma(acc[2][mt][nt], neg1, acc[1][mt][nt]));
+            asm volatile("" : "+v"(t0), "+v"(t1));
+            float* q = Tl + (wi * 2) * TPL + (mt * 16 + ((tid_f & 63) >> 4) * 4) * TW + nt * 16 + (tid_f & 15);
+#pragma unroll
+            for (int r = 0; r < 4; ++r) {
+                q[r * TW] = t0[r];
+                q[TPL + r * TW] = t1[r];
+            }
+        }
+#pragma unroll
+    for (int k = 0; k < NT; ++k) bs[k] = buf_ld16(rs_bias, (unsigned)n0 * 4u + 64u * k, 0);
+    const float* const tq = Tl + ((px & 1) + (hi ? 2 : 0)) * TPL + (px >> 2) * TW + q4 * 4;
+    const float sgn = hi ? -1.f : 1.f;
+    __syncthreads();
+#pragma unroll
+    for (int mt = 0; mt < MT; ++mt)
+#pragma unroll
+        for (int k = 0; k < NT; ++k) {
+            const float* q = tq + mt * 16 * TW + 16 * k;
+            const f32x4 u0 = *reinterpret_cast<const f32x4*>(q);
+            const f32x4 u1 = *reinterpret_cast<const f32x4*>(q + 2 * TPL);
+            const f32x4 u2 = *reinterpret_cast<const f32x4*>(q + 4 * TPL);
+            f32x4 r = bs[k];
+            if constexpr (EPI == 2) r += rr[mt][k];
+            f32x4 y = u0 + sgn * (u1 + u2) + r;
+            y[0] = fmaxf(y[0], 0.f); y[1] = fmaxf(y[1], 0.f); y[2] = fmaxf(y[2], 0.f); y[3] = fmaxf(y[3], 0.f);
+            __builtin_amdgcn_raw_buffer_store_b128(__builtin_bit_cast(u32x4, y), rs_out, obase[mt] + 64u * k, 0, 0);
+        }
+    } else {
     const int tid_f = wi * 64 + lane_now();
     ConvKArg pe_ = args + gi;
     asm volatile("" : "+s"(pe_));
@@ -331,6 +396,7 @@
             if (!(I2R_DBG(p) & 1) || y[0] == 12345.678f) __builtin_amdgcn_raw_buffer_store_b128(__builtin_bit_cast(u32x4, y), rs_out, off, 0, 0);
         }
     }
+    }
 #undef WINO_PASS
 #undef WINO_MMA
     if (stamp) {
@@ -348,22 +414,36 @@
     return (ConvKArg)__builtin_amdgcn_kernarg_segment_ptr();
 }
 
-template <int MT, int NT>
+template <int MT, int NT, int EPI>
 __global__ __launch_bounds__(256, (MT == 1 ? (NT == 3 ? 4 : 3) : 2)) void conv_wino_f32(const ConvGroupK grp) {
-    conv_wino_body<MT, NT, false>(grp, wino_args());
-}
-
-template <int MT, int NT>
+    conv_wino_body<MT, NT, false, EPI>(grp, wino_args());
+}
+
+template <int MT, int NT, int EPI>
 __global__ __launch_bounds__(256, (MT == 1 ? (NT == 3 ? 4 : 3) : 2)) void conv_wino_fin_f32(const ConvGroupK grp) {
-    conv_wino_body<MT, NT, true>(grp, wino_args());
-}
-
-}
-
-void* i2r_pick_conv_wino(int nt, int mt, int fin) {
+    conv_wino_body<MT, NT, true, EPI>(grp, wino_args());
+}
+
+template <int NT>
+conv_fn pick_form(int fin, int epi) {
+    switch (epi + 3 * (fin != 0)) {
+        case 0: return conv_wino_f32<1, NT, 0>;
+        case 1: return conv_wino_f32<1, NT, 1>;
+        case 2: return conv_wino_f32<1, NT, 2>;
+        case 3: return conv_wino_fin_f32<1, NT, 0>;
+        case 4: return conv_wino_fin_f32<1, NT, 1>;
+        case 5: return conv_wino_fin_f32<1, NT, 2>;
+    }
+    return nullptr;
+}
+
+}
+
+void* i2r_pick_conv_wino(int nt, int mt, int fin, int epi) {
     conv_fn fn = nullptr;
-    if (mt == 1 && nt == 3) fn = fin ? conv_wino_fin_f32<1, 3> : conv_wino_f32<1, 3>;
-    if (mt == 1 && nt == 4) fn = fin ? conv_wino_fin_f32<1, 4> : conv_wino_f32<1, 4>;
+    if (epi < 0 || epi > 2) return nullptr;
+    if (mt == 1 && nt == 3) fn = pick_form<3>(fin, epi);
+    if (mt == 1 && nt == 4) fn = pick_form<4>(fin, epi);
     return reinterpret_cast<void*>(fn);
 }
 
diff --git a/intra-and-inter-human-relation-network-for-mpee_amd/engine.py b/intra-and-inter-human-relation-network-for-mpee_amd/engine.py
--- a/intra-and-inter-human-relation-network-for-mpee_amd/engine.py
+++ b/intra-and-inter-human-relation-network-for-mpee_amd/engine.py
@@ -28,6 +28,7 @@
 PRUNE_FUSE = True
 WINOGRAD = True
 WINO_SEQ = True
+WINO_FORMS = True
 PROFILER_ATTACHED = bool(os.environ.get("ROCP_TOOL_LIBRARIES") or os.environ.get("ROCPROFILER_LIBRARY_CTOR") or os.environ.get("HSA_TOOLS_LIB")
                          or any(t in os.environ.get("LD_PRELOAD", "") for t in ("rocprof", "roctracer", "rocprofiler")))
 DEVICE_SYNC = not PROFILER_ATTACHED
@@ -123,6 +124,16 @@
     nb = nfrag // nt
     wn = 4 if nb % 4 == 0 else 2 if nb % 2 == 0 else 1
     return nt, wn
+
+
+_wino_forms_pushed = None
+
+
+def push_wino_forms():
+    global _wino_forms_pushed
+    if _wino_forms_pushed != bool(WINO_FORMS):
+        cabi.check(cabi.lib().i2r_conv_wino_forms(int(bool(WINO_FORMS))), "i2r_conv_wino_forms")
+        _wino_forms_pushed = bool(WINO_FORMS)
 
 
 class Program:
@@ -258,6 +269,7 @@
             mt = 1
             d.tile_h, d.tile_w, d.mt, d.wn, d.ck = fh, fw, mt, 1, 0
             d.seq = 0 if WINO_SEQ else 1
+            push_wino_forms()
             n_frag = x.n * -(-conv_h // fh) * -(-conv_w // fw)
             geo = ("wino", -(-n_frag // mt) * (nfrag // nt))
             key = ("wino", nt, mt)
@@ -868,6 +880,7 @@
 
     def run(self, side_streams=None, events=None):
         L = cabi.lib()
+        push_wino_forms()
         cur = torch.cuda.current_stream(self.device).cuda_stream
         if side_streams is None:
             streams = (C.c_void_p * 4)(cur, cur, cur, cur)
```

New measurement: 8951 images/sec, median of 6. +2.0%, better.
